# jhong93/vpd

Hardware: AMD Instinct MI355X
Metric: frame-crops/sec (VPD student train) (higher is better)
Workload: dtype bf16; 1 GPU; configs[1]: Diving48-shaped synthetic crops 128x128, ResNet-34 student (5-ch RGB+flow), emb_dim 128, sum-MSE + AdamW, batch=256 per GPU; global_batch=256, parallelism=dp1

## Files before the change

include/vpd_hip.h:

```cpp
#ifndef VPD_HIP_H
#define VPD_HIP_H
#include <stddef.h>
#ifdef __cplusplus
extern "C" {
#endif

typedef struct vpd_plan vpd_plan_t;

const char* vpd_last_error(void);
int vpd_abi_version(void);
const char* vpd_elem_dtype(void);

int vpd_plan_create(const char* arch, int c_in, int img_h, int img_w, int emb_dim, int motion,
                    int max_batch, int train, vpd_plan_t** out);
#define VPD_TRAIN_EARLY_BUCKET0 2
void vpd_plan_destroy(vpd_plan_t* plan);

int vpd_plan_num_tensors(const vpd_plan_t* plan);
int vpd_plan_tensor_info(const vpd_plan_t* plan, int i, int* kind, int* is_decoder, long long* offset,
                         long long* numel, int* ndim, int dims[4]);
long long vpd_plan_param_numel(const vpd_plan_t* plan);
int vpd_plan_num_bn(const vpd_plan_t* plan);
int vpd_plan_bn_info(const vpd_plan_t* plan, int i, int* channels, long long* rm_off, long long* rv_off);
long long vpd_plan_bn_numel(const vpd_plan_t* plan);

int vpd_plan_num_buckets(const vpd_plan_t* plan);
int vpd_plan_bucket_range(const vpd_plan_t* plan, int bucket, long long* offset, long long* numel);

size_t vpd_plan_workspace_bytes(const vpd_plan_t* plan);
int vpd_plan_init_workspace(vpd_plan_t* plan, void* workspace, void* stream);

int vpd_pack_weights(vpd_plan_t* plan, const float* params, const float* bn_running, void* workspace, void* stream);

int vpd_forward_eval(vpd_plan_t* plan, const float* params, const float* x, int n, float* emb_out,
                     const float* target, float* loss_step, double* loss_accum, void* workspace, void* stream);


int vpd_forward_train(vpd_plan_t* plan, const float* params, float* bn_running, const float* x,
                      const float* target, int n, float* emb_out, float* loss_step, double* loss_accum,
                      void* workspace, void* stream);

int vpd_backward(vpd_plan_t* plan, const float* params, float* grads, int n, void** bucket_events,
                 void* workspace, void* stream);

int vpd_backward_ext(vpd_plan_t* plan, const float* params, float* grads, const float* d_emb, int n, float* dx_nchw,
                     void** bucket_events, void* workspace, void* stream);

int vpd_adamw_step(float* params, const float* grads, float* adam_m, float* adam_v, long long numel,
                   double lr, double beta1, double beta2, double eps, double weight_decay, int step, void* stream);

int vpd_plan_adamw_step(vpd_plan_t* plan, float* params, const float* grads, float* adam_m, float* adam_v,
                        long long numel, double lr, double beta1, double beta2, double eps, double weight_decay,
                        int step, void* workspace, void* stream);

int vpd_plan_set_loss_scale(vpd_plan_t* plan, float scale);

typedef struct vpd_scale_state {
    float scale;
    unsigned int found;
    int growth_tracker;
    int applied_steps;
    int skipped_steps;
    int reserved[3];
} vpd_scale_state;

int vpd_plan_set_scale_state(vpd_plan_t* plan, const vpd_scale_state* state);

int vpd_plan_check_grads(vpd_plan_t* plan, const float* grads, long long numel, vpd_scale_state* state, void* workspace,
                         void* stream);
int vpd_op_check_finite(const float* x, long long n, vpd_scale_state* state, void* stream);

int vpd_adamw_step_scaled(float* params, const float* grads, float* adam_m, float* adam_v, long long numel, double lr,
                          double beta1, double beta2, double eps, double weight_decay, const vpd_scale_state* state,
                          void* stream);
int vpd_plan_adamw_step_scaled(vpd_plan_t* plan, float* params, const float* grads, float* adam_m, float* adam_v,
                               long long numel, double lr, double beta1, double beta2, double eps, double weight_decay,
                               const vpd_scale_state* state, void* workspace, void* stream);

int vpd_scale_state_update(vpd_scale_state* state, float growth, float backoff, int growth_interval, void* stream);

int vpd_plan_set_lazy_grads(vpd_plan_t* plan, int on);
int vpd_plan_bucket_scratch_range(const vpd_plan_t* plan, int bucket, long long* ws_byte_offset, long long* numel);
int vpd_plan_grads_pending(const vpd_plan_t* plan);
int vpd_plan_materialize_grads(vpd_plan_t* plan, float* grads, void* workspace, void* stream);

typedef struct vpd_aug_params {
    int order[4];
    float factor[4];
    int flip;
    int noise;
    int crop_i, crop_j, crop_h, crop_w;
    unsigned int seed_lo, seed_hi;
} vpd_aug_params;

int vpd_augment_crops(const unsigned char* rgb_u8, const unsigned char* flow_u8, const unsigned char* mask_u8,
                      const float* noise, const vpd_aug_params* params, int n, int height, int width, int out_dim,
                      const float* mean_std6, float noise_sd, float* out_nchw, float* scratch, void* stream);
int vpd_plan_stage_crops(vpd_plan_t* plan, const unsigned char* rgb_u8, const unsigned char* flow_u8,
                         const unsigned char* mask_u8, const float* noise, const vpd_aug_params* params, int n,
                         int height, int width, const float* mean_std6, float noise_sd, float* scratch,
                         void* workspace, void* stream);

int vpd_plan_stage_views(vpd_plan_t* plan, const unsigned char* rgb_u8, const unsigned char* flow_u8, int n_frames,
                         int k_views, int height, int width, const float* mean_std6, void* workspace, void* stream);

int vpd_augment_views(const unsigned char* rgb_u8, const unsigned char* flow_u8, const vpd_aug_params* params, int n_frames,
                      int jitter, int flip, int height, int width, const float* mean_std6, float* out_nchw, float* scratch,
                      void* stream);
int vpd_plan_stage_views_jitter(vpd_plan_t* plan, const unsigned char* rgb_u8, const unsigned char* flow_u8,
                                const vpd_aug_params* params, int n_frames, int jitter, int flip, int height, int width,
                                const float* mean_std6, float* scratch, void* workspace, void* stream);

int vpd_graph_capture_eval(vpd_plan_t* plan, const float* params, const float* x, int n, float* emb_out,
                           void* workspace, void* stream);
int vpd_graph_launch_eval(vpd_plan_t* plan, int n, void* stream);

int vpd_plan_sync_errors(vpd_plan_t* plan, void* workspace, void* stream, unsigned* count_out);

int vpd_plan_set_timing(vpd_plan_t* plan, int enable);
int vpd_plan_read_timing(vpd_plan_t* plan, double* out, int nclasses);

int vpd_op_conv2d(const void* x_bf16, const void* w_bf16, void* y_bf16, double* stats, int n, int xHp, int xWp,
                  int xC, int yHp, int yWp, int yC, int ypad, int Hs, int Ws, int osub, int oph, int opw, int istr,
                  int Kc, int Co, const int* tapset9, int accumulate, void* stream);
int vpd_op_conv_bm(int M, int Co);
int vpd_op_conv2d_ep(const void* x_bf16, const void* w_bf16, void* y_bf16, int n, int xHp, int xWp, int xC, int yHp, int yWp,
                     int yC, int ypad, int Hs, int Ws, int istr, int Kc, int Co, const int* tapset9, const float* ep_scale,
                     const float* ep_shift, const void* res_padded_bf16, int ep_relu, int accumulate,
                     const unsigned char* acc_mask, void* stream);
int vpd_op_conv2d_bnsums(const void* x_bf16, const void* w_bf16, void* y_bf16, const void* bst_z_bf16,
                         const unsigned char* bst_mask, double* rows, int n, int xHp, int xWp, int xC, int Hs, int Ws,
                         int Kc, int Co, const int* tapset9, int accumulate, void* stream);
int vpd_op_conv2d_bnsums2(const void* x_bf16, const void* w_bf16, void* y_bf16, const void* bst_z_bf16,
                          const unsigned char* bst_mask, double* rows, const void* bst_z2_bf16, double* rows2, int n, int xHp,
                          int xWp, int xC, int Hs, int Ws, int Kc, int Co, const int* tapset9, void* stream);
int vpd_op_conv2d_dispatch(int n, int xHp, int xWp, int xC, int yHp, int yWp, int yC, int ypad, int Hs, int Ws, int osub, int oph,
                           int opw, int istr, int Kc, int Co, const int* tapset9, int accumulate, int flags, int* out12);
int vpd_op_bn_forward(const void* z_bf16, const double* rows, const float* gamma, const float* beta, float* running_mean,
                      float* running_var, float* mean, float* rstd, float* scale, float* shift, const void* res_padded_bf16,
                      void* out_padded_bf16, unsigned char* mask_bits, int n, int H, int W, int C, int relu, float momentum,
                      float eps, void* stream);
int vpd_op_bn_backward_apply(const void* dy_bf16, const void* z_bf16, const unsigned char* mask_bits, const double* rows,
                             const float* gamma, const float* mean, const float* rstd, void* dz_padded_bf16, float* dgamma,
                             float* dbeta, int n, int H, int W, int C, void* stream);
int vpd_op_conv1x1_bn(int mode, const void* x_padded, const void* w, int n, int H, int W, int istr, int Kc, int Co, double* rows,
                      const float* gamma, const float* beta, float* running_mean, float* running_var, float momentum, float eps,
                      float* mean, float* rstd, float* scale, float* shift, const void* res_padded, void* out_padded,
                      unsigned char* mask_bits, const void* dout, void* dz_padded, float* dgamma, float* dbeta, void* stream);
int vpd_op_conv1x1_bn2(int mode, const void* x_padded, const void* w, const void* x2_padded, const void* w2, int n, int H, int W,
                       int Kc, int Kc2, int Co, double* rows, double* rows2, const float* gamma, const float* beta,
                       float* running_mean, float* running_var, float* mean, float* rstd, float* scale, float* shift,
                       const float* gamma2, const float* beta2, float* running_mean2, float* running_var2, float* mean2, float* rstd2,
                       float* scale2, float* shift2, float momentum, float eps, void* out_padded, unsigned char* mask_bits,
                       const void* dout, void* dz_padded, void* dz2_padded, float* dgamma, float* dbeta, float* dgamma2,
                       float* dbeta2, void* stream);
int vpd_op_conv1x1_bn_dispatch(int n, int H, int W, int Kc, int Co, int two, int* out5);
int vpd_op_stem_pool_forward(const void* z, const float* scale, const float* shift, void* out_padded, unsigned char* idx,
                             int n, int Hz, int Wz, int C, int opad, void* stream);
int vpd_op_stem_dgrad(const void* dz, const float* w_oihw, float* dx_nchw, int n, int c_in, int H, int W, void* stream);
int vpd_op_stem_pool_backward(const void* dpool, const unsigned char* idx, const void* z, const float* mean, const float* rstd,
                              const float* scale, const float* shift, const float* gamma, const float* beta,
                              const void* pooled_padded, double* rows, float* coef, void* dz, float* dgamma, float* dbeta,
                              int n, int Hz, int Wz, int C, void* stream);
int vpd_op_bn_backward(void* dy, const void* z, const void* act_padded, const unsigned char* mask_bits, const float* mscale,
                       const float* mshift, const float* dy_pooled, double* rows, float* coef, void* sync, unsigned* err,
                       const float* gamma, const float* mean, const float* rstd, void* dz, int dzpad, float* dgamma,
                       float* dbeta, int n, int H, int W, int C, int write_g, int fused, void* stream);
int vpd_op_bn_backward_pair(void* dy, const void* act_padded, const void* zA, const float* meanA, const float* rstdA,
                            const float* gammaA, double* rowsA, void* dzA, float* dgammaA, float* dbetaA, const void* zB,
                            const float* meanB, const float* rstdB, const float* gammaB, double* rowsB, void* dzB,
                            float* dgammaB, float* dbetaB, void* sync, unsigned* err, int n, int H, int W, int C, void* stream);
int vpd_op_bn_backward_residency(int M, int C, int pair, int* out4);
int vpd_op_avgpool(const void* act_padded, int n, int H, int W, int C, int pad, float* pooled, void* stream);
int vpd_op_avgpool_bwd(const float* dpooled, int n, int H, int W, int C, void* dact, void* stream);
int vpd_op_sgemm(const float* A, const float* B, float* Y, const float* bias, int M, int N, int K, int ta, int tb, int relu,
                 void* stream);
int vpd_op_colsum(const float* A, int M, int N, float* out, void* stream);
int vpd_op_relu_mask(float* d, const float* act, long long n, void* stream);
int vpd_op_mse(const float* e, const float* t, long long n, float* de, float* loss_step, double* loss_accum, void* stream);
int vpd_op_wgrad(const void* dz_bf16, const void* x_bf16, float* dw, int n, int dzHp, int dzWp, int dzC, int dzpad,
                 int xHp, int xWp, int xC, int Hs, int Ws, int istr, int Kc, int Co, const int* tapset9,
                 float* slab, void* stream);
size_t vpd_op_wgrad_slab_bytes(void);
int vpd_op_wgrad_pair(const void* dz_bf16, const void* dz2_bf16, const void* x_bf16, float* dw, float* dw2, int n, int dzHp, int dzWp,
                      int dzC, int dzpad, int xHp, int xWp, int xC, int Hs, int Ws, int istr, int Kc, int Co, const int* tapset9,
                      float* slab, float* slab2, void* stream);
int vpd_op_wgrad_pair_lds_bytes(int Hs, int Ws, int ns, long long* bytes);
int vpd_op_tr_read_probe(const void* tile_bf16, void* out_bf16, void* stream);
size_t vpd_op_wgrad128_table_bytes(void);
size_t vpd_op_wgrad128_slab_floats(int Co, int Ci);
int vpd_op_wgrad128_group(int nprob, const void* const* dz, const void* const* x, float* const* dw, float* const* slab,
                          const int* dims, void* dev_table, void* stream);
int vpd_op_wgrad128_schedule(int n, const int* dims4, int G, int* ksplit, int* blk_begin, int* tasks, int cap,
                             double* est_us);

#ifdef __cplusplus
}
#endif
#endif
```

vpd_amd/_lib.py:

```python
import ctypes as C
import os

_HERE = os.path.dirname(os.path.abspath(__file__))
LIB_PATH = os.environ.get("VPD_LIB_PATH") or os.path.join(_HERE, "libvpdhip.so")
LIB_PATH_F16 = os.environ.get("VPD_LIB_PATH_F16") or os.path.join(_HERE, "libvpdhip_f16.so")
ABI_VERSION = 5

c_int_p = C.POINTER(C.c_int)
c_ll_p = C.POINTER(C.c_longlong)
vp = C.c_void_p

SIGNATURES = {
    "vpd_last_error": (C.c_char_p, []),
    "vpd_abi_version": (C.c_int, []),
    "vpd_elem_dtype": (C.c_char_p, []),
    "vpd_plan_create": (C.c_int, [C.c_char_p, C.c_int, C.c_int, C.c_int, C.c_int, C.c_int, C.c_int, C.c_int,
                                  C.POINTER(vp)]),
    "vpd_plan_destroy": (None, [vp]),
    "vpd_plan_num_tensors": (C.c_int, [vp]),
    "vpd_plan_tensor_info": (C.c_int, [vp, C.c_int, c_int_p, c_int_p, c_ll_p, c_ll_p, c_int_p, c_int_p]),
    "vpd_plan_param_numel": (C.c_longlong, [vp]),
    "vpd_plan_num_bn": (C.c_int, [vp]),
    "vpd_plan_bn_info": (C.c_int, [vp, C.c_int, c_int_p, c_ll_p, c_ll_p]),
    "vpd_plan_bn_numel": (C.c_longlong, [vp]),
    "vpd_plan_num_buckets": (C.c_int, [vp]),
    "vpd_plan_bucket_range": (C.c_int, [vp, C.c_int, c_ll_p, c_ll_p]),
    "vpd_plan_workspace_bytes": (C.c_size_t, [vp]),
    "vpd_plan_init_workspace": (C.c_int, [vp, vp, vp]),
    "vpd_pack_weights": (C.c_int, [vp, vp, vp, vp, vp]),
    "vpd_forward_eval": (C.c_int, [vp, vp, vp, C.c_int, vp, vp, vp, vp, vp, vp]),
    "vpd_forward_train": (C.c_int, [vp, vp, vp, vp, vp, C.c_int, vp, vp, vp, vp, vp]),
    "vpd_backward": (C.c_int, [vp, vp, vp, C.c_int, C.POINTER(vp), vp, vp]),
    "vpd_backward_ext": (C.c_int, [vp, vp, vp, vp, C.c_int, vp, C.POINTER(vp), vp, vp]),
    "vpd_adamw_step": (C.c_int, [vp, vp, vp, vp, C.c_longlong, C.c_double, C.c_double, C.c_double, C.c_double,
                                 C.c_double, C.c_int, vp]),
    "vpd_plan_adamw_step": (C.c_int, [vp, vp, vp, vp, vp, C.c_longlong, C.c_double, C.c_double, C.c_double, C.c_double,
                                      C.c_double, C.c_int, vp, vp]),
    "vpd_augment_crops": (C.c_int, [vp, vp, vp, vp, vp, C.c_int, C.c_int, C.c_int, C.c_int, C.POINTER(C.c_float),
                                    C.c_float, vp, vp, vp]),
    "vpd_plan_stage_crops": (C.c_int, [vp, vp, vp, vp, vp, vp, C.c_int, C.c_int, C.c_int, C.POINTER(C.c_float),
                                       C.c_float, vp, vp, vp]),
    "vpd_plan_stage_views": (C.c_int, [vp, vp, vp, C.c_int, C.c_int, C.c_int, C.c_int, C.POINTER(C.c_float), vp, vp]),
    "vpd_augment_views": (C.c_int, [vp, vp, vp, C.c_int, C.c_int, C.c_int, C.c_int, C.c_int, C.POINTER(C.c_float), vp, vp, vp]),
    "vpd_plan_stage_views_jitter": (C.c_int, [vp, vp, vp, vp, C.c_int, C.c_int, C.c_int, C.c_int, C.c_int,
                                              C.POINTER(C.c_float), vp, vp, vp]),
    "vpd_graph_capture_eval": (C.c_int, [vp, vp, vp, C.c_int, vp, vp, vp]),
    "vpd_graph_launch_eval": (C.c_int, [vp, C.c_int, vp]),
    "vpd_plan_sync_errors": (C.c_int, [vp, vp, vp, C.POINTER(C.c_uint)]),
    "vpd_plan_set_lazy_grads": (C.c_int, [vp, C.c_int]),
    "vpd_plan_set_loss_scale": (C.c_int, [vp, C.c_float]),
    "vpd_plan_set_scale_state": (C.c_int, [vp, vp]),
    "vpd_plan_check_grads": (C.c_int, [vp, vp, C.c_longlong, vp, vp, vp]),
    "vpd_op_check_finite": (C.c_int, [vp, C.c_longlong, vp, vp]),
    "vpd_adamw_step_scaled": (C.c_int, [vp, vp, vp, vp, C.c_longlong, C.c_double, C.c_double, C.c_double, C.c_double,
                                        C.c_double, vp, vp]),
    "vpd_plan_adamw_step_scaled": (C.c_int, [vp, vp, vp, vp, vp, C.c_longlong, C.c_double, C.c_double, C.c_double, C.c_double,
                                             C.c_double, vp, vp, vp]),
    "vpd_scale_state_update": (C.c_int, [vp, C.c_float, C.c_float, C.c_int, vp]),
    "vpd_plan_bucket_scratch_range": (C.c_int, [vp, C.c_int, C.POINTER(C.c_longlong), C.POINTER(C.c_longlong)]),
    "vpd_plan_grads_pending": (C.c_int, [vp]),
    "vpd_plan_materialize_grads": (C.c_int, [vp, vp, vp, vp]),
    "vpd_plan_set_timing": (C.c_int, [vp, C.c_int]),
    "vpd_plan_read_timing": (C.c_int, [vp, C.POINTER(C.c_double), C.c_int]),
    "vpd_op_conv2d": (C.c_int, [vp, vp, vp, vp] + [C.c_int] * 16 + [c_int_p, C.c_int, vp]),
    "vpd_op_conv_bm": (C.c_int, [C.c_int, C.c_int]),
    "vpd_op_conv2d_ep": (C.c_int, [vp, vp, vp] + [C.c_int] * 13 + [c_int_p, vp, vp, vp, C.c_int, C.c_int, vp, vp]),
    "vpd_op_conv2d_bnsums": (C.c_int, [vp] * 6 + [C.c_int] * 8 + [c_int_p, C.c_int, vp]),
    "vpd_op_conv2d_bnsums2": (C.c_int, [vp] * 8 + [C.c_int] * 8 + [c_int_p, vp]),
    "vpd_op_conv2d_dispatch": (C.c_int, [C.c_int] * 16 + [c_int_p, C.c_int, C.c_int, c_int_p]),
    "vpd_op_bn_forward": (C.c_int, [vp] * 13 + [C.c_int] * 5 + [C.c_float, C.c_float, vp]),
    "vpd_op_bn_backward_apply": (C.c_int, [vp] * 10 + [C.c_int] * 4 + [vp]),
    "vpd_op_conv1x1_bn": (C.c_int, [C.c_int, vp, vp] + [C.c_int] * 6 + [vp] * 5 + [C.c_float, C.c_float] + [vp] * 12),
    "vpd_op_conv1x1_bn2": (C.c_int, [C.c_int] + [vp] * 4 + [C.c_int] * 6 + [vp] * 18 + [C.c_float, C.c_float] + [vp] * 10),
    "vpd_op_conv1x1_bn_dispatch": (C.c_int, [C.c_int] * 6 + [c_int_p]),
    "vpd_op_stem_pool_forward": (C.c_int, [vp] * 5 + [C.c_int] * 5 + [vp]),
    "vpd_op_stem_dgrad": (C.c_int, [vp, vp, vp, C.c_int, C.c_int, C.c_int, C.c_int, vp]),
    "vpd_op_stem_pool_backward": (C.c_int, [vp] * 15 + [C.c_int] * 4 + [vp]),
    "vpd_op_bn_backward": (C.c_int, [vp] * 15 + [C.c_int] + [vp, vp] + [C.c_int] * 6 + [vp]),
    "vpd_op_bn_backward_pair": (C.c_int, [vp] * 20 + [C.c_int] * 4 + [vp]),
    "vpd_op_bn_backward_residency": (C.c_int, [C.c_int, C.c_int, C.c_int, c_int_p]),
    "vpd_op_avgpool": (C.c_int, [vp] + [C.c_int] * 5 + [vp, vp]),
    "vpd_op_avgpool_bwd": (C.c_int, [vp] + [C.c_int] * 4 + [vp, vp]),
    "vpd_op_sgemm": (C.c_int, [vp] * 4 + [C.c_int] * 6 + [vp]),
    "vpd_op_colsum": (C.c_int, [vp, C.c_int, C.c_int, vp, vp]),
    "vpd_op_relu_mask": (C.c_int, [vp, vp, C.c_longlong, vp]),
    "vpd_op_mse": (C.c_int, [vp, vp, C.c_longlong, vp, vp, vp, vp]),
    "vpd_op_wgrad": (C.c_int, [vp, vp, vp] + [C.c_int] * 13 + [c_int_p, vp, vp]),
    "vpd_op_wgrad_slab_bytes": (C.c_size_t, []),
    "vpd_op_wgrad_pair": (C.c_int, [vp] * 5 + [C.c_int] * 13 + [c_int_p, vp, vp, vp]),
    "vpd_op_wgrad_pair_lds_bytes": (C.c_int, [C.c_int, C.c_int, C.c_int, c_ll_p]),
    "vpd_op_tr_read_probe": (C.c_int, [vp, vp, vp]),
    "vpd_op_wgrad128_table_bytes": (C.c_size_t, []),
    "vpd_op_wgrad128_slab_floats": (C.c_size_t, [C.c_int, C.c_int]),
    "vpd_op_wgrad128_group": (C.c_int, [C.c_int, vp, vp, vp, vp, c_int_p, vp, vp]),
    "vpd_op_wgrad128_schedule": (C.c_int, [C.c_int, c_int_p, C.c_int, c_int_p, c_int_p, c_int_p, C.c_int,
                                           C.POINTER(C.c_double)]),
}

_libs = {}


class VpdHipError(RuntimeError):
    pass


def lib(dtype="bf16"):
    if dtype in _libs:
        return _libs[dtype]
    if dtype not in ("bf16", "fp16"):
        raise VpdHipError("unknown element type %r (bf16 | fp16)" % (dtype,))
    path = LIB_PATH if dtype == "bf16" else LIB_PATH_F16
    name = os.path.basename(path)
    if not os.path.isfile(path):
        raise VpdHipError(
            "%s not found at %s: build it with `python -c 'import __graft_entry__ as g; g.build()'` "
            "or `make -C vpd_amd/csrc`.  vpd_amd has no PyTorch/CPU fallback." % (name, path))
    import torch
    h = C.CDLL(path)
    ab_build = "VPD_LIB_PATH" in os.environ and dtype == "bf16"
    for sym, (res, args) in SIGNATURES.items():
        try:
            fn = getattr(h, sym)
        except AttributeError as e:
            if ab_build and (sym.startswith("vpd_op_") or sym in ("vpd_elem_dtype", "vpd_plan_set_loss_scale", "vpd_backward_ext")):
                continue
            raise VpdHipError("%s lacks symbol %s declared in include/vpd_hip.h" % (name, sym)) from e
        fn.restype = res
        fn.argtypes = args
    if h.vpd_abi_version() != ABI_VERSION and not (ab_build and os.environ.get("VPD_LIB_ALLOW_ABI") == str(h.vpd_abi_version())):
        raise VpdHipError("%s ABI version %d != expected %d" % (name, h.vpd_abi_version(), ABI_VERSION))
    if hasattr(h, "vpd_elem_dtype") and h.vpd_elem_dtype().decode() != dtype:
        raise VpdHipError("%s was built with %s elements, %s asked for" % (path, h.vpd_elem_dtype().decode(), dtype))
    _libs[dtype] = h
    return h


def check(rc, what="", dtype="bf16"):
    if rc != 0:
        msg = lib(dtype).vpd_last_error()
        raise VpdHipError("%s failed: %s" % (what or "libvpdhip call", msg.decode() if msg else "unknown error"))
```

vpd_amd/csrc/head.hip:

```cpp
#include "../../include/vpd_hip.h"
#include "common.h"
#include "kernels.h"

__global__ __launch_bounds__(256) void avgpool_kernel(const bf16_t* act, int Hp, int Wp, int pad, int H, int W, int C,
                                                      int N, float* pooled) {
    const int cv = C >> 3;
    const long total = (long)N * cv;
    const float inv = 1.f / (float)(H * W);
    for (long it = (long)blockIdx.x * blockDim.x + threadIdx.x; it < total; it += (long)gridDim.x * blockDim.x) {
        const int b = (int)(it / cv);
        const int c = (int)(it - (long)b * cv) << 3;
        float acc[8] = {0, 0, 0, 0, 0, 0, 0, 0};
        if (H == 4 && W == 4) {
            uint4 px[16];
#pragma unroll
            for (int q = 0; q < 16; ++q)
                px[q] = *reinterpret_cast<const uint4*>(act + ((size_t)(b * Hp + (q >> 2) + pad) * Wp + (q & 3) + pad) * C + c);
#pragma unroll
            for (int q = 0; q < 16; ++q) {
                float v[8];
                unpack8(px[q], v);
#pragma unroll
                for (int j = 0; j < 8; ++j) acc[j] += v[j];
            }
        } else {
            for (int y = 0; y < H; ++y)
                for (int x = 0; x < W; ++x) {
                    float v[8];
                    unpack8(*reinterpret_cast<const uint4*>(act + ((size_t)(b * Hp + y + pad) * Wp + x + pad) * C + c), v);
#pragma unroll
                    for (int j = 0; j < 8; ++j) acc[j] += v[j];
                }
        }
        float* o = pooled + (size_t)b * C + c;
#pragma unroll
        for (int j = 0; j < 8; ++j) o[j] = acc[j] * inv;
    }
}
hipError_t vpd_launch_avgpool(const bf16_t* act, int Hp, int Wp, int pad, int H, int W, int C, int N, float* pooled,
                              hipStream_t s) {
    long items = (long)N * (C / 8);
    int g = (int)((items + 255) / 256);
    hipLaunchKernelGGL(avgpool_kernel, dim3(g < 1 ? 1 : g), dim3(256), 0, s, act, Hp, Wp, pad, H, W, C, N, pooled);
    return hipGetLastError();
}

__global__ __launch_bounds__(256) void avgpool_bwd_kernel(const float* dpooled, int HW, int C, int N, bf16_t* dact) {
    const int cv = C >> 3;
    const long total = (long)N * HW * cv;
    const float inv = 1.f / (float)HW;
    const bool pow2 = (HW & (HW - 1)) == 0;
    for (long it = (long)blockIdx.x * blockDim.x + threadIdx.x; it < total; it += (long)gridDim.x * blockDim.x) {
        const int c = (int)(it % cv) << 3;
        const long m = it / cv;
        const int b = (int)(m / HW);
        float v[8];
        const float* d = dpooled + (size_t)b * C + c;
#pragma unroll
        for (int j = 0; j < 8; ++j) v[j] = pow2 ? d[j] * inv : d[j] / (float)HW;
        *reinterpret_cast<uint4*>(dact + (size_t)m * C + c) = pack8(v);
    }
}
hipError_t vpd_launch_avgpool_bwd(const float* dpooled, int H, int W, int C, int N, bf16_t* dact, hipStream_t s) {
    long items = (long)N * H * W * (C / 8);
    long g = (items + 255) / 256;
    if (g > 4096) g = 4096;
    hipLaunchKernelGGL(avgpool_bwd_kernel, dim3(g < 1 ? 1 : (int)g), dim3(256), 0, s, dpooled, H * W, C, N, dact);
    return hipGetLastError();
}

__global__ __launch_bounds__(256) void sgemm_small_kernel(const float* A, const float* B, float* Y, const float* bias,
                                                          int M, int N, int K, int ta, int tb, int relu) {
    const int lane = threadIdx.x & 63;
    const int tiles_n = (N + 15) >> 4;
    const int tile = blockIdx.x * 4 + (threadIdx.x >> 6);
    const int tm = tile / tiles_n, tn = tile - tm * tiles_n;
    if (tm * 16 >= M) return;
    const int r = lane & 15, kq = lane >> 4;
    const int m = tm * 16 + r, n = tn * 16 + r;
    const bool mok = m < M, nok = n < N;
    f32x4 acc = {0.f, 0.f, 0.f, 0.f};
    const size_t a_m = ta ? (size_t)(mok ? m : 0) : (size_t)(mok ? m : 0) * K;
    const size_t a_k = ta ? (size_t)M : 1;
    const size_t b_n = tb ? (size_t)(nok ? n : 0) * K : (size_t)(nok ? n : 0);
    const size_t b_k = tb ? 1 : (size_t)N;
    for (int k0 = 0; k0 < K; k0 += 32) {
        float av[8], bv[8];
#pragma unroll
        for (int u = 0; u < 8; ++u) {
            const int k = k0 + 4 * u + kq;
            const bool kok = k < K;
            av[u] = (mok && kok) ? A[a_m + (size_t)k * a_k] : 0.f;
            bv[u] = (nok && kok) ? B[b_n + (size_t)k * b_k] : 0.f;
        }
#pragma unroll
        for (int u = 0; u < 8; ++u) acc = __builtin_amdgcn_mfma_f32_16x16x4f32(av[u], bv[u], acc, 0, 0, 0);
    }
    if (nok) {
        const float bb = bias ? bias[n] : 0.f;
#pragma unroll
        for (int j = 0; j < 4; ++j) {
            const int mm = tm * 16 + 4 * kq + j;
            if (mm < M) {
                float v = acc[j] + bb;
                if (relu) v = v > 0.f ? v : 0.f;
                Y[(size_t)mm * N + n] = v;
            }
        }
    }
}
__global__ __launch_bounds__(256) void sgemm_nt_splitk_kernel(const float* A, const float* B, float* Y, const float* bias,
                                                              int M, int N, int K, int relu) {
    __shared__ float red[4][16][17];
    const int lane = threadIdx.x & 63, wave = threadIdx.x >> 6;
    const int tiles_n = (N + 15) >> 4;
    const int tm = blockIdx.x / tiles_n, tn = blockIdx.x - tm * tiles_n;
    const int r = lane & 15, kq = lane >> 4;
    const int m = tm * 16 + r, n = tn * 16 + r;
    const bool mok = m < M, nok = n < N;
    const float4* Ap = reinterpret_cast<const float4*>(A + (size_t)(mok ? m : 0) * K);
    const float4* Bp = reinterpret_cast<const float4*>(B + (size_t)(nok ? n : 0) * K);
    const int kper = K / 4;
    f32x4 acc = {0.f, 0.f, 0.f, 0.f};
    for (int k0 = wave * kper; k0 < (wave + 1) * kper; k0 += 64) {
        float4 av[4], bv[4];
#pragma unroll
        for (int u = 0; u < 4; ++u) {
            const int k = k0 + 16 * u + 4 * kq;
            const bool kok = k < (wave + 1) * kper;
            av[u] = (mok && kok) ? Ap[k >> 2] : float4{0.f, 0.f, 0.f, 0.f};
            bv[u] = (nok && kok) ? Bp[k >> 2] : float4{0.f, 0.f, 0.f, 0.f};
        }
#pragma unroll
        for (int u = 0; u < 4; ++u) {
            acc = __builtin_amdgcn_mfma_f32_16x16x4f32(av[u].x, bv[u].x, acc, 0, 0, 0);
            acc = __builtin_amdgcn_mfma_f32_16x16x4f32(av[u].y, bv[u].y, acc, 0, 0, 0);
            acc = __builtin_amdgcn_mfma_f32_16x16x4f32(av[u].z, bv[u].z, acc, 0, 0, 0);
            acc = __builtin_amdgcn_mfma_f32_16x16x4f32(av[u].w, bv[u].w, acc, 0, 0, 0);
        }
    }
#pragma unroll
    for (int j = 0; j < 4; ++j) red[wave][4 * kq + j][r] = acc[j];
    __syncthreads();
    if (wave == 0 && nok) {
        const float bb = bias ? bias[n] : 0.f;
#pragma unroll
        for (int j = 0; j < 4; ++j) {
            const int mm = tm * 16 + 4 * kq + j;
            if (mm < M) {
                float v = ((red[0][4 * kq + j][r] + red[1][4 * kq + j][r]) + red[2][4 * kq + j][r]) + red[3][4 * kq + j][r] + bb;
                if (relu) v = v > 0.f ? v : 0.f;
                Y[(size_t)mm * N + n] = v;
            }
        }
    }
}

hipError_t vpd_launch_sgemm(const float* A, const float* B, float* Y, const float* bias, int M, int N, int K, int ta,
                            int tb, int relu, hipStream_t s) {
    const int tiles = ((M + 15) / 16) * ((N + 15) / 16);
    if (!ta && tb && K % 64 == 0 && K >= 64) {
        hipLaunchKernelGGL(sgemm_nt_splitk_kernel, dim3(tiles), dim3(256), 0, s, A, B, Y, bias, M, N, K, relu);
        return hipGetLastError();
    }
    hipLaunchKernelGGL(sgemm_small_kernel, dim3((tiles + 3) / 4), dim3(256), 0, s, A, B, Y, bias, M, N, K, ta, tb, relu);
    return hipGetLastError();
}

__global__ __launch_bounds__(256) void colsum_kernel(const float* A, int M, int N, float* out) {
    __shared__ float sh[8][32];
    const int tx = threadIdx.x & 31, ty = threadIdx.x >> 5;
    const int n = blockIdx.x * 32 + tx;
    float a = 0.f;
    if (n < N)
        for (int m = ty; m < M; m += 8) a += A[(size_t)m * N + n];
    sh[ty][tx] = a;
    __syncthreads();
    if (ty == 0 && n < N) {
        float t = 0.f;
#pragma unroll
        for (int i = 0; i < 8; ++i) t += sh[i][tx];
        out[n] = t;
    }
}
hipError_t vpd_launch_colsum(const float* A, int M, int N, float* out, hipStream_t s) {
    hipLaunchKernelGGL(colsum_kernel, dim3((N + 31) / 32), dim3(256), 0, s, A, M, N, out);
    return hipGetLastError();
}

__global__ void relu_mask_kernel(float* d, const float* act, long n) {
    for (long i = (long)blockIdx.x * blockDim.x + threadIdx.x; i < n; i += (long)gridDim.x * blockDim.x)
        d[i] = act[i] > 0.f ? d[i] : 0.f;
}
hipError_t vpd_launch_relu_mask(float* d, const float* act, long n, hipStream_t s) {
    long g = (n + 255) / 256;
    if (g > 1024) g = 1024;
    hipLaunchKernelGGL(relu_mask_kernel, dim3(g < 1 ? 1 : (int)g), dim3(256), 0, s, d, act, n);
    return hipGetLastError();
}

__global__ __launch_bounds__(1024) void mse_kernel(const float* e, const float* t, long n, float* de,
                                                   float* loss_step, double* loss_accum) {
    __shared__ float sh[16];
    float a = 0.f;
    const long n4 = n >> 2;
    for (long i0 = threadIdx.x; i0 < n4; i0 += 8 * 1024) {
        float4 ev[8], tv[8];
#pragma unroll
        for (int u = 0; u < 8; ++u) {
            const long i = i0 + u * 1024;
            const long ic = i < n4 ? i : i0;
            ev[u] = reinterpret_cast<const float4*>(e)[ic];
            tv[u] = reinterpret_cast<const float4*>(t)[ic];
        }
#pragma unroll
        for (int u = 0; u < 8; ++u) {
            const long i = i0 + u * 1024;
            if (i < n4) {
                const float4 d = {ev[u].x - tv[u].x, ev[u].y - tv[u].y, ev[u].z - tv[u].z, ev[u].w - tv[u].w};
                a += d.x * d.x + d.y * d.y + d.z * d.z + d.w * d.w;
                if (de) reinterpret_cast<float4*>(de)[i] = float4{2.f * d.x, 2.f * d.y, 2.f * d.z, 2.f * d.w};
            }
        }
    }
    for (long i = (n4 << 2) + threadIdx.x; i < n; i += 1024) {
        const float d = e[i] - t[i];
        a += d * d;
        if (de) de[i] = 2.f * d;
    }
    a = wave_sum(a);
    if ((threadIdx.x & 63) == 0) sh[threadIdx.x >> 6] = a;
    __syncthreads();
    if (threadIdx.x == 0) {
        float tot = 0.f;
#pragma unroll
        for (int i = 0; i < 16; ++i) tot += sh[i];
        if (loss_step) loss_step[0] = tot;
        if (loss_accum) loss_accum[0] += (double)tot;
    }
}
hipError_t vpd_launch_mse(const float* e, const float* t, long n, float* de, float* loss_step, double* loss_accum,
                          hipStream_t s) {
    hipLaunchKernelGGL(mse_kernel, dim3(1), dim3(1024), 0, s, e, t, n, de, loss_step, loss_accum);
    return hipGetLastError();
}


__global__ __launch_bounds__(256) void scale_kernel(float* x, long n, float s) {
    for (long i = (long)blockIdx.x * 256 + threadIdx.x; i < n; i += (long)gridDim.x * 256) x[i] *= s;
}
hipError_t vpd_launch_scale(float* x, long n, float s, hipStream_t stream) {
    if (n <= 0) return hipSuccess;
    long g = (n + 255) / 256;
    if (g > 1024) g = 1024;
    hipLaunchKernelGGL(scale_kernel, dim3((unsigned)g), dim3(256), 0, stream, x, n, s);
    return hipGetLastError();
}
__global__ __launch_bounds__(256) void scale_by_state_kernel(float* x, long n, const vpd_scale_state* st) {
    const float s = st->scale;
    for (long i = (long)blockIdx.x * 256 + threadIdx.x; i < n; i += (long)gridDim.x * 256) x[i] *= s;
}
hipError_t vpd_launch_scale_by_state(float* x, long n, const vpd_scale_state* st, hipStream_t stream) {
    if (n <= 0) return hipSuccess;
    long g = (n + 255) / 256;
    if (g > 1024) g = 1024;
    hipLaunchKernelGGL(scale_by_state_kernel, dim3((unsigned)g), dim3(256), 0, stream, x, n, st);
    return hipGetLastError();
}
```

vpd_amd/csrc/kernels.h:

```cpp
#pragma once
#include <vector>

#include "common.h"

struct BnApplyParams {
    const bf16_t* z;
    const float* scale; const float* shift;
    int res_kind;
    const bf16_t* res; int rHp, rWp, rpad;
    const float* rscale; const float* rshift;
    bf16_t* out; int oHp, oWp, opad;
    int M, H, W, C, relu;
    unsigned char* mask_out;
    int xcd_tile_px;
};

struct StemPoolParams {
    const bf16_t* z; int Hz, Wz;
    const float* scale; const float* shift;
    bf16_t* out; int opad;
    unsigned char* idx;
    int N, Ho, Wo, C;
};

struct BnBwdParams {
    const bf16_t* dy;
    bf16_t* dy_rw;
    const bf16_t* z;
    const bf16_t* act; int aHp, aWp, apad;
    const float* mean; const float* rstd;
    float* coef;
    double* partials;
    bf16_t* dz; int dzHp, dzWp, dzpad;
    int M, H, W, C, write_g, ppb;
    const float* mscale; const float* mshift;
    const unsigned char* mask_bits;
    const float* dy_pooled; float dy_pool_scale;
    int xcd_tile_px;
};

struct StemPoolBwdParams {
    const bf16_t* dpool;
    const unsigned char* idx;
    const bf16_t* z;
    const float* mean; const float* rstd; const float* scale; const float* shift;
    bf16_t* g;
    double* partials;
    int M, Hz, Wz, Ho, Wo, C, ppb;
    int pass; const float* coef; bf16_t* dz;
    const bf16_t* pooled; int ppad; const float* gamma_p; const float* beta_p;
};

struct PackDesc {
    long long src_off;
    long long fwd_off;
    long long dgr_off;
    long long wg_off;
    int Co, Ci, kh, kw, Kc, ntaps, stem;
    long long numel;
};
struct AdamHyper { float decay, omb1, b2, omb2, step_size, inv_sqrt_bc2, eps, gscale; };
struct vpd_scale_state;
struct AdamHyperDyn { AdamHyper h; const vpd_scale_state* st; double lr, b1, b2; };
#define FR_MAX 96
struct FiniteRanges {
    const float* ptr[FR_MAX];
    long n[FR_MAX];
    int count;
};

hipError_t vpd_launch_conv(const ConvParams& p, hipStream_t stream);
hipError_t vpd_launch_scale(float* x, long n, float s, hipStream_t stream);
bool vpd_conv1x1_stream_eligible(const ConvParams& p);
hipError_t vpd_launch_conv1x1_stream(const ConvParams& p, hipStream_t stream);
void vpd_conv1x1_stream_grid(const ConvParams& p, int* bm, int* bn, int* lanes);
int vpd_conv_kernel_class(const ConvParams& p);
bool vpd_conv_takes_bn_sums(const ConvParams& p);
struct ConvDispatch {
    int kclass;
    int pws;
    int geo;
    int c64x2;
    int ws1x1, stream1x1;
    int halo;
    int bm, bn;
    int mode;
    int tiles_per_block;
};
ConvDispatch vpd_conv_dispatch(const ConvParams& p);
int vpd_conv_xcd_tile_px(const ConvParams& p);
hipError_t vpd_launch_wgrad_reduce(const WgradParams& p, hipStream_t stream);
extern "C" int vpd_conv_bm(int M, int Co);
hipError_t vpd_launch_wgrad(const WgradParams& p, hipStream_t stream);
size_t vpd_wgrad_slab_bytes();
bool vpd_wgrad_group_eligible(const WgradParams& p);
size_t vpd_wgrad_group_slab_floats(int M, int Co, int Kc, int ntaps = 9);
hipError_t vpd_launch_wgrad_group(const WgradParams* ps, int n, hipStream_t stream);
bool vpd_wgrad_overwrites(const WgradParams& p);
bool vpd_wgrad_pair_ok(const WgradParams& p3, const WgradParams& p1);
hipError_t vpd_launch_wgrad_pair(const WgradParams& p3, const WgradParams& p1, hipStream_t stream);
hipError_t vpd_launch_wgrad_pair_reduce(const WgradParams& p3, const WgradParams& p1, hipStream_t stream);
int vpd_wgrad_pair_lds_query(int H, int W, int ns, long long* bytes);
bool vpd_wgrad128_eligible(const WgradParams& p);
size_t vpd_wgrad128_table_bytes();
void* vpd_wgrad128_cache_new();
void vpd_wgrad128_cache_free(void* cache);
hipError_t vpd_launch_wgrad128_group(const WgradParams* ps, int n, void* cache, void* dev_table, hipStream_t stream);
bool vpd_wgrad_halo_shape_ok(int Hout, int Wout, int stride = 1, int Hin = 0, int Win = 0);

hipError_t vpd_launch_bn_finalize(double* partials, int T, int C, float count, const float* gamma,
                                  const float* beta, float* rm, float* rv, float momentum, float eps,
                                  float* mean, float* rstd, float* scale, float* shift, hipStream_t s);
hipError_t vpd_launch_bn_fold(const float* gamma, const float* beta, const float* rm, const float* rv, float eps,
                              float* scale, float* shift, int C, hipStream_t s);
hipError_t vpd_launch_bn_apply(const BnApplyParams& p, hipStream_t s);
hipError_t vpd_launch_stem_pool(const StemPoolParams& p, hipStream_t s);
int vpd_bn_bwd_blocks(int M, int C, int* ppb_out);
hipError_t vpd_launch_bn_bwd(const BnBwdParams& p, float count, const float* gamma, float* dgamma, float* dbeta,
                             hipStream_t s, bool reduce_done = false);
hipError_t vpd_launch_stem_pool_bwd(const StemPoolBwdParams& p, float count, const float* gamma, float* dgamma,
                                    float* dbeta, float* coef, bf16_t* dz, hipStream_t s);

struct BnFusedFwd {
    double* rows; float count; const float* gamma; const float* beta; float* rm; float* rv;
    float* mean; float* rstd; float* scale; float* shift;
    double* rows2; float count2; const float* gamma2; const float* beta2; float* rm2; float* rv2;
    float* mean2; float* rstd2; float* scale2; float* shift2;
    float momentum, eps;
};
struct BnFusedBwd {
    double* rows; void* sync; unsigned* err;
    const float* gamma; float* dgamma; float* dbeta; float count;
};
struct BnBwdSecond {
    BnFusedBwd f;
    const bf16_t* z; const float* mean; const float* rstd;
    bf16_t* dz;
};
#define VPD_GRID_SYNC_BYTES (18 * 128)
hipError_t vpd_launch_bn_fwd_fused(const BnApplyParams& p, const BnFusedFwd& f, hipStream_t s);
bool vpd_conv1x1_bn_eligible(const ConvParams& p);
bool vpd_conv1x1_bn2_eligible(const ConvParams& p);
hipError_t vpd_launch_conv1x1_bn2(const ConvParams& p, const BnFusedFwd* fwd, const BnFusedBwd* bwd3, const BnFusedBwd* bwdD,
                                  const float* mean3, const float* rstd3, const float* meanD, const float* rstdD,
                                  unsigned char* mask_out, bf16_t* dz3, bf16_t* dzD, int dzpad, int mode, hipStream_t stream);
hipError_t vpd_launch_conv1x1_bn(const ConvParams& p, const BnFusedFwd* fwd, const BnFusedBwd* bwd, const float* mean,
                                 const float* rstd, unsigned char* mask_out, bf16_t* dz, int dzpad, int mode, hipStream_t stream);
void vpd_conv1x1_bn_grid(const ConvParams& p, bool two, int out4[4]);
bool vpd_bn_bwd_fused_ok(int M, int C, bool mask_act, bool write_g);
struct BnBwdFusedGeom { int G, ppb, iters, keep[3]; size_t lds; };
BnBwdFusedGeom vpd_bn_bwd_fused_geom(int M, int C, int nt);
hipError_t vpd_launch_bn_bwd_fused(const BnBwdParams& p, const BnFusedBwd& f, hipStream_t s);
hipError_t vpd_launch_bn_bwd_apply_fused(const BnBwdParams& p, const BnFusedBwd& f, hipStream_t s, const BnBwdSecond* B = nullptr);
bool vpd_bn_bwd_fused2_ok(int M, int C);
hipError_t vpd_launch_bn_bwd_fused2(const BnBwdParams& p, const BnFusedBwd& fA, const BnBwdSecond& B, hipStream_t s);

hipError_t vpd_launch_stem_dgrad(const bf16_t* dz, const float* w_oihw, float* dx_nchw, int N, int Cin, int H, int W,
                                 hipStream_t s);

hipError_t vpd_launch_avgpool(const bf16_t* act, int Hp, int Wp, int pad, int H, int W, int C, int N, float* pooled,
                              hipStream_t s);
hipError_t vpd_launch_avgpool_bwd(const float* dpooled, int H, int W, int C, int N, bf16_t* dact, hipStream_t s);
hipError_t vpd_launch_sgemm(const float* A, const float* B, float* Y, const float* bias, int M, int N, int K, int ta,
                            int tb, int relu, hipStream_t s);
hipError_t vpd_launch_colsum(const float* A, int M, int N, float* out, hipStream_t s);
hipError_t vpd_launch_relu_mask(float* d, const float* act, long n, hipStream_t s);
hipError_t vpd_launch_mse(const float* e, const float* t, long n, float* de, float* loss_step, double* loss_accum,
                          hipStream_t s);

hipError_t vpd_launch_pack_input(const float* x, int N, int C, int H, int W, bf16_t* out, int Hp, int Wp, int pad,
                                 int Cp, hipStream_t s);
hipError_t vpd_launch_pack_weights(const PackDesc* d_descs, int ndesc, const int* d_blockmap, int nblocks,
                                   const float* master, bf16_t* arena, hipStream_t s);
hipError_t vpd_launch_adamw_pack(const PackDesc* d_descs, const int* d_blockmap, int nblocks, float* p, const float* g,
                                 float* m, float* v, bf16_t* arena, double lr, double b1, double b2, double eps, double wd,
                                 int step, hipStream_t s, const float* wg = nullptr, float gscale = 1.f);
hipError_t vpd_launch_unpack_grads(const PackDesc* d_descs, int ndesc, const int* d_blockmap, int nblocks,
                                   const float* wg, float* grads, hipStream_t s);
hipError_t vpd_launch_adamw(float* p, const float* g, float* m, float* v, long n, double lr, double b1, double b2,
                            double eps, double wd, int step, hipStream_t s, float gscale = 1.f);
hipError_t vpd_launch_adamw_pack_scaled(const PackDesc* d_descs, const int* d_blockmap, int nblocks, float* p, const float* g,
                                        float* m, float* v, bf16_t* arena, double lr, double b1, double b2, double eps,
                                        double wd, const vpd_scale_state* st, hipStream_t s, const float* wg = nullptr);
hipError_t vpd_launch_adamw_scaled(float* p, const float* g, float* m, float* v, long n, double lr, double b1, double b2,
                                   double eps, double wd, const vpd_scale_state* st, hipStream_t s);
hipError_t vpd_launch_check_finite(const FiniteRanges& r, vpd_scale_state* st, hipStream_t s);
hipError_t vpd_launch_scale_update(vpd_scale_state* st, float growth, float backoff, int interval, hipStream_t s);
hipError_t vpd_launch_scale_by_state(float* x, long n, const vpd_scale_state* st, hipStream_t stream);

#define ZR_MAX 16
struct ZeroRanges {
    float* ptr[ZR_MAX];
    long n4[ZR_MAX];
    int count;
};
hipError_t vpd_launch_zero_ranges(const ZeroRanges& z, hipStream_t s);

struct vpd_aug_params;
hipError_t vpd_launch_augment(const unsigned char* rgb, const unsigned char* flow, const unsigned char* mask,
                              const float* noise, const vpd_aug_params* params, int N, int H, int W, int out_dim,
                              const float* mean_std6, float noise_sd, float* out_nchw, bf16_t* xin, int xHp, int xWp,
                              int xpad, float* cmean_scratch, hipStream_t s);
hipError_t vpd_launch_views(const unsigned char* rgb, const unsigned char* flow, int F, int K, int H, int W,
                            const float* mean_std6, bf16_t* xin, int xHp, int xWp, int xpad, hipStream_t s);
hipError_t vpd_launch_views_jitter(const unsigned char* rgb, const unsigned char* flow, const vpd_aug_params* params, int F,
                                   int J, int flip, int H, int W, const float* mean_std6, float* out_nchw, bf16_t* xin,
                                   int xHp, int xWp, int xpad, float* cmean_scratch, hipStream_t s);
```

vpd_amd/csrc/plan.h:

```cpp
#pragma once
#include <hip/hip_runtime.h>
#include <string.h>

#include <vector>

#include "../../include/vpd_hip.h"
#include "common.h"
#include "kernels.h"

int fail(const char* what, hipError_t e = hipSuccess);
#define HCHECK(expr)                                   \
    do {                                               \
        hipError_t _e = (expr);                        \
        if (_e != hipSuccess) return fail(#expr, _e);  \
    } while (0)
#define LCHECK(expr)                                   \
    do {                                               \
        hipError_t _e = (expr);                        \
        if (_e != hipSuccess) return fail(#expr, _e);  \
    } while (0)

constexpr float kBnEps = 1e-5f;
constexpr float kBnMomentum = 0.1f;

struct BnInfo {
    int C = 0;
    long long w_off = 0, b_off = 0;
    long long rm_off = 0, rv_off = 0;
    size_t fl_off = 0;
    size_t rows_off = 0;
    size_t sync_off = 0;
};
struct ConvInfo {
    int Ci = 0, Co = 0, k = 0, stride = 1, pad = 0;
    int Hin = 0, Win = 0, Hout = 0, Wout = 0;
    bool stem = false;
    int Kc = 0, ntaps = 0;
    long long w_off = 0;
    long long fwd_off = 0, dgr_off = -1;
    long long wg_off = 0;
    long long slab_off = -1;
    size_t dz_own_off = 0;
    long long gslab_off = 0;
    BnInfo bn;
    size_t z_off = 0;
};
struct BlockInfo {
    ConvInfo c1, c2, c3, cd;
    bool ds = false;
    int stage = 0;
    size_t a1_off = 0, a2_off = 0, out_off = 0;
    size_t mask_off = 0;
    size_t mask1_off = 0;
    size_t mask2_off = 0;
};
struct StageInfo {
    int H = 0, W = 0, C = 0;
    size_t dz2_off[2] = {0, 0}, dz1_off[2] = {0, 0}, dzd_off = 0, idn_off = 0;
    size_t dz3_off = 0;
};
struct TensorRow {
    int kind, is_dec;
    long long off, numel;
    int ndim, dims[4];
};
struct LinInfo {
    int in = 0, out = 0;
    long long w_off = 0, b_off = 0;
};

struct vpd_plan {
    int c_in, H, W, D, motion, max_batch, train;
    int bottleneck = 0, base_width = 64, feat = 512;
    std::vector<int> layers;
    ConvInfo stem;
    std::vector<BlockInfo> blocks;
    StageInfo stages[4];
    LinInfo fc, dec[3];
    std::vector<TensorRow> tensors;
    std::vector<BnInfo*> bns;
    long long nparam = 0, nparam_padded = 0, nbn = 0;
    long long arena_elems = 0, wg_elems = 0, slab_elems = 0;
    long long bucket_off[4], bucket_numel[4];
    long long bucket_wg_off[4], bucket_wg_numel[4];
    size_t ws_bytes = 0;
    size_t xin_off = 0, arena_off = 0, wg_off = 0, partial_off = 0, z0_off = 0, p0_off = 0, idx_off = 0;
    size_t g0_off = 0, dz0_off = 0, G_off[3] = {0, 0, 0}, T_off[2] = {0, 0}, slab_off = 0;
    size_t pooled_off = 0, emb_off = 0, h1_off = 0, h2_off = 0, pred_off = 0;
    size_t dpred_off = 0, dh2_off = 0, dh1_off = 0, demb_off = 0, dpooled_off = 0;
    size_t desc_off = 0, bmap_pack_off = 0, bmap_unpack_off[4] = {0, 0, 0, 0};
    int xHp = 0, xWp = 0;
    int H0 = 0, W0 = 0, H1 = 0, W1 = 0;
    std::vector<PackDesc> descs;
    std::vector<int> bmap_pack;
    std::vector<int> bmap_adam;
    size_t bmap_adam_off = 0;
    int nstem_pack_blocks = 0;
    std::vector<int> bmap_unpack[4];
    size_t partial_bytes = 0;
    struct Graph { int n; hipGraph_t g; hipGraphExec_t e; };
    std::vector<Graph> graphs;
    void* bound_ws = nullptr;
    bool fused_bn = true;
    size_t fused_off = 0, fused_bytes = 0;
    size_t syncerr_off = 0;
    bool wg_group = true;
    size_t gslab_off = 0;
    bool dgrad_sums = true;
    bool relu_bits = true;
    bool lazy_next = false, grads_in_scratch = false;
    bool fwd_had_x = false;
    int nstem_unpack_blocks = 0;
    bool wg_merge34 = true;
    bool early_bucket0 = false;
    float loss_scale = 1.f;
    const vpd_scale_state* scale_state = nullptr;
    size_t wg2_tbl_off[8] = {0, 0, 0, 0, 0, 0, 0, 0};
    void* wg2_cache[8] = {nullptr, nullptr, nullptr, nullptr, nullptr, nullptr, nullptr, nullptr};
    bool timing = false;
    struct TimedLaunch { int cls; double flops; hipEvent_t a, b; };
    std::vector<TimedLaunch> timed;
    std::vector<hipEvent_t> ev_pool;
};

int check_call(const vpd_plan* p, const void* ws, int n, int min_n = 1);

inline TapSet conv_taps_fwd(const ConvInfo& c) {
    TapSet t;
    if (c.stem) {
        t.nr = c.k; t.nc = 1; t.dy0 = 0; t.dys = 1; t.dx0 = 0; t.dxs = 0; t.w0 = 0; t.wrs = 1; t.wcs = 0;
    } else {
        t.nr = c.k; t.nc = c.k; t.dy0 = 1 - c.pad; t.dys = 1; t.dx0 = 1 - c.pad; t.dxs = 1;
        t.w0 = 0; t.wrs = c.k; t.wcs = 1;
    }
    return t;
}

inline WgradParams wgrad_params(const ConvInfo& cv, int n, const bf16_t* dz, const bf16_t* x) {
    WgradParams q;
    memset(&q, 0, sizeof q);
    q.dz = dz; q.dzHp = cv.Hout + 2; q.dzWp = cv.Wout + 2; q.dzC = cv.Co; q.dzpad = 1;
    q.x = x; q.xHp = cv.Hin + 2; q.xWp = cv.Win + 2; q.xC = cv.Ci;
    q.N = n; q.Hs = cv.Hout; q.Ws = cv.Wout; q.istr = cv.stride; q.Kc = cv.Kc; q.Co = cv.Co;
    q.M = n * cv.Hout * cv.Wout;
    q.taps = conv_taps_fwd(cv);
    return q;
}
inline WgradParams grouped_wgrad_params(const ConvInfo& cv, int n, const bf16_t* dz, const bf16_t* x) {
    WgradParams q = wgrad_params(cv, n, dz, x);
    if (cv.k == 1 && cv.stride == 1 && cv.Co % 128 != 0 && cv.Ci % 128 == 0) {
        q.dz = x; q.dzC = cv.Ci; q.x = dz; q.xC = cv.Co; q.Co = cv.Ci; q.Kc = cv.Co; q.transposed = 1;
    }
    return q;
}
```

vpd_amd/csrc/plan.hip:

```cpp
#include <hip/hip_runtime.h>
#include <math.h>
#include <stdio.h>
#include <stdlib.h>
#include <string.h>

#include <string>
#include <algorithm>
#include <vector>

#include "plan.h"

static thread_local std::string g_err;
int fail(const char* what, hipError_t e) {
    char buf[512];
    if (e != hipSuccess) snprintf(buf, sizeof buf, "%s: %s", what, hipGetErrorString(e));
    else snprintf(buf, sizeof buf, "%s", what);
    g_err = buf;
    return -1;
}

extern "C" const char* vpd_last_error(void) { return g_err.c_str(); }
extern "C" const char* vpd_elem_dtype(void) { return VPD_ELEM_NAME; }
extern "C" int vpd_abi_version(void) { return 5; }

namespace {

struct Bump {
    size_t cur = 0;
    size_t take(size_t bytes) {
        size_t o = cur;
        cur += (bytes + 255) & ~(size_t)255;
        return o;
    }
};

inline size_t padded_elems(int n, int H, int W, int C, int pad) {
    return (size_t)n * (H + 2 * pad) * (W + 2 * pad) * C;
}

void add_tensor(vpd_plan* p, int kind, int is_dec, long long numel, int ndim, int d0, int d1, int d2, int d3,
                long long* off_out) {
    TensorRow r;
    r.kind = kind; r.is_dec = is_dec; r.off = p->nparam; r.numel = numel; r.ndim = ndim;
    r.dims[0] = d0; r.dims[1] = d1; r.dims[2] = d2; r.dims[3] = d3;
    p->tensors.push_back(r);
    *off_out = p->nparam;
    p->nparam += numel;
}

void add_conv(vpd_plan* p, ConvInfo& c, int Ci, int Co, int k, int stride, int pad, int Hin, int Win, bool stem) {
    c.Ci = Ci; c.Co = Co; c.k = k; c.stride = stride; c.pad = pad; c.Hin = Hin; c.Win = Win; c.stem = stem;
    c.Hout = (Hin + 2 * pad - k) / stride + 1;
    c.Wout = (Win + 2 * pad - k) / stride + 1;
    if (stem) { c.Kc = 64; c.ntaps = k; } else { c.Kc = Ci; c.ntaps = k * k; }
    add_tensor(p, 0, 0, (long long)Co * Ci * k * k, 4, Co, Ci, k, k, &c.w_off);
    c.bn.C = Co;
    add_tensor(p, 1, 0, Co, 1, Co, 0, 0, 0, &c.bn.w_off);
    add_tensor(p, 2, 0, Co, 1, Co, 0, 0, 0, &c.bn.b_off);
    c.bn.rm_off = p->nbn; c.bn.rv_off = p->nbn + Co;
    p->nbn += 2 * Co;
    c.fwd_off = p->arena_elems;
    p->arena_elems += (long long)c.ntaps * Co * c.Kc;
    if (!stem) {
        c.dgr_off = p->arena_elems;
        p->arena_elems += (long long)k * k * Ci * Co;
    }
    c.wg_off = p->wg_elems;
    p->wg_elems += (long long)c.ntaps * Co * c.Kc;
    if (stem && p->train && p->slab_elems == 0)
        p->slab_elems += 2 * (long long)(vpd_wgrad_slab_bytes() / 4);
    if (!stem && ((k == 3 && pad == 1) || (k == 1 && pad == 0)) && (stride == 1 || stride == 2) && p->train &&
        vpd_wgrad_halo_shape_ok(c.Hout, c.Wout, stride, Hin, Win)) {
        c.slab_off = k == 1 ? (long long)(vpd_wgrad_slab_bytes() / 4) : 0;
    }
}

}

extern "C" int vpd_plan_create(const char* arch, int c_in, int img_h, int img_w, int emb_dim, int motion,
                               int max_batch, int train, vpd_plan_t** out) {
    if (!arch || !out) return fail("null argument");
    std::vector<int> layers;
    int bottleneck = 0, base_width = 64;
    if (!strcmp(arch, "resnet18")) layers = {2, 2, 2, 2};
    else if (!strcmp(arch, "resnet34")) layers = {3, 4, 6, 3};
    else if (!strcmp(arch, "resnet50")) { layers = {3, 4, 6, 3}; bottleneck = 1; }
    else if (!strcmp(arch, "resnet101")) { layers = {3, 4, 23, 3}; bottleneck = 1; }
    else if (!strcmp(arch, "wide_resnet50_2")) { layers = {3, 4, 6, 3}; bottleneck = 1; base_width = 128; }
    else if (!strcmp(arch, "wide_resnet101_2")) { layers = {3, 4, 23, 3}; bottleneck = 1; base_width = 128; }
    else return fail("unsupported arch (resnet18 | resnet34 | resnet50 | resnet101 | wide_resnet50_2 | wide_resnet101_2)");
    if (c_in < 1 || c_in > 8) return fail("c_in must be in 1..8");
    if (img_h < 32 || img_w < 32 || (img_h % 2) || (img_w % 2)) return fail("img dims must be even and >= 32");
    if (emb_dim < 1 || max_batch < 1) return fail("bad emb_dim / max_batch");

    vpd_plan* p = new vpd_plan();
    p->c_in = c_in; p->H = img_h; p->W = img_w; p->D = emb_dim; p->motion = motion ? 1 : 0;
    p->max_batch = max_batch; p->train = train ? 1 : 0; p->layers = layers;
    p->early_bucket0 = (train & VPD_TRAIN_EARLY_BUCKET0) != 0;
    p->bottleneck = bottleneck; p->base_width = base_width; p->feat = bottleneck ? 2048 : 512;

    add_conv(p, p->stem, c_in, 64, 7, 2, 3, img_h, img_w, true);
    p->bns.push_back(&p->stem.bn);
    p->H0 = p->stem.Hout; p->W0 = p->stem.Wout;
    p->H1 = (p->H0 + 2 - 3) / 2 + 1; p->W1 = (p->W0 + 2 - 3) / 2 + 1;
    int inplanes = 64, h = p->H1, w = p->W1;
    const int widths[4] = {64, 128, 256, 512};
    long long stage_first_tensor_off[5];
    int nblocks_total = 0;
    for (int s = 0; s < 4; ++s) nblocks_total += layers[s];
    p->blocks.resize(nblocks_total);
    int bi = 0;
    for (int s = 0; s < 4; ++s) {
        stage_first_tensor_off[s] = p->nparam;
        for (int b = 0; b < layers[s]; ++b, ++bi) {
            BlockInfo& B = p->blocks[bi];
            const int stride = (b == 0 && s > 0) ? 2 : 1;
            B.stage = s;
            if (!bottleneck) {
                add_conv(p, B.c1, inplanes, widths[s], 3, stride, 1, h, w, false);
                add_conv(p, B.c2, widths[s], widths[s], 3, 1, 1, B.c1.Hout, B.c1.Wout, false);
                B.ds = (stride != 1 || inplanes != widths[s]);
                if (B.ds) add_conv(p, B.cd, inplanes, widths[s], 1, stride, 0, h, w, false);
                h = B.c1.Hout; w = B.c1.Wout; inplanes = widths[s];
            } else {
                const int width = widths[s] * base_width / 64, outc = widths[s] * 4;
                add_conv(p, B.c1, inplanes, width, 1, 1, 0, h, w, false);
                add_conv(p, B.c2, width, width, 3, stride, 1, h, w, false);
                add_conv(p, B.c3, width, outc, 1, 1, 0, B.c2.Hout, B.c2.Wout, false);
                B.ds = (stride != 1 || inplanes != outc);
                if (B.ds) add_conv(p, B.cd, inplanes, outc, 1, stride, 0, h, w, false);
                h = B.c2.Hout; w = B.c2.Wout; inplanes = outc;
            }
        }
        p->stages[s].H = h; p->stages[s].W = w; p->stages[s].C = inplanes;
    }
    for (auto& B : p->blocks) {
        p->bns.push_back(&B.c1.bn);
        p->bns.push_back(&B.c2.bn);
        if (bottleneck) p->bns.push_back(&B.c3.bn);
        if (B.ds) p->bns.push_back(&B.cd.bn);
    }
    if (h < 1 || w < 1) { delete p; return fail("image too small for 5 stride-2 stages"); }
    stage_first_tensor_off[4] = p->nparam;
    p->fc.in = p->feat; p->fc.out = emb_dim;
    add_tensor(p, 3, 0, (long long)emb_dim * p->feat, 2, emb_dim, p->feat, 0, 0, &p->fc.w_off);
    add_tensor(p, 4, 0, emb_dim, 1, emb_dim, 0, 0, 0, &p->fc.b_off);
    if (p->motion) {
        const int dims[4] = {emb_dim, 128, 128, 2 * emb_dim};
        for (int i = 0; i < 3; ++i) {
            p->dec[i].in = dims[i]; p->dec[i].out = dims[i + 1];
            add_tensor(p, 3, 1, (long long)dims[i + 1] * dims[i], 2, dims[i + 1], dims[i], 0, 0, &p->dec[i].w_off);
            add_tensor(p, 4, 1, dims[i + 1], 1, dims[i + 1], 0, 0, 0, &p->dec[i].b_off);
        }
    }
    p->nparam_padded = (p->nparam + 3) & ~3LL;
    p->bucket_off[0] = stage_first_tensor_off[3]; p->bucket_numel[0] = p->nparam - stage_first_tensor_off[3];
    p->bucket_off[1] = stage_first_tensor_off[2]; p->bucket_numel[1] = stage_first_tensor_off[3] - stage_first_tensor_off[2];
    p->bucket_off[2] = stage_first_tensor_off[1]; p->bucket_numel[2] = stage_first_tensor_off[2] - stage_first_tensor_off[1];
    p->bucket_off[3] = 0; p->bucket_numel[3] = stage_first_tensor_off[1];

    auto push_desc = [&](const ConvInfo& c, int bucket) {
        PackDesc d;
        d.src_off = c.w_off; d.fwd_off = c.fwd_off; d.dgr_off = c.dgr_off; d.wg_off = c.wg_off;
        d.Co = c.Co; d.Ci = c.Ci; d.kh = c.k; d.kw = c.k; d.Kc = c.Kc; d.ntaps = c.ntaps; d.stem = c.stem ? 1 : 0;
        d.numel = 0;
        const int id = (int)p->descs.size();
        p->descs.push_back(d);
        const long long nf = (long long)c.ntaps * c.Co * c.Kc;
        const long long ns = (long long)c.Co * c.Ci * c.k * c.k;
        const long long npk = nf > ns ? nf : ns;
        const long long npack = c.stem ? (npk + 1023) / 1024 : (long long)(c.Co / 32) * (c.Ci / 32);
        for (long long ch = 0; ch < npack; ++ch) { p->bmap_pack.push_back(id); p->bmap_pack.push_back((int)ch); }
        const long long uchunk = 1024;
        for (long long ch = 0; ch * uchunk < ns; ++ch) {
            p->bmap_unpack[bucket].push_back(id);
            p->bmap_unpack[bucket].push_back((int)ch);
        }
    };
    push_desc(p->stem, 3);
    p->nstem_unpack_blocks = (int)p->bmap_unpack[3].size() / 2;
    for (int b = 0; b < 4; ++b) { p->bucket_wg_off[b] = -1; p->bucket_wg_numel[b] = 0; }
    for (auto& B : p->blocks) {
        const int bucket = 3 - B.stage;
        push_desc(B.c1, bucket);
        push_desc(B.c2, bucket);
        if (bottleneck) push_desc(B.c3, bucket);
        if (B.ds) push_desc(B.cd, bucket);
        auto take = [&](const ConvInfo& cv) {
            const long long n = (long long)cv.ntaps * cv.Co * cv.Kc;
            if (p->bucket_wg_off[bucket] < 0) p->bucket_wg_off[bucket] = cv.wg_off;
            p->bucket_wg_off[bucket] = std::min(p->bucket_wg_off[bucket], (long long)cv.wg_off);
            p->bucket_wg_numel[bucket] += n;
        };
        take(B.c1); take(B.c2);
        if (bottleneck) take(B.c3);
        if (B.ds) take(B.cd);
    }
    {
        long long at = (long long)p->stem.ntaps * p->stem.Co * p->stem.Kc;
        for (int b = 3; b >= 0; --b) {
            if (p->bucket_wg_off[b] != at) { delete p; return fail("internal: weight-gradient scratch is not bucket-contiguous"); }
            at += p->bucket_wg_numel[b];
        }
        if (at != p->wg_elems) { delete p; return fail("internal: weight-gradient scratch size mismatch"); }
    }
    {
        const int nconv = (int)p->descs.size();
        for (size_t i = 0; i + 1 < p->bmap_pack.size(); i += 2) {
            if (p->bmap_pack[i] == 0) { p->nstem_pack_blocks++; continue; }
            p->bmap_adam.push_back(p->bmap_pack[i]); p->bmap_adam.push_back(p->bmap_pack[i + 1]);
        }
        std::vector<std::pair<long long, long long>> convs;
        for (int i = 1; i < nconv; ++i)
            convs.push_back({p->descs[i].src_off, (long long)p->descs[i].Co * p->descs[i].Ci * p->descs[i].kh * p->descs[i].kw});
        std::sort(convs.begin(), convs.end());
        long long pos = 0;
        auto plain = [&](long long a, long long b) {
            if (b <= a) return;
            PackDesc d = {};
            d.src_off = a; d.numel = b - a; d.stem = 2; d.kh = d.kw = 1; d.dgr_off = -1;
            const int id = (int)p->descs.size();
            p->descs.push_back(d);
            for (long long ch = 0; ch * 2048 < b - a; ++ch) { p->bmap_adam.push_back(id); p->bmap_adam.push_back((int)ch); }
        };
        for (auto& cv : convs) { plain(pos, cv.first); pos = cv.first + cv.second; }
        plain(pos, p->nparam_padded);
    }

    Bump bp;
    const int NB = max_batch;
    p->xHp = img_h + 6; p->xWp = img_w + 8;
    p->xin_off = bp.take(((size_t)NB * p->xHp * p->xWp * 8 + 256) * 2);
    p->arena_off = bp.take((size_t)p->arena_elems * 2);
    p->wg_off = bp.take((size_t)p->wg_elems * 4);
    for (BnInfo* b : p->bns) b->fl_off = bp.take((size_t)9 * b->C * 4);
    p->fused_bn = vpd_switches().fused_bn;
    {
        const size_t start = bp.cur;
        for (BnInfo* b : p->bns) {
            b->rows_off = bp.take((size_t)VPD_FUSED_ROWS * 2 * b->C * sizeof(double));
            b->sync_off = bp.take(VPD_GRID_SYNC_BYTES);
        }
        p->fused_off = start; p->fused_bytes = bp.cur - start;
        p->syncerr_off = bp.take(256);
    }
    p->desc_off = bp.take(p->descs.size() * sizeof(PackDesc));
    p->bmap_pack_off = bp.take(p->bmap_pack.size() * sizeof(int));
    p->bmap_adam_off = bp.take(p->bmap_adam.size() * sizeof(int));
    for (int i = 0; i < 4; ++i) p->bmap_unpack_off[i] = bp.take(p->bmap_unpack[i].size() * sizeof(int) + 16);
    p->partial_bytes = (size_t)VPD_STAT_ROWS * 2 * p->feat * sizeof(double);
    p->partial_off = bp.take(p->partial_bytes);
    p->z0_off = bp.take((size_t)NB * p->H0 * p->W0 * 64 * 2);
    p->p0_off = bp.take(padded_elems(NB, p->H1, p->W1, 64, 1) * 2);
    for (auto& B : p->blocks) {
        B.a1_off = bp.take(padded_elems(NB, B.c1.Hout, B.c1.Wout, B.c1.Co, 1) * 2);
        if (bottleneck) {
            B.a2_off = bp.take(padded_elems(NB, B.c2.Hout, B.c2.Wout, B.c2.Co, 1) * 2);
            B.out_off = bp.take(padded_elems(NB, B.c3.Hout, B.c3.Wout, B.c3.Co, 1) * 2);
        } else {
            B.out_off = bp.take(padded_elems(NB, B.c1.Hout, B.c1.Wout, B.c1.Co, 1) * 2);
        }
    }
    for (int s = 0; s < 4; ++s) {
        StageInfo& S = p->stages[s];
        S.idn_off = bp.take(padded_elems(NB, S.H, S.W, S.C, 1) * 2);
    }
    p->pooled_off = bp.take((size_t)NB * p->feat * 4);
    p->emb_off = bp.take((size_t)NB * emb_dim * 4);
    p->h1_off = bp.take((size_t)NB * 128 * 4);
    p->h2_off = bp.take((size_t)NB * 128 * 4);
    p->pred_off = bp.take((size_t)NB * 2 * emb_dim * 4);
    if (p->train) {
        p->idx_off = bp.take((size_t)NB * p->H1 * p->W1 * 64);
        size_t maxact = (size_t)NB * p->H1 * p->W1 * 64;
        for (auto& B : p->blocks) {
            B.c1.z_off = bp.take((size_t)NB * B.c1.Hout * B.c1.Wout * B.c1.Co * 2);
            B.c2.z_off = bp.take((size_t)NB * B.c2.Hout * B.c2.Wout * B.c2.Co * 2);
            if (bottleneck) B.c3.z_off = bp.take((size_t)NB * B.c3.Hout * B.c3.Wout * B.c3.Co * 2);
            if (B.ds) B.cd.z_off = bp.take((size_t)NB * B.cd.Hout * B.cd.Wout * B.cd.Co * 2);
            size_t e = (size_t)NB * B.c1.Hout * B.c1.Wout * B.c1.Co;
            maxact = e > maxact ? e : maxact;
            if (bottleneck) {
                e = (size_t)NB * B.c1.Hin * B.c1.Win * B.c1.Ci; maxact = e > maxact ? e : maxact;
                e = (size_t)NB * B.c2.Hout * B.c2.Wout * B.c2.Co; maxact = e > maxact ? e : maxact;
                e = (size_t)NB * B.c3.Hout * B.c3.Wout * B.c3.Co; maxact = e > maxact ? e : maxact;
            }
        }
        for (int s = 0; s < 4; ++s) {
            StageInfo& S = p->stages[s];
            for (int k = 0; k < 2; ++k) {
                S.dz2_off[k] = bp.take(padded_elems(NB, S.H, S.W, S.C, 1) * 2);
                S.dz1_off[k] = bp.take(padded_elems(NB, S.H, S.W, S.C, 1) * 2);
            }
            S.dzd_off = bp.take(padded_elems(NB, S.H, S.W, S.C, 1) * 2);
        }
        if (bottleneck) {
            for (int s = 0; s < 4; ++s) {
                size_t m1 = 0, m2 = 0, m3 = 0;
                for (auto& B : p->blocks) {
                    if (B.stage != s) continue;
                    size_t e1 = padded_elems(NB, B.c1.Hout, B.c1.Wout, B.c1.Co, 1), e2 = padded_elems(NB, B.c2.Hout, B.c2.Wout, B.c2.Co, 1),
                           e3 = padded_elems(NB, B.c3.Hout, B.c3.Wout, B.c3.Co, 1);
                    m1 = e1 > m1 ? e1 : m1; m2 = e2 > m2 ? e2 : m2; m3 = e3 > m3 ? e3 : m3;
                }
                StageInfo& S = p->stages[s];
                S.dz1_off[0] = S.dz1_off[1] = bp.take(m1 * 2);
                S.dz2_off[0] = S.dz2_off[1] = bp.take(m2 * 2);
                S.dz3_off = bp.take(m3 * 2);
            }
            for (int i = 0; i < 2; ++i) p->T_off[i] = bp.take(maxact * 2);
        }
        p->wg_group = vpd_switches().wg_group;
        p->wg_merge34 = vpd_switches().wg_merge && !p->early_bucket0;
        if (p->wg_group) {
            size_t stage_slab[4] = {0, 0, 0, 0};
            for (auto& B : p->blocks) {
                std::vector<ConvInfo*> cvs = {&B.c1, &B.c2};
                if (bottleneck) cvs.push_back(&B.c3);
                if (B.ds) cvs.push_back(&B.cd);
                for (ConvInfo* cv : cvs) {
                    if (cv->slab_off < 0) continue;
                    if (cv->k == 1) {
                        if (!bottleneck || !vpd_wgrad128_eligible(grouped_wgrad_params(*cv, NB, nullptr, nullptr))) continue;
                    } else if (cv->k != 3) {
                        continue;
                    } else if (cv->stride != 1) {
                        continue;
                    }
                    cv->dz_own_off = bp.take(padded_elems(NB, cv->Hout, cv->Wout, cv->Co, 1) * 2);
                    const int grp = (p->wg_merge34 && B.stage == 3) ? 2 : B.stage;
                    cv->gslab_off = (long long)stage_slab[grp];
                    stage_slab[grp] += vpd_wgrad_group_slab_floats(NB * cv->Hout * cv->Wout, cv->Co, cv->Kc, cv->k == 1 ? 1 : 9);
                }
            }
            size_t mx = 16;
            for (int s2 = 0; s2 < 4; ++s2) mx = stage_slab[s2] > mx ? stage_slab[s2] : mx;
            p->gslab_off = bp.take(mx * 4);
            for (int s2 = 0; s2 < 8; ++s2) p->wg2_tbl_off[s2] = bp.take(vpd_wgrad128_table_bytes());
        }
        p->relu_bits = vpd_switches().relu_bits;
        if (p->relu_bits)
            for (auto& B : p->blocks) {
                const ConvInfo& last = bottleneck ? B.c3 : B.c2;
                B.mask_off = bp.take((size_t)NB * last.Hout * last.Wout * last.Co / 8 + 16);
            }
        p->dgrad_sums = p->relu_bits && p->fused_bn && vpd_switches().dgrad_sums;
        if (p->dgrad_sums)
            for (auto& B : p->blocks) {
                if (bottleneck && B.stage < 2) continue;
                B.mask1_off = bp.take((size_t)NB * B.c1.Hout * B.c1.Wout * B.c1.Co / 8 + 16);
                if (bottleneck) B.mask2_off = bp.take((size_t)NB * B.c2.Hout * B.c2.Wout * B.c2.Co / 8 + 16);
            }
        for (int i = 0; i < 3; ++i) p->G_off[i] = bp.take(maxact * 2);
        p->slab_off = bp.take((size_t)(p->slab_elems > 0 ? p->slab_elems : 1) * 4);
        p->g0_off = bp.take((size_t)NB * p->H0 * p->W0 * 64 * 2);
        p->dz0_off = bp.take((size_t)NB * p->H0 * p->W0 * 64 * 2);
        p->dpred_off = bp.take((size_t)NB * 2 * emb_dim * 4);
        p->dh2_off = bp.take((size_t)NB * 128 * 4);
        p->dh1_off = bp.take((size_t)NB * 128 * 4);
        p->demb_off = bp.take((size_t)NB * emb_dim * 4);
        p->dpooled_off = bp.take((size_t)NB * p->feat * 4);
    }
    p->ws_bytes = bp.cur;
    *out = p;
    return 0;
}

extern "C" void vpd_plan_destroy(vpd_plan_t* p) {
    if (!p) return;
    for (auto& g : p->graphs) {
        (void)hipGraphExecDestroy(g.e);
        (void)hipGraphDestroy(g.g);
    }
    for (auto& t : p->timed) { (void)hipEventDestroy(t.a); (void)hipEventDestroy(t.b); }
    for (auto e : p->ev_pool) (void)hipEventDestroy(e);
    for (int i = 0; i < 8; ++i)
        if (p->wg2_cache[i]) vpd_wgrad128_cache_free(p->wg2_cache[i]);
    delete p;
}

extern "C" int vpd_plan_num_tensors(const vpd_plan_t* p) { return (int)p->tensors.size(); }
extern "C" int vpd_plan_tensor_info(const vpd_plan_t* p, int i, int* kind, int* is_decoder, long long* offset,
                                    long long* numel, int* ndim, int dims[4]) {
    if (i < 0 || i >= (int)p->tensors.size()) return fail("tensor index out of range");
    const TensorRow& r = p->tensors[i];
    *kind = r.kind; *is_decoder = r.is_dec; *offset = r.off; *numel = r.numel; *ndim = r.ndim;
    for (int k = 0; k < 4; ++k) dims[k] = r.dims[k];
    return 0;
}
extern "C" long long vpd_plan_param_numel(const vpd_plan_t* p) { return p->nparam_padded; }
extern "C" int vpd_plan_num_bn(const vpd_plan_t* p) { return (int)p->bns.size(); }
extern "C" int vpd_plan_bn_info(const vpd_plan_t* p, int i, int* channels, long long* rm_off, long long* rv_off) {
    if (i < 0 || i >= (int)p->bns.size()) return fail("bn index out of range");
    *channels = p->bns[i]->C; *rm_off = p->bns[i]->rm_off; *rv_off = p->bns[i]->rv_off;
    return 0;
}
extern "C" long long vpd_plan_bn_numel(const vpd_plan_t* p) { return p->nbn; }
extern "C" int vpd_plan_num_buckets(const vpd_plan_t*) { return 4; }
extern "C" int vpd_plan_bucket_range(const vpd_plan_t* p, int b, long long* offset, long long* numel) {
    if (b < 0 || b >= 4) return fail("bucket index out of range");
    *offset = p->bucket_off[b]; *numel = p->bucket_numel[b];
    return 0;
}
extern "C" int vpd_plan_bucket_scratch_range(const vpd_plan_t* p, int b, long long* ws_byte_offset, long long* numel) {
    if (b < 0 || b >= 4) return fail("bucket index out of range");
    if (!p->train) return fail("plan was created with train=0");
    *ws_byte_offset = (long long)p->wg_off + p->bucket_wg_off[b] * 4;
    *numel = p->bucket_wg_numel[b];
    return 0;
}
extern "C" size_t vpd_plan_workspace_bytes(const vpd_plan_t* p) { return p->ws_bytes; }

extern "C" int vpd_plan_init_workspace(vpd_plan_t* p, void* ws, void* stream) {
    hipStream_t s = (hipStream_t)stream;
    char* w = (char*)ws;
    HCHECK(hipMemsetAsync(ws, 0, p->ws_bytes, s));
    HCHECK(hipMemcpyAsync(w + p->desc_off, p->descs.data(), p->descs.size() * sizeof(PackDesc), hipMemcpyHostToDevice, s));
    HCHECK(hipMemcpyAsync(w + p->bmap_pack_off, p->bmap_pack.data(), p->bmap_pack.size() * sizeof(int), hipMemcpyHostToDevice, s));
    HCHECK(hipMemcpyAsync(w + p->bmap_adam_off, p->bmap_adam.data(), p->bmap_adam.size() * sizeof(int), hipMemcpyHostToDevice, s));
    for (int i = 0; i < 4; ++i)
        if (!p->bmap_unpack[i].empty())
            HCHECK(hipMemcpyAsync(w + p->bmap_unpack_off[i], p->bmap_unpack[i].data(),
                                  p->bmap_unpack[i].size() * sizeof(int), hipMemcpyHostToDevice, s));
    HCHECK(hipStreamSynchronize(s));
    p->bound_ws = ws;
    return 0;
}

int check_call(const vpd_plan* p, const void* ws, int n, int min_n) {
    if (!p || !ws) return fail("null plan / workspace");
    if (p->bound_ws != ws) return fail("workspace not initialised with vpd_plan_init_workspace");
    if (n < min_n || n > p->max_batch) return fail(min_n ? "batch size outside 1..max_batch" : "batch size outside 0..max_batch");
    return 0;
}

extern "C" int vpd_augment_crops(const unsigned char* rgb_u8, const unsigned char* flow_u8, const unsigned char* mask_u8,
                                 const float* noise, const vpd_aug_params* params, int n, int height, int width,
                                 int out_dim, const float* mean_std6, float noise_sd, float* out_nchw, float* scratch,
                                 void* stream) {
    if (!rgb_u8 || !params || !mean_std6 || !out_nchw || !scratch) return fail("null argument");
    if (n < 1 || height < 1 || width < 1 || out_dim < 1) return fail("bad shape");
    LCHECK(vpd_launch_augment(rgb_u8, flow_u8, mask_u8, noise, params, n, height, width, out_dim, mean_std6, noise_sd,
                              out_nchw, nullptr, 0, 0, 0, scratch, (hipStream_t)stream));
    return 0;
}

extern "C" int vpd_plan_stage_crops(vpd_plan_t* p, const unsigned char* rgb_u8, const unsigned char* flow_u8,
                                    const unsigned char* mask_u8, const float* noise, const vpd_aug_params* params,
                                    int n, int height, int width, const float* mean_std6, float noise_sd,
                                    float* scratch, void* workspace, void* stream) {
    if (n > 65535) return fail("more than 65535 crops per staging call");
    if (check_call(p, workspace, n)) return -1;
    if (!rgb_u8 || !params || !mean_std6 || !scratch) return fail("null argument");
    if (p->H != p->W) return fail("the input pipeline resizes to a square img_dim");
    if ((p->c_in == 5) != (flow_u8 != nullptr)) return fail("flow_u8 must be given exactly when the plan has 5 input channels");
    char* ws = (char*)workspace;
    LCHECK(vpd_launch_augment(rgb_u8, flow_u8, mask_u8, noise, params, n, height, width, p->H, mean_std6, noise_sd,
                              nullptr, reinterpret_cast<bf16_t*>(ws + p->xin_off), p->xHp, p->xWp, 3, scratch,
                              (hipStream_t)stream));
    return 0;
}

extern "C" int vpd_plan_stage_views(vpd_plan_t* p, const unsigned char* rgb_u8, const unsigned char* flow_u8, int n_frames,
                                    int k_views, int height, int width, const float* mean_std6, void* workspace,
                                    void* stream) {
    if (n_frames < 0 || (k_views != 1 && k_views != 2)) return fail("k_views must be 1 (frame) or 2 (frame, h-flip)");
    if ((long)n_frames * k_views > 65535) return fail("n_frames * k_views exceeds 65535 views per staging call");
    if (check_call(p, workspace, n_frames * k_views)) return -1;
    if (!rgb_u8 || !mean_std6) return fail("null argument");
    if (height != p->H || width != p->W) return fail("inference views are not resized: the frames must have the plan's size");
    if (width % 4) return fail("width must be a multiple of 4");
    if ((p->c_in == 5) != (flow_u8 != nullptr)) return fail("flow_u8 must be given exactly when the plan has 5 input channels");
    if (p->c_in != 3 && p->c_in != 5) return fail("inference views: 3 or 5 input channels");
    if (n_frames == 0) return 0;
    char* ws = (char*)workspace;
    LCHECK(vpd_launch_views(rgb_u8, flow_u8, n_frames, k_views, height, width, mean_std6,
                            reinterpret_cast<bf16_t*>(ws + p->xin_off), p->xHp, p->xWp, 3, (hipStream_t)stream));
    return 0;
}

static int check_jitter_views(const unsigned char* rgb_u8, const vpd_aug_params* params, int n_frames, int jitter, int height,
                              int width, const float* mean_std6, const float* scratch) {
    if (n_frames < 0 || jitter < 0) return fail("n_frames and jitter must not be negative");
    if (!rgb_u8 || !mean_std6) return fail("null argument");
    if (jitter > 0 && (!params || !scratch)) return fail("jittered views need params and scratch");
    if (height < 1 || width < 1) return fail("bad shape");
    if (width % 4) return fail("width must be a multiple of 4");
    return 0;
}

extern "C" int vpd_augment_views(const unsigned char* rgb_u8, const unsigned char* flow_u8, const vpd_aug_params* params,
                                 int n_frames, int jitter, int flip, int height, int width, const float* mean_std6,
                                 float* out_nchw, float* scratch, void* stream) {
    if (check_jitter_views(rgb_u8, params, n_frames, jitter, height, width, mean_std6, scratch)) return -1;
    if (!out_nchw) return fail("null argument");
    if ((long)n_frames * (1 + jitter) * (flip ? 2 : 1) > 65535) return fail("n_frames * views exceeds 65535 views per call");
    if (n_frames == 0) return 0;
    LCHECK(vpd_launch_views_jitter(rgb_u8, flow_u8, params, n_frames, jitter, flip, height, width, mean_std6, out_nchw,
                                   nullptr, 0, 0, 0, scratch, (hipStream_t)stream));
    return 0;
}

extern "C" int vpd_plan_stage_views_jitter(vpd_plan_t* p, const unsigned char* rgb_u8, const unsigned char* flow_u8,
                                           const vpd_aug_params* params, int n_frames, int jitter, int flip, int height,
                                           int width, const float* mean_std6, float* scratch, void* workspace,
                                           void* stream) {
    if (check_jitter_views(rgb_u8, params, n_frames, jitter, height, width, mean_std6, scratch)) return -1;
    const long views = (long)n_frames * (1 + jitter) * (flip ? 2 : 1);
    if (views > 65535) return fail("n_frames * views exceeds 65535 views per staging call");
    if (check_call(p, workspace, (int)views)) return -1;
    if (height != p->H || width != p->W) return fail("inference views are not resized: the frames must have the plan's size");
    if ((p->c_in == 5) != (flow_u8 != nullptr)) return fail("flow_u8 must be given exactly when the plan has 5 input channels");
    if (p->c_in != 3 && p->c_in != 5) return fail("inference views: 3 or 5 input channels");
    if (n_frames == 0) return 0;
    char* ws = (char*)workspace;
    LCHECK(vpd_launch_views_jitter(rgb_u8, flow_u8, params, n_frames, jitter, flip, height, width, mean_std6, nullptr,
                                   reinterpret_cast<bf16_t*>(ws + p->xin_off), p->xHp, p->xWp, 3, scratch,
                                   (hipStream_t)stream));
    return 0;
}

extern "C" int vpd_adamw_step(float* params, const float* grads, float* adam_m, float* adam_v, long long numel,
                              double lr, double beta1, double beta2, double eps, double weight_decay, int step,
                              void* stream) {
    if (!params || !grads || !adam_m || !adam_v) return fail("null argument");
    if (numel % 4) return fail("numel must be a multiple of 4 (use vpd_plan_param_numel)");
    if (step < 1) return fail("step is 1-based");
    LCHECK(vpd_launch_adamw(params, grads, adam_m, adam_v, (long)numel, lr, beta1, beta2, eps, weight_decay, step,
                            (hipStream_t)stream));
    return 0;
}

extern "C" int vpd_plan_adamw_step(vpd_plan_t* p, float* params, const float* grads, float* adam_m, float* adam_v,
                                   long long numel, double lr, double beta1, double beta2, double eps,
                                   double weight_decay, int step, void* workspace, void* stream) {
    if (!p || !params || !grads || !adam_m || !adam_v || !workspace) return fail("null argument");
    if (p->bound_ws != workspace) return fail("workspace not initialised with vpd_plan_init_workspace");
    if (numel % 4 || numel < p->nparam_padded) return fail("numel must be a multiple of 4 and cover the plan's parameters");
    if (step < 1) return fail("step is 1-based");
    hipStream_t s = (hipStream_t)stream;
    char* ws = (char*)workspace;
    LCHECK(vpd_launch_adamw_pack(reinterpret_cast<const PackDesc*>(ws + p->desc_off),
                                 reinterpret_cast<const int*>(ws + p->bmap_adam_off), (int)p->bmap_adam.size() / 2, params,
                                 grads, adam_m, adam_v, reinterpret_cast<bf16_t*>(ws + p->arena_off), lr, beta1, beta2,
                                 eps, weight_decay, step, s,
// ... 280 lines not shown
    if (q.taps.nr < 1 || q.taps.nc < 1) return fail("empty tap set");
    const ConvDispatch d = vpd_conv_dispatch(q);
    const int v[12] = {d.kclass, d.pws, d.geo, d.c64x2, d.ws1x1, d.stream1x1, d.halo, d.bm, d.bn, d.mode, d.tiles_per_block,
                       (flags & 8) ? (int)vpd_conv_takes_bn_sums(q) : 0};
    memcpy(out12, v, sizeof v);
    return 0;
}

extern "C" int vpd_op_bn_forward(const void* z, const double* rows, const float* gamma, const float* beta, float* running_mean,
                                 float* running_var, float* mean, float* rstd, float* scale, float* shift, const void* res,
                                 void* out, unsigned char* mask_bits, int n, int H, int W, int C, int relu, float momentum,
                                 float eps, void* stream) {
    if (!z || !rows || !gamma || !beta || !mean || !rstd || !scale || !shift || !out) return fail("null argument");
    BnApplyParams a;
    memset(&a, 0, sizeof a);
    a.z = (const bf16_t*)z;
    a.res_kind = res ? 1 : 0; a.res = (const bf16_t*)res; a.rHp = H + 2; a.rWp = W + 2; a.rpad = 1;
    a.out = (bf16_t*)out; a.oHp = H + 2; a.oWp = W + 2; a.opad = 1;
    a.M = n * H * W; a.H = H; a.W = W; a.C = C; a.relu = relu; a.mask_out = mask_bits;
    BnFusedFwd f;
    memset(&f, 0, sizeof f);
    f.rows = const_cast<double*>(rows); f.count = (float)a.M; f.gamma = gamma; f.beta = beta; f.rm = running_mean; f.rv = running_var;
    f.mean = mean; f.rstd = rstd; f.scale = scale; f.shift = shift; f.momentum = momentum; f.eps = eps;
    LCHECK(vpd_launch_bn_fwd_fused(a, f, (hipStream_t)stream));
    return 0;
}

extern "C" int vpd_op_bn_backward_apply(const void* dy, const void* z, const unsigned char* mask_bits, const double* rows,
                                        const float* gamma, const float* mean, const float* rstd, void* dz, float* dgamma,
                                        float* dbeta, int n, int H, int W, int C, void* stream) {
    if (!dy || !z || !mask_bits || !rows || !gamma || !mean || !rstd || !dz || !dgamma || !dbeta) return fail("null argument");
    BnBwdParams b;
    memset(&b, 0, sizeof b);
    b.dy = (const bf16_t*)dy; b.z = (const bf16_t*)z; b.mean = mean; b.rstd = rstd;
    b.dz = (bf16_t*)dz; b.dzHp = H + 2; b.dzWp = W + 2; b.dzpad = 1;
    b.M = n * H * W; b.H = H; b.W = W; b.C = C; b.mask_bits = mask_bits;
    BnFusedBwd f;
    memset(&f, 0, sizeof f);
    f.rows = const_cast<double*>(rows); f.gamma = gamma; f.dgamma = dgamma; f.dbeta = dbeta; f.count = (float)b.M;
    LCHECK(vpd_launch_bn_bwd_apply_fused(b, f, (hipStream_t)stream));
    return 0;
}

static ConvParams op_conv1x1_bn_params(const void* x, const void* w, int n, int H, int W, int istr, int Kc, int Co) {
    ConvParams q;
    memset(&q, 0, sizeof q);
    q.x = (const bf16_t*)x; q.xHp = H * istr + 2; q.xWp = W * istr + 2; q.xC = Kc; q.w = (const bf16_t*)w;
    q.yHp = H; q.yWp = W; q.yC = Co; q.ypad = 0;
    q.N = n; q.Hs = H; q.Ws = W; q.osub = 1; q.istr = istr;
    q.Kc = Kc; q.Co = Co; q.M = n * H * W;
    q.taps.nr = 1; q.taps.nc = 1; q.taps.dy0 = 1; q.taps.dys = 1; q.taps.dx0 = 1; q.taps.dxs = 1; q.taps.w0 = 0; q.taps.wrs = 1; q.taps.wcs = 1;
    return q;
}
static bool op_conv1x1_bn_shape_ok(int n, int H, int W, int istr, int Kc, int Co) {
    return n >= 1 && H >= 1 && W >= 1 && istr >= 1 && Kc >= 64 && Kc % 64 == 0 && Co >= 64 && Co % 64 == 0 &&
           (long long)n * H * W < (1ll << 31);
}

extern "C" int vpd_op_conv1x1_bn(int mode, const void* x, const void* w, int n, int H, int W, int istr, int Kc, int Co, double* rows,
                                 const float* gamma, const float* beta, float* running_mean, float* running_var, float momentum,
                                 float eps, float* mean, float* rstd, float* scale, float* shift, const void* res, void* out,
                                 unsigned char* mask_bits, const void* dout, void* dz, float* dgamma, float* dbeta, void* stream) {
    if (mode < 0 || mode > 3) return fail("mode 0 .. 3");
    if (!x || !w || !rows) return fail("null argument");
    if (mode == 1 && (!gamma || !beta || !mean || !rstd || !scale || !shift || !res || !out || (running_mean == nullptr) != (running_var == nullptr)))
        return fail("null argument");
    if (mode >= 2 && (!dout || !mask_bits)) return fail("null argument");
    if (mode == 3 && (!gamma || !mean || !rstd || !dz || !dgamma || !dbeta)) return fail("null argument");
    if (!op_conv1x1_bn_shape_ok(n, H, W, istr, Kc, Co)) return fail("bad argument");
    ConvParams q = op_conv1x1_bn_params(x, w, n, H, W, istr, Kc, Co);
    if (!vpd_conv1x1_bn_eligible(q)) return fail("conv1x1_bn_stream_kernel does not take this shape");
    BnFusedFwd f;
    BnFusedBwd b;
    memset(&f, 0, sizeof f);
    memset(&b, 0, sizeof b);
    if (mode == 0) { q.stats = rows; q.stat_rows = VPD_FUSED_ROWS; }
    else if (mode == 1) {
        q.y = (bf16_t*)out; q.yHp = H + 2; q.yWp = W + 2; q.ypad = 1;
        q.res = (const bf16_t*)res; q.rHp = H + 2; q.rWp = W + 2; q.rC = Co; q.rpad = 1;
        f.rows = rows; f.count = (float)q.M; f.gamma = gamma; f.beta = beta; f.rm = running_mean; f.rv = running_var;
        f.mean = mean; f.rstd = rstd; f.scale = scale; f.shift = shift; f.momentum = momentum; f.eps = eps;
    } else {
        q.y = (bf16_t*)const_cast<void*>(dout); q.acc_mask = mask_bits;
        b.rows = rows; b.gamma = gamma; b.dgamma = dgamma; b.dbeta = dbeta; b.count = (float)q.M;
    }
    LCHECK(vpd_launch_conv1x1_bn(q, mode == 1 ? &f : nullptr, mode >= 2 ? &b : nullptr, mode == 3 ? mean : nullptr,
                                 mode == 3 ? rstd : nullptr, mode == 1 ? mask_bits : nullptr, mode == 3 ? (bf16_t*)dz : nullptr,
                                 mode == 3 ? 1 : 0, mode, (hipStream_t)stream));
    return 0;
}

extern "C" int vpd_op_conv1x1_bn2(int mode, const void* x, const void* w, const void* x2, const void* w2, int n, int H, int W, int Kc,
                                  int Kc2, int Co, double* rows, double* rows2, const float* gamma, const float* beta,
                                  float* running_mean, float* running_var, float* mean, float* rstd, float* scale, float* shift,
                                  const float* gamma2, const float* beta2, float* running_mean2, float* running_var2, float* mean2,
                                  float* rstd2, float* scale2, float* shift2, float momentum, float eps, void* out,
                                  unsigned char* mask_bits, const void* dout, void* dz, void* dz2, float* dgamma, float* dbeta,
                                  float* dgamma2, float* dbeta2, void* stream) {
    if (mode < 1 || mode > 3) return fail("mode 1 .. 3");
    if (!x || !w || !x2 || !w2 || !rows || !rows2) return fail("null argument");
    if (mode == 1 && (!gamma || !beta || !mean || !rstd || !scale || !shift || !gamma2 || !beta2 || !mean2 || !rstd2 || !scale2 || !shift2 ||
                      !out || (running_mean == nullptr) != (running_var == nullptr) || (running_mean == nullptr) != (running_mean2 == nullptr) ||
                      (running_mean2 == nullptr) != (running_var2 == nullptr)))
        return fail("null argument");
    if (mode >= 2 && (!dout || !mask_bits)) return fail("null argument");
    if (mode == 3 && (!gamma || !mean || !rstd || !gamma2 || !mean2 || !rstd2 || !dz || !dz2 || !dgamma || !dbeta || !dgamma2 || !dbeta2))
        return fail("null argument");
    if (!op_conv1x1_bn_shape_ok(n, H, W, 1, Kc, Co) || Kc2 < 1) return fail("bad argument");
    ConvParams q = op_conv1x1_bn_params(x, w, n, H, W, 1, Kc, Co);
    q.x2 = (const bf16_t*)x2; q.w2 = (const bf16_t*)w2; q.Kc2 = Kc2;
    if (!vpd_conv1x1_bn2_eligible(q)) return fail("conv1x1_bn2_stream_kernel does not take this shape");
    BnFusedFwd f;
    BnFusedBwd b3, bd;
    memset(&f, 0, sizeof f);
    memset(&b3, 0, sizeof b3);
    memset(&bd, 0, sizeof bd);
    if (mode == 1) {
        q.y = (bf16_t*)out; q.yHp = H + 2; q.yWp = W + 2; q.ypad = 1;
        f.rows = rows; f.count = (float)q.M; f.gamma = gamma; f.beta = beta; f.rm = running_mean; f.rv = running_var;
        f.mean = mean; f.rstd = rstd; f.scale = scale; f.shift = shift;
        f.rows2 = rows2; f.count2 = (float)q.M; f.gamma2 = gamma2; f.beta2 = beta2; f.rm2 = running_mean2; f.rv2 = running_var2;
        f.mean2 = mean2; f.rstd2 = rstd2; f.scale2 = scale2; f.shift2 = shift2;
        f.momentum = momentum; f.eps = eps;
    } else {
        q.y = (bf16_t*)const_cast<void*>(dout); q.acc_mask = mask_bits;
        b3.rows = rows; b3.gamma = gamma; b3.dgamma = dgamma; b3.dbeta = dbeta; b3.count = (float)q.M;
        bd.rows = rows2; bd.gamma = gamma2; bd.dgamma = dgamma2; bd.dbeta = dbeta2; bd.count = (float)q.M;
    }
    const bool m3 = mode == 3;
    LCHECK(vpd_launch_conv1x1_bn2(q, mode == 1 ? &f : nullptr, mode >= 2 ? &b3 : nullptr, mode >= 2 ? &bd : nullptr, m3 ? mean : nullptr,
                                  m3 ? rstd : nullptr, m3 ? mean2 : nullptr, m3 ? rstd2 : nullptr, mode == 1 ? mask_bits : nullptr,
                                  m3 ? (bf16_t*)dz : nullptr, m3 ? (bf16_t*)dz2 : nullptr, m3 ? 1 : 0, mode, (hipStream_t)stream));
    return 0;
}

extern "C" int vpd_op_conv1x1_bn_dispatch(int n, int H, int W, int Kc, int Co, int two, int* out5) {
    if (!out5) return fail("null argument");
    if (!op_conv1x1_bn_shape_ok(n, H, W, 1, Kc, Co)) return fail("bad argument");
    static const double present = 0.0;
    ConvParams q = op_conv1x1_bn_params(nullptr, nullptr, n, H, W, 1, Kc, Co);
    if (two) { q.x2 = (const bf16_t*)&present; q.w2 = (const bf16_t*)&present; q.Kc2 = Kc; }
    int v[5] = {0, 0, 0, 0, 0};
    v[0] = two ? (int)vpd_conv1x1_bn2_eligible(q) : (int)vpd_conv1x1_bn_eligible(q);
    if (v[0]) vpd_conv1x1_bn_grid(q, two != 0, v + 1);
    memcpy(out5, v, sizeof v);
    return 0;
}

extern "C" int vpd_op_stem_pool_forward(const void* z, const float* scale, const float* shift, void* out_padded,
                                        unsigned char* idx, int n, int Hz, int Wz, int C, int opad, void* stream) {
    if (!z || !scale || !shift || !out_padded) return fail("null argument");
    if (n < 1 || Hz < 1 || Wz < 1 || C < 8 || C % 8 || opad < 0) return fail("bad shape");
    StemPoolParams q;
    memset(&q, 0, sizeof q);
    q.z = (const bf16_t*)z; q.Hz = Hz; q.Wz = Wz; q.scale = scale; q.shift = shift;
    q.out = (bf16_t*)out_padded; q.opad = opad; q.idx = idx;
    q.N = n; q.Ho = (Hz - 1) / 2 + 1; q.Wo = (Wz - 1) / 2 + 1; q.C = C;
    LCHECK(vpd_launch_stem_pool(q, (hipStream_t)stream));
    return 0;
}

extern "C" int vpd_op_stem_pool_backward(const void* dpool, const unsigned char* idx, const void* z, const float* mean,
                                         const float* rstd, const float* scale, const float* shift, const float* gamma,
                                         const float* beta, const void* pooled_padded, double* rows, float* coef, void* dz,
                                         float* dgamma, float* dbeta, int n, int Hz, int Wz, int C, void* stream) {
    if (!dpool || !idx || !z || !mean || !rstd || !scale || !shift || !gamma || !beta || !rows || !coef || !dz || !dgamma || !dbeta)
        return fail("null argument");
    if (n < 1 || Hz < 1 || Wz < 1 || C < 8 || C % 8 || 256 % (C / 8)) return fail("bad shape");
    StemPoolBwdParams sb;
    memset(&sb, 0, sizeof sb);
    sb.dpool = (const bf16_t*)dpool; sb.idx = idx; sb.z = (const bf16_t*)z;
    sb.mean = mean; sb.rstd = rstd; sb.scale = scale; sb.shift = shift; sb.partials = rows;
    sb.pooled = (const bf16_t*)pooled_padded; sb.ppad = 1; sb.gamma_p = gamma; sb.beta_p = beta;
    sb.M = n * Hz * Wz; sb.Hz = Hz; sb.Wz = Wz; sb.Ho = (Hz - 1) / 2 + 1; sb.Wo = (Wz - 1) / 2 + 1; sb.C = C;
    LCHECK(vpd_launch_stem_pool_bwd(sb, (float)sb.M, gamma, dgamma, dbeta, coef, (bf16_t*)dz, (hipStream_t)stream));
    return 0;
}

extern "C" int vpd_op_stem_dgrad(const void* dz, const float* w_oihw, float* dx_nchw, int n, int c_in, int H, int W, void* stream) {
    if (!dz || !w_oihw || !dx_nchw) return fail("null argument");
    if (n < 1) return fail("n must be at least 1");
    if (c_in < 1 || c_in > 8) return fail("c_in outside 1..8");
    if (H < 32 || W < 32 || (H & 1) || (W & 1)) return fail("H and W must be even and at least 32");
    if (reinterpret_cast<size_t>(dx_nchw) & 7) return fail("dx_nchw must be 8-byte aligned");
    LCHECK(vpd_launch_stem_dgrad((const bf16_t*)dz, w_oihw, dx_nchw, n, c_in, H, W, (hipStream_t)stream));
    return 0;
}

static BnBwdParams op_bn_bwd_params(void* dy, const void* z, const void* act_padded, const float* mean, const float* rstd,
                                    void* dz, int dzpad, int n, int H, int W, int C) {
    BnBwdParams b;
    memset(&b, 0, sizeof b);
    b.dy = (const bf16_t*)dy; b.dy_rw = (bf16_t*)dy; b.z = (const bf16_t*)z;
    b.act = (const bf16_t*)act_padded; b.aHp = H + 2; b.aWp = W + 2; b.apad = 1;
    b.mean = mean; b.rstd = rstd;
    b.dz = (bf16_t*)dz; b.dzHp = H + 2 * dzpad; b.dzWp = W + 2 * dzpad; b.dzpad = dzpad;
    b.M = n * H * W; b.H = H; b.W = W; b.C = C;
    return b;
}

extern "C" int vpd_op_bn_backward(void* dy, const void* z, const void* act_padded, const unsigned char* mask_bits,
                                  const float* mscale, const float* mshift, const float* dy_pooled, double* rows, float* coef,
                                  void* sync, unsigned* err, const float* gamma, const float* mean, const float* rstd, void* dz,
                                  int dzpad, float* dgamma, float* dbeta, int n, int H, int W, int C, int write_g, int fused,
                                  void* stream) {
    if (!dy || !z || !rows || !gamma || !mean || !rstd || !dz || !dgamma || !dbeta) return fail("null argument");
    if (n < 1 || H < 1 || W < 1 || C < 8 || C % 8 || dzpad < 0) return fail("bad shape");
    if ((mscale == nullptr) != (mshift == nullptr)) return fail("mscale and mshift come together");
    if ((act_padded != nullptr) + (mask_bits != nullptr) + (mscale != nullptr) > 1) return fail("one ReLU mask at most");
    if (write_g && !act_padded) return fail("write_g goes with the activation mask");
    BnBwdParams b = op_bn_bwd_params(dy, z, act_padded, mean, rstd, dz, dzpad, n, H, W, C);
    b.coef = coef; b.partials = rows; b.write_g = write_g; b.mscale = mscale; b.mshift = mshift; b.mask_bits = mask_bits;
    if (!fused) {
        if (mask_bits || dy_pooled) return fail("the three-launch path takes neither a ReLU bit map nor a pooled gradient");
        if (!coef) return fail("the three-launch path needs coef");
        LCHECK(vpd_launch_bn_bwd(b, (float)b.M, gamma, dgamma, dbeta, (hipStream_t)stream));
        return 0;
    }
    if (!sync || !err) return fail("the fused launch needs sync and err");
    if (!vpd_bn_bwd_fused_ok(b.M, C, act_padded != nullptr, write_g != 0)) return fail("no fused BatchNorm backward for this shape");
    if (dy_pooled) {
        if (!mask_bits) return fail("the folded average-pool gradient needs the ReLU bit map");
        if ((H * W) & (H * W - 1)) return fail("the folded average-pool gradient takes a power-of-two H W (vpd_op_avgpool_bwd first otherwise)");
        b.dy_pooled = dy_pooled; b.dy_pool_scale = 1.f / (float)(H * W);
    }
    BnFusedBwd f;
    memset(&f, 0, sizeof f);
    f.rows = rows; f.sync = sync; f.err = err; f.gamma = gamma; f.dgamma = dgamma; f.dbeta = dbeta; f.count = (float)b.M;
    LCHECK(vpd_launch_bn_bwd_fused(b, f, (hipStream_t)stream));
    return 0;
}

extern "C" int vpd_op_bn_backward_pair(void* dy, const void* act_padded, const void* zA, const float* meanA, const float* rstdA,
                                       const float* gammaA, double* rowsA, void* dzA, float* dgammaA, float* dbetaA,
                                       const void* zB, const float* meanB, const float* rstdB, const float* gammaB,
                                       double* rowsB, void* dzB, float* dgammaB, float* dbetaB, void* sync, unsigned* err, int n,
                                       int H, int W, int C, void* stream) {
    if (!dy || !act_padded || !zA || !meanA || !rstdA || !gammaA || !rowsA || !dzA || !dgammaA || !dbetaA || !zB || !meanB ||
        !rstdB || !gammaB || !rowsB || !dzB || !dgammaB || !dbetaB || !sync || !err)
        return fail("null argument");
    if (n < 1 || H < 1 || W < 1) return fail("bad shape");
    if (!vpd_bn_bwd_fused2_ok(n * H * W, C)) return fail("no paired BatchNorm backward for this shape");
    BnBwdParams b = op_bn_bwd_params(dy, zA, act_padded, meanA, rstdA, dzA, 1, n, H, W, C);
    BnFusedBwd fA;
    BnBwdSecond B;
    memset(&fA, 0, sizeof fA);
    memset(&B, 0, sizeof B);
    fA.rows = rowsA; fA.gamma = gammaA; fA.dgamma = dgammaA; fA.dbeta = dbetaA; fA.count = (float)b.M;
    fA.sync = sync; fA.err = err;
    B.f.rows = rowsB; B.f.gamma = gammaB; B.f.dgamma = dgammaB; B.f.dbeta = dbetaB; B.f.count = (float)b.M;
    B.z = (const bf16_t*)zB; B.mean = meanB; B.rstd = rstdB; B.dz = (bf16_t*)dzB;
    LCHECK(vpd_launch_bn_bwd_fused2(b, fA, B, (hipStream_t)stream));
    return 0;
}

extern "C" int vpd_op_bn_backward_residency(int M, int C, int pair, int* out4) {
    if (!out4 || M < 1 || C < 64 || C > 2048 || C % 8 || 1024 % (C / 8)) return fail("bad argument");
    const BnBwdFusedGeom q = vpd_bn_bwd_fused_geom(M, C, pair ? 3 : 2);
    out4[0] = q.G; out4[1] = q.keep[0]; out4[2] = q.keep[1]; out4[3] = q.keep[2];
    return 0;
}

extern "C" int vpd_op_avgpool(const void* act_padded, int n, int H, int W, int C, int pad, float* pooled, void* stream) {
    if (!act_padded || !pooled) return fail("null argument");
    if (n < 1 || H < 1 || W < 1 || C < 8 || C % 8 || pad < 0) return fail("bad shape");
    LCHECK(vpd_launch_avgpool((const bf16_t*)act_padded, H + 2 * pad, W + 2 * pad, pad, H, W, C, n, pooled, (hipStream_t)stream));
    return 0;
}

extern "C" int vpd_op_avgpool_bwd(const float* dpooled, int n, int H, int W, int C, void* dact, void* stream) {
    if (!dpooled || !dact) return fail("null argument");
    if (n < 1 || H < 1 || W < 1 || C < 8 || C % 8) return fail("bad shape");
    LCHECK(vpd_launch_avgpool_bwd(dpooled, H, W, C, n, (bf16_t*)dact, (hipStream_t)stream));
    return 0;
}

extern "C" int vpd_op_sgemm(const float* A, const float* B, float* Y, const float* bias, int M, int N, int K, int ta, int tb,
                            int relu, void* stream) {
    if (!A || !B || !Y) return fail("null argument");
    if (M < 1 || N < 1 || K < 1) return fail("bad shape");
    LCHECK(vpd_launch_sgemm(A, B, Y, bias, M, N, K, ta, tb, relu, (hipStream_t)stream));
    return 0;
}

extern "C" int vpd_op_colsum(const float* A, int M, int N, float* out, void* stream) {
    if (!A || !out || M < 1 || N < 1) return fail("bad argument");
    LCHECK(vpd_launch_colsum(A, M, N, out, (hipStream_t)stream));
    return 0;
}

extern "C" int vpd_op_relu_mask(float* d, const float* act, long long n, void* stream) {
    if (!d || !act || n < 1) return fail("bad argument");
    LCHECK(vpd_launch_relu_mask(d, act, (long)n, (hipStream_t)stream));
    return 0;
}

extern "C" int vpd_op_mse(const float* e, const float* t, long long n, float* de, float* loss_step, double* loss_accum,
                          void* stream) {
    if (!e || !t || n < 1) return fail("bad argument");
    LCHECK(vpd_launch_mse(e, t, (long)n, de, loss_step, loss_accum, (hipStream_t)stream));
    return 0;
}

extern "C" int vpd_op_wgrad(const void* dz, const void* x, float* dw, int n, int dzHp, int dzWp, int dzC, int dzpad,
                            int xHp, int xWp, int xC, int Hs, int Ws, int istr, int Kc, int Co, const int* tapset9,
                            float* slab, void* stream) {
    WgradParams q;
    memset(&q, 0, sizeof q);
    q.dz = (const bf16_t*)dz; q.dzHp = dzHp; q.dzWp = dzWp; q.dzC = dzC; q.dzpad = dzpad;
    q.x = (const bf16_t*)x; q.xHp = xHp; q.xWp = xWp; q.xC = xC; q.dw = dw; q.slab = slab;
    q.N = n; q.Hs = Hs; q.Ws = Ws; q.istr = istr; q.Kc = Kc; q.Co = Co; q.M = n * Hs * Ws;
    q.taps = tapset_from(tapset9);
    if (q.taps.nr < 1 || q.taps.nc < 1) return fail("empty tap set");
    LCHECK(vpd_launch_wgrad(q, (hipStream_t)stream));
    return 0;
}

extern "C" int vpd_op_wgrad_pair(const void* dz, const void* dz2, const void* x, float* dw, float* dw2, int n, int dzHp, int dzWp,
                                 int dzC, int dzpad, int xHp, int xWp, int xC, int Hs, int Ws, int istr, int Kc, int Co,
                                 const int* tapset9, float* slab, float* slab2, void* stream) {
    if (!dz || !dz2 || !x || !dw || !dw2 || !tapset9 || !slab || !slab2) return fail("null argument");
    if (n < 1 || Hs < 1 || Ws < 1) return fail("bad argument");
    WgradParams q;
    memset(&q, 0, sizeof q);
    q.dz = (const bf16_t*)dz; q.dzHp = dzHp; q.dzWp = dzWp; q.dzC = dzC; q.dzpad = dzpad;
    q.x = (const bf16_t*)x; q.xHp = xHp; q.xWp = xWp; q.xC = xC; q.dw = dw; q.slab = slab;
    q.N = n; q.Hs = Hs; q.Ws = Ws; q.istr = istr; q.Kc = Kc; q.Co = Co; q.M = n * Hs * Ws;
    WgradParams q1 = q;
    q1.dz = (const bf16_t*)dz2; q1.dw = dw2; q1.slab = slab2; q1.prefer_halo_1x1 = 1;
    q1.taps.nr = 1; q1.taps.nc = 1; q1.taps.dy0 = 1; q1.taps.dys = 1; q1.taps.dx0 = 1; q1.taps.dxs = 1;
    q1.taps.w0 = 0; q1.taps.wrs = 1; q1.taps.wcs = 1;
    q.taps = tapset_from(tapset9);
    if (!vpd_wgrad_pair_ok(q, q1)) return fail("not a pair the halo weight-gradient launch takes (shapes, or VPD_WGRAD_DS_RIDE=0 / VPD_WGRAD_1X1=0 / VPD_WGRAD_S2=0)");
    LCHECK(vpd_launch_wgrad_pair(q, q1, (hipStream_t)stream));
    return 0;
}
extern "C" int vpd_op_wgrad_pair_lds_bytes(int Hs, int Ws, int ns, long long* bytes) {
    return vpd_wgrad_pair_lds_query(Hs, Ws, ns, bytes);
}

extern "C" size_t vpd_op_wgrad128_table_bytes(void) { return vpd_wgrad128_table_bytes(); }
extern "C" size_t vpd_op_wgrad128_slab_floats(int Co, int Ci) { return vpd_wgrad_group_slab_floats(0, Co, Ci, 1) > vpd_wgrad_group_slab_floats(0, Co, Ci, 9) ? vpd_wgrad_group_slab_floats(0, Co, Ci, 1) : vpd_wgrad_group_slab_floats(0, Co, Ci, 9); }
extern "C" int vpd_op_wgrad128_group(int nprob, const void* const* dz, const void* const* x, float* const* dw,
                                     float* const* slab, const int* dims, void* dev_table, void* stream) {
    if (nprob < 1 || nprob > 18 || !dz || !x || !dw || !slab || !dims || !dev_table) return fail("bad argument");
    WgradParams qs[18];
    for (int i = 0; i < nprob; ++i) {
        const int n = dims[7 * i], H = dims[7 * i + 1], W = dims[7 * i + 2], Co = dims[7 * i + 3], Ci = dims[7 * i + 4];
        const int S = dims[7 * i + 5], ksz = dims[7 * i + 6];
        if ((S != 1 && S != 2) || (ksz != 1 && ksz != 3)) return fail("stride must be 1 or 2, k 1 or 3");
        WgradParams q;
        memset(&q, 0, sizeof q);
        q.dz = (const bf16_t*)dz[i]; q.dzHp = H + 2; q.dzWp = W + 2; q.dzC = Co; q.dzpad = 1;
        q.x = (const bf16_t*)x[i]; q.xHp = S * H + 2; q.xWp = S * W + 2; q.xC = Ci;
        q.dw = dw[i]; q.slab = slab[i];
        q.N = n; q.Hs = H; q.Ws = W; q.istr = S; q.Kc = Ci; q.Co = Co; q.M = n * H * W;
        if (ksz == 3) {
            q.taps.nr = 3; q.taps.nc = 3; q.taps.dy0 = 0; q.taps.dys = 1; q.taps.dx0 = 0; q.taps.dxs = 1;
            q.taps.w0 = 0; q.taps.wrs = 3; q.taps.wcs = 1;
        } else {
            q.taps.nr = 1; q.taps.nc = 1; q.taps.dy0 = 1; q.taps.dys = 1; q.taps.dx0 = 1; q.taps.dxs = 1;
            q.taps.w0 = 0; q.taps.wrs = 1; q.taps.wcs = 1;
        }
        if (!vpd_wgrad128_eligible(q)) return fail("shape not eligible for the 128 x 64 weight-gradient kernel");
        qs[i] = q;
    }
    LCHECK(vpd_launch_wgrad128_group(qs, nprob, nullptr, dev_table, (hipStream_t)stream));
    return 0;
}
```

vpd_amd/csrc/step.hip:

```cpp
#include <hip/hip_runtime.h>
#include <string.h>

#include <algorithm>
#include <vector>

#include "plan.h"

namespace {

struct Ctx {
    vpd_plan* p;
    char* ws;
    hipStream_t s;
    const float* params;
    int n;
    bf16_t* b16(size_t off) const { return reinterpret_cast<bf16_t*>(ws + off); }
    float* f32(size_t off) const { return reinterpret_cast<float*>(ws + off); }
    unsigned char* u8(size_t off) const { return reinterpret_cast<unsigned char*>(ws + off); }
    bf16_t* dz(const ConvInfo& cv, size_t shared_off) const { return b16(cv.dz_own_off ? cv.dz_own_off : shared_off); }
    double* stat_rows() const { return reinterpret_cast<double*>(ws + p->partial_off); }
    double* bn_rows(const BnInfo& b) const { return reinterpret_cast<double*>(ws + b.rows_off); }
    bool fused(const ConvInfo& cv) const { return p->fused_bn && !cv.stem; }
    float* bn_mean(const BnInfo& b) const { return f32(b.fl_off); }
    float* bn_rstd(const BnInfo& b) const { return f32(b.fl_off) + b.C; }
// ... 153 lines not shown
            ++ncls;
        }
    if (ncls == 0) return hipSuccess;
    q.ncls = ncls;
    if (ds) {
        if (q.oph != 0 || q.opw != 0 || q.taps.nr != 1 || q.taps.nc != 1 || ds->Co != cv.Co) return hipErrorInvalidValue;
        q.x2 = dzd; q.w2 = c.b16(c.p->arena_off) + ds->dgr_off; q.Kc2 = ds->Co;
    }
    if (sums) {
        q.bst_z = sums->z; q.bst_mask = sums->mask;
        q.stats = sums->rows; q.stat_rows = VPD_FUSED_ROWS;
        if (accumulate || !vpd_conv_takes_bn_sums(q)) return hipErrorInvalidValue;
    }
    return vpd_launch_conv(q, c.s);
}

hipError_t run_conv_wgrad(const Ctx& c, const ConvInfo& cv, const bf16_t* dz, const bf16_t* x, ZeroRanges* collect_zero = nullptr) {
    WgradParams q = wgrad_params(cv, c.n, dz, x);
    if (cv.stem) { q.dzHp = cv.Hout; q.dzWp = cv.Wout; q.dzpad = 0; q.xHp = c.p->xHp; q.xWp = c.p->xWp; q.xC = 8; }
    q.dw = c.f32(c.p->wg_off) + cv.wg_off;
    float* slab = c.f32(c.p->slab_off);
    q.slab = cv.slab_off >= 0 ? slab + cv.slab_off : (cv.stem ? slab : nullptr);
    q.prefer_halo_1x1 = !c.p->bottleneck;
    if (cv.slab_off >= 0 && !vpd_wgrad_overwrites(q)) q.slab = nullptr;
    if (collect_zero) {
        if (!vpd_wgrad_overwrites(q) && collect_zero->count < ZR_MAX) {
            collect_zero->ptr[collect_zero->count] = q.dw;
            collect_zero->n4[collect_zero->count++] = (long)cv.ntaps * cv.Co * cv.Kc / 4;
        }
        return hipSuccess;
    }
    if (vpd_wgrad_overwrites(q) && !cv.stem) {
        hipError_t e;
        {
            TimeScope ts(c.p, c.s, cv.stride == 1 ? 5 : 6, conv_flops(cv, c.n));
            q.defer_reduce = 1;
            e = vpd_launch_wgrad(q, c.s);
        }
        if (e != hipSuccess) return e;
        return vpd_launch_wgrad_reduce(q, c.s);
    }
    TimeScope ts(c.p, c.s, cv.stem ? 7 : (vpd_wgrad_overwrites(q) ? 5 : 6), conv_flops(cv, c.n));
    return vpd_launch_wgrad(q, c.s);
}

static void wgrad_pair_params(const Ctx& c, const ConvInfo& c1, const ConvInfo& cd, const bf16_t* dz1, const bf16_t* dzd, const bf16_t* x,
                              WgradParams* q3, WgradParams* q1) {
    float* slab = c.f32(c.p->slab_off);
    const ConvInfo* cvs[2] = {&c1, &cd};
    WgradParams* qs[2] = {q3, q1};
    for (int i = 0; i < 2; ++i) {
        *qs[i] = wgrad_params(*cvs[i], c.n, i ? dzd : dz1, x);
        qs[i]->dw = c.f32(c.p->wg_off) + cvs[i]->wg_off;
        qs[i]->slab = cvs[i]->slab_off >= 0 ? slab + cvs[i]->slab_off : nullptr;
        qs[i]->prefer_halo_1x1 = !c.p->bottleneck;
    }
}
bool wgrad_pair_ok(const Ctx& c, const ConvInfo& c1, const ConvInfo& cd) {
    if (c1.stem || cd.stem || c1.dz_own_off || cd.dz_own_off) return false;
    WgradParams q3, q1;
    wgrad_pair_params(c, c1, cd, c.b16(0), c.b16(0), c.b16(0), &q3, &q1);
    return vpd_wgrad_pair_ok(q3, q1);
}
hipError_t run_conv_wgrad_pair(const Ctx& c, const ConvInfo& c1, const ConvInfo& cd, const bf16_t* dz1, const bf16_t* dzd, const bf16_t* x) {
    WgradParams q3, q1;
    wgrad_pair_params(c, c1, cd, dz1, dzd, x, &q3, &q1);
    hipError_t e;
    {
        TimeScope ts(c.p, c.s, 6, conv_flops(c1, c.n) + conv_flops(cd, c.n));
        q3.defer_reduce = 1;
        e = vpd_launch_wgrad_pair(q3, q1, c.s);
    }
    if (e != hipSuccess) return e;
    return vpd_launch_wgrad_pair_reduce(q3, q1, c.s);
}

BnApplyParams bn_apply_params(const Ctx& c, const ConvInfo& cv, int res_kind, const bf16_t* res, bf16_t* out, int relu) {
    BnApplyParams a;
    memset(&a, 0, sizeof a);
    a.z = c.b16(cv.z_off);
    a.res_kind = res_kind; a.res = res; a.rHp = cv.Hout + 2; a.rWp = cv.Wout + 2; a.rpad = 1;
    a.out = out; a.oHp = cv.Hout + 2; a.oWp = cv.Wout + 2; a.opad = 1;
    a.M = c.n * cv.Hout * cv.Wout; a.H = cv.Hout; a.W = cv.Wout; a.C = cv.Co; a.relu = relu;
    return a;
}
hipError_t run_bn_apply(const Ctx& c, const ConvInfo& cv, int res_kind, const bf16_t* res, const ConvInfo* rcv,
                        bf16_t* out, int relu) {
    BnApplyParams a = bn_apply_params(c, cv, res_kind, res, out, relu);
    a.scale = c.bn_scale(cv.bn); a.shift = c.bn_shift(cv.bn);
    if (rcv) { a.rscale = c.bn_scale(rcv->bn); a.rshift = c.bn_shift(rcv->bn); }
    return vpd_launch_bn_apply(a, c.s);
}

hipError_t run_conv_train(const Ctx& c, const ConvInfo& cv, const bf16_t* x, float* bn_running) {
    hipError_t e = run_conv_fwd(c, cv, x, c.b16(cv.z_off), 0, true, nullptr, nullptr, nullptr, 0);
    if (e != hipSuccess || c.fused(cv)) return e;
    return run_bn_finalize(c, cv, bn_running);
}

int bn_xcd_tile_px(const Ctx& c, const ConvInfo& cv) {
    if (cv.k != 3 || cv.stride != 1 || cv.stem || cv.Ci != cv.Co) return 0;
    const ConvParams q = conv_dgrad_params(c, cv, c.b16(0), c.b16(0), 0);
    return vpd_conv_xcd_tile_px(q);
}

BnFusedFwd bn_fused_fwd(const Ctx& c, const ConvInfo& cv, float* bn_running, const ConvInfo* cv2 = nullptr) {
    BnFusedFwd f;
    memset(&f, 0, sizeof f);
    const BnInfo& b = cv.bn;
    f.rows = c.bn_rows(b); f.count = (float)(c.n * cv.Hout * cv.Wout);
    f.gamma = c.params + b.w_off; f.beta = c.params + b.b_off;
    f.rm = bn_running ? bn_running + b.rm_off : nullptr; f.rv = bn_running ? bn_running + b.rv_off : nullptr;
    f.mean = c.bn_mean(b); f.rstd = c.bn_rstd(b); f.scale = c.bn_scale(b); f.shift = c.bn_shift(b);
    if (cv2) {
        const BnFusedFwd g = bn_fused_fwd(c, *cv2, bn_running);
        f.rows2 = g.rows; f.count2 = g.count; f.gamma2 = g.gamma; f.beta2 = g.beta; f.rm2 = g.rm; f.rv2 = g.rv;
        f.mean2 = g.mean; f.rstd2 = g.rstd; f.scale2 = g.scale; f.shift2 = g.shift;
    }
    f.momentum = kBnMomentum; f.eps = kBnEps;
    return f;
}
hipError_t run_bn_fwd(const Ctx& c, const ConvInfo& cv, float* bn_running, int res_kind, const bf16_t* res,
                      const ConvInfo* rcv, bf16_t* out, int relu, unsigned char* mask_out = nullptr) {
    if (!c.fused(cv)) return run_bn_apply(c, cv, res_kind, res, rcv, out, relu);
    BnApplyParams a = bn_apply_params(c, cv, res_kind, res, out, relu);
    a.mask_out = mask_out;
    a.xcd_tile_px = bn_xcd_tile_px(c, cv);
    return vpd_launch_bn_fwd_fused(a, bn_fused_fwd(c, cv, bn_running, rcv), c.s);
}

BnBwdParams bn_bwd_params(const Ctx& c, const ConvInfo& cv, const bf16_t* dy, bf16_t* dz, int dzpad) {
    BnBwdParams b;
    memset(&b, 0, sizeof b);
    b.dy = dy; b.z = c.b16(cv.z_off);
    b.mean = c.bn_mean(cv.bn); b.rstd = c.bn_rstd(cv.bn);
    b.dz = dz; b.dzHp = cv.Hout + 2 * dzpad; b.dzWp = cv.Wout + 2 * dzpad; b.dzpad = dzpad;
    b.M = c.n * cv.Hout * cv.Wout; b.H = cv.Hout; b.W = cv.Wout; b.C = cv.Co;
    return b;
}
BnFusedBwd bn_bwd_side(const Ctx& c, const ConvInfo& cv, float* grads) {
    BnFusedBwd f;
    memset(&f, 0, sizeof f);
    f.rows = c.bn_rows(cv.bn);
    f.gamma = c.params + cv.bn.w_off; f.dgamma = grads + cv.bn.w_off; f.dbeta = grads + cv.bn.b_off;
    f.count = (float)(c.n * cv.Hout * cv.Wout);
    return f;
}
BnBwdSecond bn_bwd_second(const Ctx& c, const ConvInfo& cv, float* grads, bf16_t* dz) {
    return BnBwdSecond{bn_bwd_side(c, cv, grads), c.b16(cv.z_off), c.bn_mean(cv.bn), c.bn_rstd(cv.bn), dz};
}

bool relu_bits_ok(const Ctx& c, const ConvInfo& cv) {
    return c.p->relu_bits && c.fused(cv) && vpd_bn_bwd_fused_ok(c.n * cv.Hout * cv.Wout, cv.Co, false, false);
}
hipError_t run_bn_bwd(const Ctx& c, const ConvInfo& cv, bf16_t* dy, const bf16_t* act, bf16_t* dz, int dzpad,
                      int write_g, float* grads, bool relu_from_z = false, bool reduce_done = false,
                      const unsigned char* mask_bits = nullptr, const float* dy_pooled = nullptr) {
    BnBwdParams b = bn_bwd_params(c, cv, dy, dz, dzpad);
    b.dy_rw = dy; b.act = act; b.aHp = cv.Hout + 2; b.aWp = cv.Wout + 2; b.apad = 1;
    b.coef = c.bn_coef(cv.bn); b.partials = c.stat_rows(); b.write_g = write_g;
    if (mask_bits) { b.mask_bits = mask_bits; b.act = nullptr; b.write_g = 0; write_g = 0; }
    if (relu_from_z && !reduce_done) { b.act = nullptr; b.mscale = c.bn_scale(cv.bn); b.mshift = c.bn_shift(cv.bn); }
    if (reduce_done) b.act = nullptr;
    const bool fused = c.fused(cv) && !reduce_done && vpd_bn_bwd_fused_ok(b.M, b.C, b.act != nullptr, write_g != 0);
    if (dy_pooled) {
        const int hw = cv.Hout * cv.Wout;
        if (fused && mask_bits && vpd_switches().poolbwd_fold && (hw & (hw - 1)) == 0) { b.dy_pooled = dy_pooled; b.dy_pool_scale = 1.f / (float)hw; }
        else {
            hipError_t e = vpd_launch_avgpool_bwd(dy_pooled, cv.Hout, cv.Wout, cv.Co, c.n, dy, c.s);
            if (e != hipSuccess) return e;
        }
    }
    if (fused) {
        BnFusedBwd f = bn_bwd_side(c, cv, grads);
        f.sync = c.ws + cv.bn.sync_off; f.err = reinterpret_cast<unsigned*>(c.ws + c.p->syncerr_off);
        return vpd_launch_bn_bwd_fused(b, f, c.s);
    }
    return vpd_launch_bn_bwd(b, (float)b.M, c.params + cv.bn.w_off, grads + cv.bn.w_off, grads + cv.bn.b_off, c.s,
                             reduce_done);
}

hipError_t run_bn_bwd_apply(const Ctx& c, const ConvInfo& cv, const bf16_t* dy, bf16_t* dz, int dzpad, float* grads,
                            const unsigned char* mask_bits, const ConvInfo* cvB = nullptr, bf16_t* dzB = nullptr) {
    BnBwdParams b = bn_bwd_params(c, cv, dy, dz, dzpad);
    b.mask_bits = mask_bits;
    b.xcd_tile_px = bn_xcd_tile_px(c, cv);
    const BnFusedBwd f = bn_bwd_side(c, cv, grads);
    if (cvB) {
        const BnBwdSecond B = bn_bwd_second(c, *cvB, grads, dzB);
        return vpd_launch_bn_bwd_apply_fused(b, f, c.s, &B);
    }
    return vpd_launch_bn_bwd_apply_fused(b, f, c.s);
}

bool bn_bwd_pair_ok(const Ctx& c, const ConvInfo& A, const ConvInfo& Bc) {
    return c.fused(A) && c.fused(Bc) && A.Co == Bc.Co && vpd_bn_bwd_fused2_ok(c.n * A.Hout * A.Wout, A.Co);
}
hipError_t run_bn_bwd_pair(const Ctx& c, const ConvInfo& A, const ConvInfo& Bc, bf16_t* dy, const bf16_t* act, bf16_t* dzA,
                           bf16_t* dzB, float* grads) {
    BnBwdParams b = bn_bwd_params(c, A, dy, dzA, 1);
    b.dy_rw = dy; b.act = act; b.aHp = A.Hout + 2; b.aWp = A.Wout + 2; b.apad = 1;
    BnFusedBwd fA = bn_bwd_side(c, A, grads);
    fA.sync = c.ws + A.bn.sync_off;
    fA.err = reinterpret_cast<unsigned*>(c.ws + c.p->syncerr_off);
    return vpd_launch_bn_bwd_fused2(b, fA, bn_bwd_second(c, Bc, grads, dzB), c.s);
}

ConvParams conv3_params(const Ctx& c, const ConvInfo& cv, const bf16_t* x) {
    ConvParams q;
    memset(&q, 0, sizeof q);
    q.x = x; q.xHp = cv.Hin + 2; q.xWp = cv.Win + 2; q.xC = cv.Ci;
    q.w = c.b16(c.p->arena_off) + cv.fwd_off;
    q.yHp = cv.Hout; q.yWp = cv.Wout; q.yC = cv.Co; q.ypad = 0;
    q.N = c.n; q.Hs = cv.Hout; q.Ws = cv.Wout; q.osub = 1; q.istr = cv.stride;
    q.Kc = cv.Kc; q.Co = cv.Co; q.M = c.n * cv.Hout * cv.Wout;
    q.taps = conv_taps_fwd(cv);
    return q;
}
bool bneck_recompute_ok(const Ctx& c, const BlockInfo& B) {
    if (!c.p->bottleneck || B.ds || !c.p->train || !c.fused(B.c3) || !relu_bits_ok(c, B.c3)) return false;
    if (B.c3.k != 1 || B.c3.stride != 1) return false;
    return vpd_conv1x1_bn_eligible(conv3_params(c, B.c3, c.b16(B.a2_off)));
}
ConvParams conv3d_params(const Ctx& c, const BlockInfo& B, const bf16_t* xin) {
    ConvParams q = conv3_params(c, B.c3, c.b16(B.a2_off));
    q.x2 = xin; q.w2 = c.b16(c.p->arena_off) + B.cd.fwd_off; q.Kc2 = B.cd.Kc;
    return q;
}
bool bneck_recompute2_ok(const Ctx& c, const BlockInfo& B) {
    if (!c.p->bottleneck || !B.ds || !c.p->train || !c.fused(B.c3) || !c.fused(B.cd) || !relu_bits_ok(c, B.c3)) return false;
    if (B.c3.k != 1 || B.cd.k != 1 || B.c3.stride != 1 || B.cd.stride != 1 || B.c3.Ci != B.cd.Ci || B.c3.Co != B.cd.Co) return false;
    if (B.c3.Hin != B.cd.Hin || B.c3.Win != B.cd.Win) return false;
    return vpd_conv1x1_bn2_eligible(conv3d_params(c, B, c.b16(B.a2_off)));
}
hipError_t run_conv3d_bn_fwd(const Ctx& c, const BlockInfo& B, const bf16_t* xin, bf16_t* out, unsigned char* mask_out,
                             float* bn_running) {
    hipError_t e;
    for (int k = 0; k < 2; ++k) {
        const ConvInfo& cv = k ? B.cd : B.c3;
        ConvParams q = conv3_params(c, cv, k ? xin : c.b16(B.a2_off));
        q.stats = c.bn_rows(cv.bn); q.stat_rows = VPD_FUSED_ROWS;
        TimeScope ts(c.p, c.s, 4, 0.0);
        e = vpd_launch_conv1x1_bn(q, nullptr, nullptr, nullptr, nullptr, nullptr, nullptr, 0, 0, c.s);
        if (e != hipSuccess) return e;
    }
    ConvParams q = conv3d_params(c, B, xin);
    q.y = out; q.yHp = B.c3.Hout + 2; q.yWp = B.c3.Wout + 2; q.ypad = 1;
    const BnFusedFwd f = bn_fused_fwd(c, B.c3, bn_running, &B.cd);
    TimeScope ts(c.p, c.s, 4, conv_flops(B.c3, c.n) + conv_flops(B.cd, c.n));
    return vpd_launch_conv1x1_bn2(q, &f, nullptr, nullptr, nullptr, nullptr, nullptr, nullptr, mask_out, nullptr, nullptr, 0, 1, c.s);
}
hipError_t run_conv3d_bn_bwd(const Ctx& c, const BlockInfo& B, const bf16_t* xin, bf16_t* dout, const unsigned char* mask_bits,
                             bf16_t* dz3, bf16_t* dzd, float* grads) {
    ConvParams q = conv3d_params(c, B, xin);
    q.y = dout; q.acc_mask = mask_bits;
    const BnFusedBwd f3 = bn_bwd_side(c, B.c3, grads), fd = bn_bwd_side(c, B.cd, grads);
    hipError_t e;
    {
        TimeScope ts(c.p, c.s, 4, 0.0);
        e = vpd_launch_conv1x1_bn2(q, nullptr, &f3, &fd, nullptr, nullptr, nullptr, nullptr, nullptr, nullptr, nullptr, 0, 2, c.s);
    }
    if (e != hipSuccess) return e;
    TimeScope ts(c.p, c.s, 4, 0.0);
    return vpd_launch_conv1x1_bn2(q, nullptr, &f3, &fd, c.bn_mean(B.c3.bn), c.bn_rstd(B.c3.bn), c.bn_mean(B.cd.bn), c.bn_rstd(B.cd.bn),
                                  nullptr, dz3, dzd, 1, 3, c.s);
}
hipError_t run_conv3_bn_fwd(const Ctx& c, const ConvInfo& cv, const bf16_t* x, const bf16_t* res, bf16_t* out,
                            unsigned char* mask_out, float* bn_running) {
    ConvParams q = conv3_params(c, cv, x);
    q.stats = c.bn_rows(cv.bn); q.stat_rows = VPD_FUSED_ROWS;
    hipError_t e;
    {
        TimeScope ts(c.p, c.s, 4, 0.0);
        e = vpd_launch_conv1x1_bn(q, nullptr, nullptr, nullptr, nullptr, nullptr, nullptr, 0, 0, c.s);
    }
    if (e != hipSuccess) return e;
    q.stats = nullptr; q.stat_rows = 0;
    q.y = out; q.yHp = cv.Hout + 2; q.yWp = cv.Wout + 2; q.ypad = 1;
    q.res = res; q.rHp = cv.Hout + 2; q.rWp = cv.Wout + 2; q.rC = cv.Co; q.rpad = 1;
    const BnFusedFwd f = bn_fused_fwd(c, cv, bn_running);
    TimeScope ts(c.p, c.s, 4, conv_flops(cv, c.n));
    return vpd_launch_conv1x1_bn(q, &f, nullptr, nullptr, nullptr, mask_out, nullptr, 0, 1, c.s);
}
hipError_t run_conv3_bn_bwd(const Ctx& c, const ConvInfo& cv, const bf16_t* x, bf16_t* dout, const unsigned char* mask_bits,
                            bf16_t* dz, float* grads) {
    ConvParams q = conv3_params(c, cv, x);
    q.y = dout; q.acc_mask = mask_bits;
    const BnFusedBwd f = bn_bwd_side(c, cv, grads);
    hipError_t e;
    {
        TimeScope ts(c.p, c.s, 4, 0.0);
        e = vpd_launch_conv1x1_bn(q, nullptr, &f, nullptr, nullptr, nullptr, nullptr, 0, 2, c.s);
    }
    if (e != hipSuccess) return e;
    TimeScope ts(c.p, c.s, 4, 0.0);
    return vpd_launch_conv1x1_bn(q, nullptr, &f, c.bn_mean(cv.bn), c.bn_rstd(cv.bn), nullptr, dz, 1, 3, c.s);
}


int run_head(const Ctx& c, const bf16_t* last_act, float* emb_out, const float* target, bool need_grad,
             float* loss_step, double* loss_accum) {
    vpd_plan* p = c.p;
    const StageInfo& S = p->stages[3];
    LCHECK(vpd_launch_avgpool(last_act, S.H + 2, S.W + 2, 1, S.H, S.W, p->feat, c.n, c.f32(p->pooled_off), c.s));
    float* emb = (emb_out && !p->motion) ? emb_out : c.f32(p->emb_off);
    LCHECK(vpd_launch_sgemm(c.f32(p->pooled_off), c.params + p->fc.w_off, emb, c.params + p->fc.b_off, c.n, p->D, p->feat,
                            0, 1, 0, c.s));
    if (emb_out && emb != emb_out) LCHECK(hipMemcpyAsync(emb_out, emb, (size_t)c.n * p->D * 4, hipMemcpyDeviceToDevice, c.s));
    if (!target) return 0;
    const float* pred = emb;
    int pd = p->D;
    if (p->motion) {
        LCHECK(vpd_launch_sgemm(emb, c.params + p->dec[0].w_off, c.f32(p->h1_off), c.params + p->dec[0].b_off, c.n, 128,
                                p->D, 0, 1, 1, c.s));
        LCHECK(vpd_launch_sgemm(c.f32(p->h1_off), c.params + p->dec[1].w_off, c.f32(p->h2_off),
                                c.params + p->dec[1].b_off, c.n, 128, 128, 0, 1, 1, c.s));
        LCHECK(vpd_launch_sgemm(c.f32(p->h2_off), c.params + p->dec[2].w_off, c.f32(p->pred_off),
                                c.params + p->dec[2].b_off, c.n, 2 * p->D, 128, 0, 1, 0, c.s));
        pred = c.f32(p->pred_off);
        pd = 2 * p->D;
    }
    LCHECK(vpd_launch_mse(pred, target, (long)c.n * pd, need_grad ? c.f32(p->dpred_off) : nullptr, loss_step,
                          loss_accum, c.s));
    return 0;
}

ZeroRanges accumulator_zero_ranges(const Ctx& c) {
    ZeroRanges z;
    memset(&z, 0, sizeof z);
    z.ptr[0] = c.f32(c.p->partial_off); z.n4[0] = (long)c.p->partial_bytes / 16; z.count = 1;
    if (c.p->fused_bn) { z.ptr[1] = c.f32(c.p->fused_off); z.n4[1] = (long)c.p->fused_bytes / 16; z.count = 2; }
    return z;
}

StemPoolParams stem_pool_params(const Ctx& c, const float* scale, const float* shift, unsigned char* idx) {
    StemPoolParams sp;
    memset(&sp, 0, sizeof sp);
    sp.z = c.b16(c.p->z0_off); sp.Hz = c.p->H0; sp.Wz = c.p->W0;
    sp.scale = scale; sp.shift = shift;
    sp.out = c.b16(c.p->p0_off); sp.opad = 1; sp.idx = idx; sp.N = c.n; sp.Ho = c.p->H1; sp.Wo = c.p->W1; sp.C = 64;
    return sp;
}

int run_eval_forward(vpd_plan* p, const float* params, const float* x, int n, float* emb_out, const float* target,
                     float* loss_step, double* loss_accum, char* ws, hipStream_t s) {
    Ctx c{p, ws, s, params, n};
    if (x) LCHECK(vpd_launch_pack_input(x, n, p->c_in, p->H, p->W, c.b16(p->xin_off), p->xHp, p->xWp, 3, 8, s));
    bool pooled = false;
    if (vpd_switches().stem_pool_fused && n >= 64)
        LCHECK(run_conv_fwd(c, p->stem, c.b16(p->xin_off), c.b16(p->z0_off), 0, false, c.bn_escale(p->stem.bn),
                            c.bn_eshift(p->stem.bn), nullptr, 1, nullptr, c.b16(p->p0_off), &pooled));
    else
        LCHECK(run_conv_fwd(c, p->stem, c.b16(p->xin_off), c.b16(p->z0_off), 0, false, nullptr, nullptr, nullptr, 0));
    if (!pooled) LCHECK(vpd_launch_stem_pool(stem_pool_params(c, c.bn_escale(p->stem.bn), c.bn_eshift(p->stem.bn), nullptr), s));
    const bf16_t* cur = c.b16(p->p0_off);
    for (auto& B : p->blocks) {
        bf16_t* a1 = c.b16(B.a1_off);
        bf16_t* idb = c.b16(p->stages[B.stage].idn_off);
        const bool pair = B.ds && conv_pair_ok(c, B.c1, B.cd, false);
        const AltConv alt{&B.cd, idb, c.bn_escale(B.cd.bn), c.bn_eshift(B.cd.bn), 0};
        LCHECK(run_conv_fwd(c, B.c1, cur, a1, 1, false, c.bn_escale(B.c1.bn), c.bn_eshift(B.c1.bn), nullptr, 1, pair ? &alt : nullptr));
        const bf16_t* last_in = a1;
        if (p->bottleneck) {
            last_in = c.b16(B.a2_off);
            LCHECK(run_conv_fwd(c, B.c2, a1, c.b16(B.a2_off), 1, false, c.bn_escale(B.c2.bn), c.bn_eshift(B.c2.bn), nullptr, 1));
        }
        if (B.ds && !pair) LCHECK(run_conv_fwd(c, B.cd, cur, idb, 1, false, c.bn_escale(B.cd.bn), c.bn_eshift(B.cd.bn), nullptr, 0));
        const ConvInfo& last = p->bottleneck ? B.c3 : B.c2;
        LCHECK(run_conv_fwd(c, last, last_in, c.b16(B.out_off), 1, false, c.bn_escale(last.bn), c.bn_eshift(last.bn),
                            B.ds ? idb : cur, 1));
        cur = c.b16(B.out_off);
    }
    return run_head(c, cur, emb_out, target, false, loss_step, loss_accum);
}

struct WgradQueue {
    const Ctx& c;
    float* grads;
    void** bucket_events;
    bool lazy;
    struct Pending { const ConvInfo* cv; const bf16_t* dz; const bf16_t* x; };
    std::vector<Pending> pending;
    std::vector<int> deferred_buckets;

    hipError_t queue(const ConvInfo& cv, const bf16_t* dz, const bf16_t* x) {
        if (cv.dz_own_off) {
            pending.push_back({&cv, dz, x});
            return hipSuccess;
        }
        return run_conv_wgrad(c, cv, dz, x);
    }
    WgradParams task(const Pending& pd) const {
        WgradParams q = grouped_wgrad_params(*pd.cv, c.n, pd.dz, pd.x);
        q.dw = c.f32(c.p->wg_off) + pd.cv->wg_off;
        q.slab = c.f32(c.p->gslab_off) + pd.cv->gslab_off;
        return q;
    }
    hipError_t flush(int slot) {
        if (pending.empty()) return hipSuccess;
        vpd_plan* p = c.p;
        hipError_t r = hipSuccess;
        std::vector<Pending> rest;
        {
            std::vector<WgradParams> elig;
            std::vector<double> fl;
            for (const Pending& pd : pending) {
                const WgradParams q = task(pd);
                if (vpd_wgrad128_eligible(q)) { elig.push_back(q); fl.push_back(conv_flops(*pd.cv, c.n)); }
                else rest.push_back(pd);
            }
            const int total = (int)elig.size();
            const int nl = (total + 17) / 18;
            int at = 0;
            for (int l = 0; l < nl && r == hipSuccess; ++l) {
                const int cnt = (total - at + (nl - l) - 1) / (nl - l);
                double flops = 0.0;
                for (int i = 0; i < cnt; ++i) flops += fl[at + i];
                const int sl = (2 * slot + (l & 1)) & 7;
                if (l >= 2) {
                    if (p->wg2_cache[sl]) { vpd_wgrad128_cache_free(p->wg2_cache[sl]); p->wg2_cache[sl] = nullptr; }
                }
                if (!p->wg2_cache[sl]) p->wg2_cache[sl] = vpd_wgrad128_cache_new();
                TimeScope ts(p, c.s, 5, flops);
                r = vpd_launch_wgrad128_group(elig.data() + at, cnt, p->wg2_cache[sl], c.ws + p->wg2_tbl_off[sl], c.s);
                at += cnt;
            }
        }
        size_t done = 0;
        while (done < rest.size() && r == hipSuccess) {
            WgradParams qs[12];
            const int cnt = (int)std::min<size_t>(12, rest.size() - done);
            double flops = 0.0;
            int take = 0;
            for (int i = 0; i < cnt; ++i) {
                if (i > 0 && rest[done + i].cv->Hout != rest[done].cv->Hout) break;
                qs[take++] = task(rest[done + i]);
                flops += conv_flops(*rest[done + i].cv, c.n);
            }
            {
                TimeScope ts(p, c.s, 5, flops);
                r = vpd_launch_wgrad_group(qs, take, c.s);
            }
            done += take;
        }
        pending.clear();
        return r;
    }
    int unpack_bucket(int b) {
        const vpd_plan* p = c.p;
        int nb = (int)p->bmap_unpack[b].size() / 2;
        if (lazy) nb = b == 3 ? p->nstem_unpack_blocks : 0;
        if (nb > 0)
            LCHECK(vpd_launch_unpack_grads(reinterpret_cast<const PackDesc*>(c.ws + p->desc_off), (int)p->descs.size(),
                                           reinterpret_cast<const int*>(c.ws + p->bmap_unpack_off[b]), nb,
                                           c.f32(p->wg_off), grads, c.s));
        if (bucket_events && bucket_events[b]) LCHECK(hipEventRecord((hipEvent_t)bucket_events[b], c.s));
        return 0;
    }
    int stage_end(int bi) {
        const vpd_plan* p = c.p;
        const BlockInfo& B = p->blocks[bi];
        const bool last_of_stage = bi == 0 || p->blocks[bi - 1].stage != B.stage;
        if (!last_of_stage) return 0;
        if (p->wg_group && p->wg_merge34 && B.stage == 3 && bi > 0) { deferred_buckets.push_back(3 - B.stage); return 0; }
        LCHECK(flush(B.stage));
        for (int b : deferred_buckets)
            if (unpack_bucket(b)) return -1;
        deferred_buckets.clear();
        if (bi > 0) return unpack_bucket(3 - B.stage);
        return 0;
    }
};

struct Backward {
    const Ctx& c;
    float* grads;
    WgradQueue wq;
    bf16_t* G[3];
    int gi = 0;
    bool pool_pending = false;
    std::vector<char> bn2_sums_for;

    Backward(const Ctx& c_, float* grads_, void** bucket_events, bool lazy)
        : c(c_), grads(grads_), wq{c_, grads_, bucket_events, lazy},
          G{c_.b16(c_.p->G_off[0]), c_.b16(c_.p->G_off[1]), c_.b16(c_.p->G_off[2])}, bn2_sums_for(c_.p->blocks.size(), 0) {}

    const bf16_t* block_input(int bi) const { return bi == 0 ? c.b16(c.p->p0_off) : c.b16(c.p->blocks[bi - 1].out_off); }

    int head(bool scaled = true) {
        vpd_plan* p = c.p;
        const int n = c.n;
        hipStream_t s = c.s;
        const float* params = c.params;
        if (scaled) {
            if (p->scale_state)
                LCHECK(vpd_launch_scale_by_state(c.f32(p->dpred_off), (long)n * (p->motion ? 2 * p->D : p->D), p->scale_state, s));
            else if (p->loss_scale != 1.f)
                LCHECK(vpd_launch_scale(c.f32(p->dpred_off), (long)n * (p->motion ? 2 * p->D : p->D), p->loss_scale, s));
        }
        const float* demb = c.f32(p->dpred_off);
        if (p->motion) {
            const LinInfo* L = p->dec;
            LCHECK(vpd_launch_sgemm(c.f32(p->dpred_off), c.f32(p->h2_off), grads + L[2].w_off, nullptr, L[2].out, L[2].in, n, 1, 0, 0, s));
            LCHECK(vpd_launch_colsum(c.f32(p->dpred_off), n, L[2].out, grads + L[2].b_off, s));
            LCHECK(vpd_launch_sgemm(c.f32(p->dpred_off), params + L[2].w_off, c.f32(p->dh2_off), nullptr, n, L[2].in, L[2].out, 0, 0, 0, s));
            LCHECK(vpd_launch_relu_mask(c.f32(p->dh2_off), c.f32(p->h2_off), (long)n * 128, s));
            LCHECK(vpd_launch_sgemm(c.f32(p->dh2_off), c.f32(p->h1_off), grads + L[1].w_off, nullptr, L[1].out, L[1].in, n, 1, 0, 0, s));
            LCHECK(vpd_launch_colsum(c.f32(p->dh2_off), n, L[1].out, grads + L[1].b_off, s));
            LCHECK(vpd_launch_sgemm(c.f32(p->dh2_off), params + L[1].w_off, c.f32(p->dh1_off), nullptr, n, L[1].in, L[1].out, 0, 0, 0, s));
            LCHECK(vpd_launch_relu_mask(c.f32(p->dh1_off), c.f32(p->h1_off), (long)n * 128, s));
            LCHECK(vpd_launch_sgemm(c.f32(p->dh1_off), c.f32(p->emb_off), grads + L[0].w_off, nullptr, L[0].out, L[0].in, n, 1, 0, 0, s));
            LCHECK(vpd_launch_colsum(c.f32(p->dh1_off), n, L[0].out, grads + L[0].b_off, s));
            LCHECK(vpd_launch_sgemm(c.f32(p->dh1_off), params + L[0].w_off, c.f32(p->demb_off), nullptr, n, L[0].in, L[0].out, 0, 0, 0, s));
            demb = c.f32(p->demb_off);
        }
        LCHECK(vpd_launch_sgemm(demb, c.f32(p->pooled_off), grads + p->fc.w_off, nullptr, p->D, p->feat, n, 1, 0, 0, s));
        LCHECK(vpd_launch_colsum(demb, n, p->D, grads + p->fc.b_off, s));
        LCHECK(vpd_launch_sgemm(demb, params + p->fc.w_off, c.f32(p->dpooled_off), nullptr, n, p->feat, p->D, 0, 0, 0, s));
        const StageInfo& S = p->stages[3];
        if (!p->bottleneck && !p->blocks.back().ds) pool_pending = true;
        else LCHECK(vpd_launch_avgpool_bwd(c.f32(p->dpooled_off), S.H, S.W, p->feat, n, G[gi], s));
        return 0;
    }

    int inner_bn_bwd(const ConvInfo& cv, const bf16_t* dz, bf16_t* dx, const ConvInfo& bc, size_t mask_off, bf16_t* dzb) {
        if (mask_off && dgrad_takes_sums(c, cv, 0)) {
            const BnSums sm{c.b16(bc.z_off), c.u8(mask_off), c.bn_rows(bc.bn), nullptr, nullptr};
            LCHECK(run_conv_dgrad(c, cv, dz, dx, 0, nullptr, nullptr, nullptr, &sm));
            LCHECK(run_bn_bwd_apply(c, bc, dx, dzb, 1, grads, c.u8(mask_off)));
        } else {
            LCHECK(run_conv_dgrad(c, cv, dz, dx, 0));
            LCHECK(run_bn_bwd(c, bc, dx, nullptr, dzb, 1, 0, grads, true));
        }
        return 0;
    }

    const BnSums* prev_bn2_sums(int bi, BnSums& sm) {
        if (bi == 0) return nullptr;
        const BlockInfo& B = c.p->blocks[bi];
        const BlockInfo& Bp = c.p->blocks[bi - 1];
        if (!relu_bits_ok(c, Bp.c2)) return nullptr;
        if (Bp.ds && !(vpd_switches().dgrad_sums_pair && c.fused(Bp.c2) && c.fused(Bp.cd) && Bp.c2.Co == Bp.cd.Co)) return nullptr;
        if (!dgrad_takes_sums(c, B.c1, B.ds ? 0 : 1, Bp.ds)) return nullptr;
        sm = BnSums{c.b16(Bp.c2.z_off), c.u8(Bp.mask_off), c.bn_rows(Bp.c2.bn), Bp.ds ? c.b16(Bp.cd.z_off) : nullptr,
                    Bp.ds ? c.bn_rows(Bp.cd.bn) : nullptr};
        bn2_sums_for[bi - 1] = true;
        return &sm;
    }

    int basic_block(int bi) {
        const BlockInfo& B = c.p->blocks[bi];
        const StageInfo& S = c.p->stages[B.stage];
        const bf16_t* xin = block_input(bi);
        bf16_t* dout = G[gi];
        bf16_t* da1 = G[(gi + 1) % 3];
        bf16_t* dnew = G[(gi + 2) % 3];
        bf16_t* dz2 = c.dz(B.c2, S.dz2_off[bi & 1]);
        bf16_t* dz1 = c.dz(B.c1, S.dz1_off[bi & 1]);
        bf16_t* dzd = B.ds ? c.dz(B.cd, S.dzd_off) : nullptr;
        const unsigned char* mbits = (!B.ds && relu_bits_ok(c, B.c2)) ? c.u8(B.mask_off) : nullptr;
        bool bn_pair = false;
        if (bn2_sums_for[bi]) {
            LCHECK(run_bn_bwd_apply(c, B.c2, dout, dz2, 1, grads, c.u8(B.mask_off), B.ds ? &B.cd : nullptr, dzd));
            bn_pair = B.ds;
        } else if (B.ds && bn_bwd_pair_ok(c, B.c2, B.cd)) {
            LCHECK(run_bn_bwd_pair(c, B.c2, B.cd, dout, c.b16(B.out_off), dz2, dzd, grads));
            bn_pair = true;
        } else {
            LCHECK(run_bn_bwd(c, B.c2, dout, c.b16(B.out_off), dz2, 1, 1, grads, false, false, mbits,
                              pool_pending ? c.f32(c.p->dpooled_off) : nullptr));
            pool_pending = false;
        }
        LCHECK(wq.queue(B.c2, dz2, c.b16(B.a1_off)));
        if (inner_bn_bwd(B.c2, dz2, da1, B.c1, B.mask1_off, dz1)) return -1;
        const bool wg_pair = B.ds && wgrad_pair_ok(c, B.c1, B.cd);
        if (!wg_pair) LCHECK(wq.queue(B.c1, dz1, xin));
        BnSums sm;
        if (B.ds) {
            if (!bn_pair) LCHECK(run_bn_bwd(c, B.cd, dout, nullptr, dzd, 1, 0, grads));
            if (wg_pair) LCHECK(run_conv_wgrad_pair(c, B.c1, B.cd, dz1, dzd, xin));
            else LCHECK(wq.queue(B.cd, dzd, xin));
            if (conv_pair_ok(c, B.c1, B.cd, true)) {
                LCHECK(run_conv_dgrad(c, B.c1, dz1, dnew, 0, &B.cd, dzd, nullptr, prev_bn2_sums(bi, sm)));
            } else {
                LCHECK(run_conv_dgrad(c, B.c1, dz1, dnew, 0));
                LCHECK(run_conv_dgrad(c, B.cd, dzd, dnew, 1));
            }
            gi = (gi + 2) % 3;
        } else {
            LCHECK(run_conv_dgrad(c, B.c1, dz1, dout, 1, nullptr, nullptr, mbits, mbits ? prev_bn2_sums(bi, sm) : nullptr));
        }
        return wq.stage_end(bi);
    }

    int bottleneck_block(int bi) {
        const BlockInfo& B = c.p->blocks[bi];
        const StageInfo& S = c.p->stages[B.stage];
        const bf16_t* xin = block_input(bi);
        bf16_t* dout = G[gi];
        bf16_t* dnew = G[(gi + 2) % 3];
        bf16_t* dz3 = c.dz(B.c3, S.dz3_off);
        bf16_t* dz2 = c.dz(B.c2, S.dz2_off[bi & 1]);
        bf16_t* dz1 = c.dz(B.c1, S.dz1_off[bi & 1]);
        bf16_t* dzd = B.ds ? c.dz(B.cd, S.dzd_off) : nullptr;
        const unsigned char* mb3 = (!B.ds && relu_bits_ok(c, B.c3)) ? c.u8(B.mask_off) : nullptr;
        bool bn3_pair = false;
        if (B.ds && bneck_recompute2_ok(c, B)) {
            LCHECK(run_conv3d_bn_bwd(c, B, xin, dout, c.u8(B.mask_off), dz3, dzd, grads));
            bn3_pair = true;
        } else if (B.ds && bn_bwd_pair_ok(c, B.c3, B.cd)) {
            LCHECK(run_bn_bwd_pair(c, B.c3, B.cd, dout, c.b16(B.out_off), dz3, dzd, grads));
            bn3_pair = true;
        }
        if (bneck_recompute_ok(c, B)) LCHECK(run_conv3_bn_bwd(c, B.c3, c.b16(B.a2_off), dout, mb3, dz3, grads));
        else if (!bn3_pair) LCHECK(run_bn_bwd(c, B.c3, dout, c.b16(B.out_off), dz3, 1, 1, grads, false, false, mb3));
        LCHECK(wq.queue(B.c3, dz3, c.b16(B.a2_off)));
        if (inner_bn_bwd(B.c3, dz3, c.b16(c.p->T_off[0]), B.c2, B.mask2_off, dz2)) return -1;
        LCHECK(wq.queue(B.c2, dz2, c.b16(B.a1_off)));
        if (inner_bn_bwd(B.c2, dz2, c.b16(c.p->T_off[1]), B.c1, B.mask1_off, dz1)) return -1;
        LCHECK(wq.queue(B.c1, dz1, xin));
        if (B.ds) {
            if (!bn3_pair) LCHECK(run_bn_bwd(c, B.cd, dout, nullptr, dzd, 1, 0, grads));
            LCHECK(wq.queue(B.cd, dzd, xin));
            LCHECK(run_conv_dgrad(c, B.c1, dz1, dnew, 0));
            LCHECK(run_conv_dgrad(c, B.cd, dzd, dnew, 1));
            gi = (gi + 2) % 3;
        } else {
            LCHECK(run_conv_dgrad(c, B.c1, dz1, dout, 1, nullptr, nullptr, mb3));
        }
        return wq.stage_end(bi);
    }

    int stem() {
        const vpd_plan* p = c.p;
        StemPoolBwdParams sb;
        memset(&sb, 0, sizeof sb);
        sb.dpool = G[gi]; sb.idx = c.u8(p->idx_off); sb.z = c.b16(p->z0_off);
        sb.mean = c.bn_mean(p->stem.bn); sb.rstd = c.bn_rstd(p->stem.bn);
        sb.scale = c.bn_scale(p->stem.bn); sb.shift = c.bn_shift(p->stem.bn);
        sb.g = c.b16(p->g0_off); sb.partials = c.stat_rows();
        sb.pooled = c.b16(p->p0_off); sb.ppad = 1;
        sb.gamma_p = c.params + p->stem.bn.w_off; sb.beta_p = c.params + p->stem.bn.b_off;
        sb.M = c.n * p->H0 * p->W0; sb.Hz = p->H0; sb.Wz = p->W0; sb.Ho = p->H1; sb.Wo = p->W1; sb.C = 64;
        LCHECK(vpd_launch_stem_pool_bwd(sb, (float)sb.M, c.params + p->stem.bn.w_off, grads + p->stem.bn.w_off,
                                        grads + p->stem.bn.b_off, c.bn_coef(p->stem.bn), c.b16(p->dz0_off), c.s));
        LCHECK(wq.queue(p->stem, c.b16(p->dz0_off), c.b16(p->xin_off)));
        return wq.unpack_bucket(3);
    }
};

}

extern "C" int vpd_pack_weights(vpd_plan_t* p, const float* params, const float* bn_running, void* workspace,
                                void* stream) {
    if (!p || !workspace || !params) return fail("null argument");
    if (p->bound_ws != workspace) return fail("workspace not initialised with vpd_plan_init_workspace");
    hipStream_t s = (hipStream_t)stream;
    char* ws = (char*)workspace;
    Ctx c{p, ws, s, params, 1};
    LCHECK(vpd_launch_pack_weights(reinterpret_cast<const PackDesc*>(ws + p->desc_off), (int)p->descs.size(),
                                   reinterpret_cast<const int*>(ws + p->bmap_pack_off), (int)p->bmap_pack.size() / 2,
                                   params, c.b16(p->arena_off), s));
    if (bn_running)
        for (BnInfo* b : p->bns)
            LCHECK(vpd_launch_bn_fold(params + b->w_off, params + b->b_off, bn_running + b->rm_off,
                                      bn_running + b->rv_off, kBnEps, c.bn_escale(*b), c.bn_eshift(*b), b->C, s));
    return 0;
}

extern "C" int vpd_forward_eval(vpd_plan_t* p, const float* params, const float* x, int n, float* emb_out,
                                const float* target, float* loss_step, double* loss_accum, void* workspace,
                                void* stream) {
    if (check_call(p, workspace, n)) return -1;
    return run_eval_forward(p, params, x, n, emb_out, target, loss_step, loss_accum, (char*)workspace,
                            (hipStream_t)stream);
}

extern "C" int vpd_forward_train(vpd_plan_t* p, const float* params, float* bn_running, const float* x,
                                 const float* target, int n, float* emb_out, float* loss_step, double* loss_accum,
                                 void* workspace, void* stream) {
    if (check_call(p, workspace, n, 0)) return -1;
    if (!p->train) return fail("plan was created with train=0");
    hipStream_t s = (hipStream_t)stream;
    char* ws = (char*)workspace;
    if (n == 0) {
        if (loss_step) HCHECK(hipMemsetAsync(loss_step, 0, sizeof(float), s));
        return 0;
    }
    Ctx c{p, ws, s, params, n};
    p->fwd_had_x = x != nullptr;
    LCHECK(vpd_launch_zero_ranges(accumulator_zero_ranges(c), s));
    if (x) LCHECK(vpd_launch_pack_input(x, n, p->c_in, p->H, p->W, c.b16(p->xin_off), p->xHp, p->xWp, 3, 8, s));
    LCHECK(run_conv_fwd(c, p->stem, c.b16(p->xin_off), c.b16(p->z0_off), 0, true, nullptr, nullptr, nullptr, 0));
    LCHECK(run_bn_finalize(c, p->stem, bn_running));
    LCHECK(vpd_launch_stem_pool(stem_pool_params(c, c.bn_scale(p->stem.bn), c.bn_shift(p->stem.bn), c.u8(p->idx_off)), s));
    const bf16_t* cur = c.b16(p->p0_off);
    for (auto& B : p->blocks) {
        bf16_t* a1 = c.b16(B.a1_off);
        bf16_t* outp = c.b16(B.out_off);
        const bool pair = B.ds && conv_pair_ok(c, B.c1, B.cd, true);
        if (pair) {
            const AltConv alt{&B.cd, c.b16(B.cd.z_off), nullptr, nullptr, 0};
            LCHECK(run_conv_fwd(c, B.c1, cur, c.b16(B.c1.z_off), 0, true, nullptr, nullptr, nullptr, 0, &alt));
        } else {
            LCHECK(run_conv_train(c, B.c1, cur, bn_running));
        }
        LCHECK(run_bn_fwd(c, B.c1, bn_running, 0, nullptr, nullptr, a1, 1, B.mask1_off ? c.u8(B.mask1_off) : nullptr));
        const bf16_t* last_in = a1;
        if (p->bottleneck) {
            last_in = c.b16(B.a2_off);
            LCHECK(run_conv_train(c, B.c2, a1, bn_running));
            LCHECK(run_bn_fwd(c, B.c2, bn_running, 0, nullptr, nullptr, c.b16(B.a2_off), 1, B.mask2_off ? c.u8(B.mask2_off) : nullptr));
        }
        const ConvInfo& last = p->bottleneck ? B.c3 : B.c2;
        unsigned char* mbits = p->relu_bits ? c.u8(B.mask_off) : nullptr;
        if (bneck_recompute_ok(c, B)) {
            LCHECK(run_conv3_bn_fwd(c, B.c3, last_in, cur, outp, mbits, bn_running));
        } else if (bneck_recompute2_ok(c, B)) {
            LCHECK(run_conv3d_bn_fwd(c, B, cur, outp, mbits, bn_running));
        } else {
            LCHECK(run_conv_train(c, last, last_in, bn_running));
            if (B.ds) {
                if (!pair) LCHECK(run_conv_train(c, B.cd, cur, bn_running));
                LCHECK(run_bn_fwd(c, last, bn_running, 2, c.b16(B.cd.z_off), &B.cd, outp, 1, mbits));
            } else {
                LCHECK(run_bn_fwd(c, last, bn_running, 1, cur, nullptr, outp, 1, mbits));
            }
        }
        cur = outp;
    }
    return run_head(c, cur, emb_out, target, true, loss_step, loss_accum);
}

namespace {
int run_backward(vpd_plan* p, const float* params, float* grads, int n, void** bucket_events, char* ws, hipStream_t s, bool lazy,
                 const float* d_emb, float* dx_nchw) {
    p->grads_in_scratch = lazy;
    if (n == 0) {
        HCHECK(hipMemsetAsync(grads, 0, (size_t)p->nparam_padded * sizeof(float), s));
        if (lazy) HCHECK(hipMemsetAsync(ws + p->wg_off, 0, (size_t)p->wg_elems * sizeof(float), s));
        for (int b = 0; b < 4; ++b)
            if (bucket_events && bucket_events[b]) HCHECK(hipEventRecord((hipEvent_t)bucket_events[b], s));
        return 0;
    }
    Ctx c{p, ws, s, params, n};
    if (d_emb) HCHECK(hipMemcpyAsync(c.f32(p->dpred_off), d_emb, (size_t)n * p->D * sizeof(float), hipMemcpyDeviceToDevice, s));
    ZeroRanges zr = accumulator_zero_ranges(c);
    auto dry = [&](const ConvInfo& cv) { (void)run_conv_wgrad(c, cv, nullptr, nullptr, &zr); };
    for (auto& B : p->blocks) { dry(B.c1); dry(B.c2); if (p->bottleneck) dry(B.c3); if (B.ds) dry(B.cd); }
    dry(p->stem);
    if (zr.count >= ZR_MAX) {
        const int k = p->fused_bn ? 2 : 1;
        zr.ptr[k] = c.f32(p->wg_off); zr.n4[k] = (long)(p->wg_elems + 3) / 4; zr.count = k + 1;
    }
    LCHECK(vpd_launch_zero_ranges(zr, s));

    Backward bw(c, grads, bucket_events, lazy);
    if (bw.head(!d_emb)) return -1;
    for (int bi = (int)p->blocks.size() - 1; bi >= 0; --bi)
        if (p->bottleneck ? bw.bottleneck_block(bi) : bw.basic_block(bi)) return -1;
    if (bw.stem()) return -1;
    if (dx_nchw)
        LCHECK(vpd_launch_stem_dgrad(c.b16(p->dz0_off), params + p->stem.w_off, dx_nchw, n, p->c_in, p->H, p->W, s));
    return 0;
}
}

extern "C" int vpd_backward(vpd_plan_t* p, const float* params, float* grads, int n, void** bucket_events,
                            void* workspace, void* stream) {
    if (check_call(p, workspace, n, 0)) return -1;
    if (!p->train) return fail("plan was created with train=0");
    const bool lazy = p->lazy_next;
    p->lazy_next = false;
    return run_backward(p, params, grads, n, bucket_events, (char*)workspace, (hipStream_t)stream, lazy, nullptr, nullptr);
}

extern "C" int vpd_backward_ext(vpd_plan_t* p, const float* params, float* grads, const float* d_emb, int n, float* dx_nchw,
                                void** bucket_events, void* workspace, void* stream) {
    if (!p || !params || !grads || !d_emb || !workspace) return fail("vpd_backward_ext: null plan / params / grads / d_emb / workspace");
    if (!p->train) return fail("plan was created with train=0");
    if (p->motion) return fail("vpd_backward_ext: the plan has the motion head (d_emb is the gradient of the encoder's output)");
    if (n < 0 || n > p->max_batch) return fail("batch size outside 0..max_batch");
    if (p->bound_ws != workspace) return fail("workspace not initialised with vpd_plan_init_workspace");
    if (dx_nchw && (reinterpret_cast<size_t>(dx_nchw) & 7)) return fail("vpd_backward_ext: dx_nchw must be 8-byte aligned");
    if (dx_nchw && !p->fwd_had_x)
        return fail("vpd_backward_ext: dx_nchw needs a forward that took x (a batch staged by vpd_plan_stage_crops has no fp32 input)");
    p->lazy_next = false;
    return run_backward(p, params, grads, n, bucket_events, (char*)workspace, (hipStream_t)stream, false, d_emb, dx_nchw);
}

extern "C" int vpd_graph_capture_eval(vpd_plan_t* p, const float* params, const float* x, int n, float* emb_out,
                                      void* workspace, void* stream) {
    if (check_call(p, workspace, n)) return -1;
    hipStream_t s = (hipStream_t)stream;
    for (size_t i = 0; i < p->graphs.size(); ++i)
        if (p->graphs[i].n == n) {
            (void)hipGraphExecDestroy(p->graphs[i].e);
            (void)hipGraphDestroy(p->graphs[i].g);
            p->graphs.erase(p->graphs.begin() + i);
            break;
        }
    HCHECK(hipStreamBeginCapture(s, hipStreamCaptureModeThreadLocal));
    const int rc = run_eval_forward(p, params, x, n, emb_out, nullptr, nullptr, nullptr, (char*)workspace, s);
    hipGraph_t g = nullptr;
    hipError_t e = hipStreamEndCapture(s, &g);
    if (rc) { if (g) (void)hipGraphDestroy(g); return -1; }
    if (e != hipSuccess) return fail("hipStreamEndCapture", e);
    hipGraphExec_t ge = nullptr;
    e = hipGraphInstantiate(&ge, g, nullptr, nullptr, 0);
    if (e != hipSuccess) { (void)hipGraphDestroy(g); return fail("hipGraphInstantiate", e); }
    p->graphs.push_back({n, g, ge});
    return 0;
}

extern "C" int vpd_graph_launch_eval(vpd_plan_t* p, int n, void* stream) {
    for (auto& g : p->graphs)
        if (g.n == n) {
            HCHECK(hipGraphLaunch(g.e, (hipStream_t)stream));
            return 0;
        }
    return fail("no captured eval graph for this batch size");
// ... 2 lines not shown
```

vpd_amd/csrc/switches.h:

```cpp
#pragma once
#include <stdlib.h>

#define VPD_SWITCHES(X)                                        \
    X(fused_bn,           "VPD_FUSED_BN",          1)          \
    X(bn_pair,            "VPD_BN_PAIR",           1)          \
    X(bn_xcd,             "VPD_BN_XCD",            1)          \
    X(bn_xcd_force,       "VPD_BN_XCD_FORCE",     -1)          \
    X(dgrad_sums,         "VPD_DGRAD_SUMS",        1)          \
    X(dgrad_sums_l1,      "VPD_DGRAD_SUMS_L1",     1)          \
    X(dgrad_sums_s2,      "VPD_DGRAD_SUMS_S2",     1)          \
    X(dgrad_sums_pair,    "VPD_DGRAD_SUMS_PAIR",   1)          \
    X(dgrad_sums_1x1,     "VPD_DGRAD_SUMS_1X1",    1)          \
    X(relu_bits,          "VPD_RELU_BITS",         1)          \
    X(poolbwd_fold,       "VPD_POOLBWD_FOLD",      1)          \
    X(ds_merge,           "VPD_DS_MERGE",          1)          \
    X(pws,                "VPD_PWS",               1)          \
    X(pws_blocks,         "VPD_PWS_BLOCKS",        0)          \
    X(ws_256x64,          "VPD_WS_256x64",         1)          \
    X(ws_mw8,             "VPD_WS_MW8",            1)          \
    X(no_ws,              "VPD_NO_WS",             0)          \
    X(pws_geo,            "VPD_PWS_GEO",           1)          \
    X(pws_rot,            "VPD_PWS_ROT",           1)          \
    X(reserve_cus,        "VPD_RESERVE_CUS",       0)          \
    X(c64x2,              "VPD_C64X2",             1)          \
    X(c64_contig,         "VPD_C64_CONTIG",        1)          \
    X(conv1x1_ws,         "VPD_CONV1X1_WS",        1)          \
    X(conv_s2_ws,         "VPD_CONV_S2_WS",        1)          \
    X(conv_s2_dgrad_ws,   "VPD_CONV_S2_DGRAD_WS",  1)          \
    X(wg2,                "VPD_WG2",               1)          \
    X(wg2_1x1,            "VPD_WG2_1X1",           1)          \
    X(wg2_tco256,         "VPD_WG2_TCO256",        1)          \
    X(conv1x1_stream,     "VPD_CONV1X1_STREAM",    1)          \
    X(bneck_recompute,    "VPD_BNECK_RECOMPUTE",   1)          \
    X(wg_group,           "VPD_WG_GROUP",          1)          \
    X(wg_merge,           "VPD_WG_MERGE",          1)          \
    X(wgrad_1x1,          "VPD_WGRAD_1X1",        -1)          \
    X(wgrad_s2,           "VPD_WGRAD_S2",          1)          \
    X(wgrad_ds_ride,      "VPD_WGRAD_DS_RIDE",     1)          \
    X(stem_lds_store,     "VPD_STEM_LDS_STORE",    1)          \
    X(stem_pair,          "VPD_STEM_PAIR",         1)          \
    X(stem_quad,          "VPD_STEM_QUAD",         1)          \
    X(stem_poolsums,      "VPD_STEM_POOLSUMS",     1)          \
    X(stem_pool_fused,    "VPD_STEM_POOL_FUSED",   1)          \
    X(ablate,             "VPD_ABLATE",            0)

struct VpdSwitches {
#define VPD_SWITCH_FIELD(field, env, dflt) int field;
    VPD_SWITCHES(VPD_SWITCH_FIELD)
#undef VPD_SWITCH_FIELD
};

inline const VpdSwitches& vpd_switches() {
    static const VpdSwitches s = [] {
        VpdSwitches v;
#define VPD_SWITCH_READ(field, env, dflt) { const char* e = getenv(env); v.field = e ? atoi(e) : (dflt); }
        VPD_SWITCHES(VPD_SWITCH_READ)
#undef VPD_SWITCH_READ
        return v;
    }();
    return s;
}
```

Before: 78240 crops/s.

## Fuse head avgpool, FC, MSE loss and backward into single kernels

```diff
diff --git a/include/vpd_hip.h b/include/vpd_hip.h
--- a/include/vpd_hip.h
+++ b/include/vpd_hip.h
@@ -178,6 +178,11 @@
 int vpd_op_colsum(const float* A, int M, int N, float* out, void* stream);
 int vpd_op_relu_mask(float* d, const float* act, long long n, void* stream);
 int vpd_op_mse(const float* e, const float* t, long long n, float* de, float* loss_step, double* loss_accum, void* stream);
+int vpd_op_head_forward(const void* act_padded, int n, int H, int W, int C, int pad, const float* w, const float* bias,
+                        const float* target, float* pooled, float* emb, float* de, float* loss_step, double* loss_accum,
+                        unsigned* ticket, int D, const float* const* mlp_wb, float* h1, float* h2, float* pred, void* stream);
+int vpd_op_head_backward(const float* dy, const float* x, const float* w, const float* mask_act, float* dw, float* db, float* dx,
+                         int n, int out, int in, void* stream);
 int vpd_op_wgrad(const void* dz_bf16, const void* x_bf16, float* dw, int n, int dzHp, int dzWp, int dzC, int dzpad,
                  int xHp, int xWp, int xC, int Hs, int Ws, int istr, int Kc, int Co, const int* tapset9,
                  float* slab, void* stream);
diff --git a/vpd_amd/_lib.py b/vpd_amd/_lib.py
--- a/vpd_amd/_lib.py
+++ b/vpd_amd/_lib.py
@@ -85,6 +85,8 @@
     "vpd_op_colsum": (C.c_int, [vp, C.c_int, C.c_int, vp, vp]),
     "vpd_op_relu_mask": (C.c_int, [vp, vp, C.c_longlong, vp]),
     "vpd_op_mse": (C.c_int, [vp, vp, C.c_longlong, vp, vp, vp, vp]),
+    "vpd_op_head_forward": (C.c_int, [vp] + [C.c_int] * 5 + [vp] * 9 + [C.c_int] + [vp] * 5),
+    "vpd_op_head_backward": (C.c_int, [vp] * 7 + [C.c_int] * 3 + [vp]),
     "vpd_op_wgrad": (C.c_int, [vp, vp, vp] + [C.c_int] * 13 + [c_int_p, vp, vp]),
     "vpd_op_wgrad_slab_bytes": (C.c_size_t, []),
     "vpd_op_wgrad_pair": (C.c_int, [vp] * 5 + [C.c_int] * 13 + [c_int_p, vp, vp, vp]),
diff --git a/vpd_amd/csrc/head.hip b/vpd_amd/csrc/head.hip
--- a/vpd_amd/csrc/head.hip
+++ b/vpd_amd/csrc/head.hip
@@ -2,6 +2,33 @@
 #include "common.h"
 #include "kernels.h"
 
+static __device__ __forceinline__ void avgpool_item(const bf16_t* act, int Hp, int Wp, int pad, int H, int W, int C, int b, int c,
+                                                    float inv, float* out) {
+    float acc[8] = {0, 0, 0, 0, 0, 0, 0, 0};
+    if (H == 4 && W == 4) {
+        uint4 px[16];
+#pragma unroll
+        for (int q = 0; q < 16; ++q)
+            px[q] = *reinterpret_cast<const uint4*>(act + ((size_t)(b * Hp + (q >> 2) + pad) * Wp + (q & 3) + pad) * C + c);
+#pragma unroll
+        for (int q = 0; q < 16; ++q) {
+            float v[8];
+            unpack8(px[q], v);
+#pragma unroll
+            for (int j = 0; j < 8; ++j) acc[j] += v[j];
+        }
+    } else {
+        for (int y = 0; y < H; ++y)
+            for (int x = 0; x < W; ++x) {
+                float v[8];
+                unpack8(*reinterpret_cast<const uint4*>(act + ((size_t)(b * Hp + y + pad) * Wp + x + pad) * C + c), v);
+#pragma unroll
+                for (int j = 0; j < 8; ++j) acc[j] += v[j];
+            }
+    }
+#pragma unroll
+    for (int j = 0; j < 8; ++j) out[j] = acc[j] * inv;
+}
 __global__ __launch_bounds__(256) void avgpool_kernel(const bf16_t* act, int Hp, int Wp, int pad, int H, int W, int C,
                                                       int N, float* pooled) {
     const int cv = C >> 3;
@@ -10,31 +37,11 @@
     for (long it = (long)blockIdx.x * blockDim.x + threadIdx.x; it < total; it += (long)gridDim.x * blockDim.x) {
         const int b = (int)(it / cv);
         const int c = (int)(it - (long)b * cv) << 3;
-        float acc[8] = {0, 0, 0, 0, 0, 0, 0, 0};
-        if (H == 4 && W == 4) {
-            uint4 px[16];
-#pragma unroll
-            for (int q = 0; q < 16; ++q)
-                px[q] = *reinterpret_cast<const uint4*>(act + ((size_t)(b * Hp + (q >> 2) + pad) * Wp + (q & 3) + pad) * C + c);
-#pragma unroll
-            for (int q = 0; q < 16; ++q) {
-                float v[8];
-                unpack8(px[q], v);
-#pragma unroll
-                for (int j = 0; j < 8; ++j) acc[j] += v[j];
-            }
-        } else {
-            for (int y = 0; y < H; ++y)
-                for (int x = 0; x < W; ++x) {
-                    float v[8];
-                    unpack8(*reinterpret_cast<const uint4*>(act + ((size_t)(b * Hp + y + pad) * Wp + x + pad) * C + c), v);
-#pragma unroll
-                    for (int j = 0; j < 8; ++j) acc[j] += v[j];
-                }
-        }
-        float* o = pooled + (size_t)b * C + c;
-#pragma unroll
-        for (int j = 0; j < 8; ++j) o[j] = acc[j] * inv;
+        float o[8];
+        avgpool_item(act, Hp, Wp, pad, H, W, C, b, c, inv, o);
+        float* dst = pooled + (size_t)b * C + c;
+#pragma unroll
+        for (int j = 0; j < 8; ++j) dst[j] = o[j];
     }
 }
 hipError_t vpd_launch_avgpool(const bf16_t* act, int Hp, int Wp, int pad, int H, int W, int C, int N, float* pooled,
@@ -69,11 +76,11 @@
     return hipGetLastError();
 }
 
-__global__ __launch_bounds__(256) void sgemm_small_kernel(const float* A, const float* B, float* Y, const float* bias,
-                                                          int M, int N, int K, int ta, int tb, int relu) {
+static __device__ __forceinline__ void sgemm_small_body(const float* A, const float* B, float* Y, const float* bias, int M, int N,
+                                                        int K, int ta, int tb, int relu, const float* mask_act, int block) {
     const int lane = threadIdx.x & 63;
     const int tiles_n = (N + 15) >> 4;
-    const int tile = blockIdx.x * 4 + (threadIdx.x >> 6);
+    const int tile = block * 4 + (threadIdx.x >> 6);
     const int tm = tile / tiles_n, tn = tile - tm * tiles_n;
     if (tm * 16 >= M) return;
     const int r = lane & 15, kq = lane >> 4;
@@ -104,10 +111,15 @@
             if (mm < M) {
                 float v = acc[j] + bb;
                 if (relu) v = v > 0.f ? v : 0.f;
+                if (mask_act) v = mask_act[(size_t)mm * N + n] > 0.f ? v : 0.f;
                 Y[(size_t)mm * N + n] = v;
             }
         }
     }
+}
+__global__ __launch_bounds__(256) void sgemm_small_kernel(const float* A, const float* B, float* Y, const float* bias,
+                                                          int M, int N, int K, int ta, int tb, int relu) {
+    sgemm_small_body(A, B, Y, bias, M, N, K, ta, tb, relu, nullptr, blockIdx.x);
 }
 __global__ __launch_bounds__(256) void sgemm_nt_splitk_kernel(const float* A, const float* B, float* Y, const float* bias,
                                                               int M, int N, int K, int relu) {
@@ -167,10 +179,10 @@
     return hipGetLastError();
 }
 
-__global__ __launch_bounds__(256) void colsum_kernel(const float* A, int M, int N, float* out) {
+static __device__ __forceinline__ void colsum_body(const float* A, int M, int N, float* out, int block) {
     __shared__ float sh[8][32];
     const int tx = threadIdx.x & 31, ty = threadIdx.x >> 5;
-    const int n = blockIdx.x * 32 + tx;
+    const int n = block * 32 + tx;
     float a = 0.f;
     if (n < N)
         for (int m = ty; m < M; m += 8) a += A[(size_t)m * N + n];
@@ -183,6 +195,9 @@
         out[n] = t;
     }
 }
+__global__ __launch_bounds__(256) void colsum_kernel(const float* A, int M, int N, float* out) {
+    colsum_body(A, M, N, out, blockIdx.x);
+}
 hipError_t vpd_launch_colsum(const float* A, int M, int N, float* out, hipStream_t s) {
     hipLaunchKernelGGL(colsum_kernel, dim3((N + 31) / 32), dim3(256), 0, s, A, M, N, out);
     return hipGetLastError();
@@ -199,12 +214,10 @@
     return hipGetLastError();
 }
 
-__global__ __launch_bounds__(1024) void mse_kernel(const float* e, const float* t, long n, float* de,
-                                                   float* loss_step, double* loss_accum) {
-    __shared__ float sh[16];
+static __device__ __forceinline__ float mse_thread_sum(const float* e, const float* t, long n, float* de, int tid) {
     float a = 0.f;
     const long n4 = n >> 2;
-    for (long i0 = threadIdx.x; i0 < n4; i0 += 8 * 1024) {
+    for (long i0 = tid; i0 < n4; i0 += 8 * 1024) {
         float4 ev[8], tv[8];
 #pragma unroll
         for (int u = 0; u < 8; ++u) {
@@ -223,11 +236,17 @@
             }
         }
     }
-    for (long i = (n4 << 2) + threadIdx.x; i < n; i += 1024) {
+    for (long i = (n4 << 2) + tid; i < n; i += 1024) {
         const float d = e[i] - t[i];
         a += d * d;
         if (de) de[i] = 2.f * d;
     }
+    return a;
+}
+__global__ __launch_bounds__(1024) void mse_kernel(const float* e, const float* t, long n, float* de,
+                                                   float* loss_step, double* loss_accum) {
+    __shared__ float sh[16];
+    float a = mse_thread_sum(e, t, n, de, threadIdx.x);
     a = wave_sum(a);
     if ((threadIdx.x & 63) == 0) sh[threadIdx.x >> 6] = a;
     __syncthreads();
@@ -245,6 +264,252 @@
     return hipGetLastError();
 }
 
+
+#define VPD_HEAD_LDS_PAD 4
+#define VPD_HEAD_HID 128
+
+static __device__ __forceinline__ void head_pool_tile(const bf16_t* act, int Hp, int Wp, int pad, int H, int W, int K, int M, int tm,
+                                                      float* pl, int ldk, float* pooled, bool store) {
+    const int cv = K >> 3;
+    const float inv = 1.f / (float)(H * W);
+    for (int it = threadIdx.x; it < 16 * cv; it += blockDim.x) {
+        const int row = it / cv, c = (it - row * cv) << 3;
+        const int b = tm * 16 + row;
+        float o[8] = {0, 0, 0, 0, 0, 0, 0, 0};
+        if (b < M) {
+            avgpool_item(act, Hp, Wp, pad, H, W, K, b, c, inv, o);
+            if (store) {
+                float* dst = pooled + (size_t)b * K + c;
+#pragma unroll
+                for (int j = 0; j < 8; ++j) dst[j] = o[j];
+            }
+        }
+        float* l = pl + row * ldk + c;
+#pragma unroll
+        for (int j = 0; j < 8; ++j) l[j] = o[j];
+    }
+}
+static __device__ __forceinline__ void head_load_b(float4 (&bv)[4], const float4* Bp, bool nok, int k0, int kq, int kend) {
+#pragma unroll
+    for (int u = 0; u < 4; ++u) {
+        const int k = k0 + 16 * u + 4 * kq;
+        bv[u] = (nok && k < kend) ? Bp[k >> 2] : float4{0.f, 0.f, 0.f, 0.f};
+    }
+}
+static __device__ __forceinline__ f32x4 head_tile_quarter(const float* al, int lda, const float4* Bp, bool nok, float4 (&bv)[4],
+                                                          int kbeg, int kend, int r, int kq) {
+    f32x4 acc = {0.f, 0.f, 0.f, 0.f};
+    for (int k0 = kbeg; k0 < kend; k0 += 64) {
+        float4 av[4];
+#pragma unroll
+        for (int u = 0; u < 4; ++u) {
+            const int k = k0 + 16 * u + 4 * kq;
+            av[u] = k < kend ? *reinterpret_cast<const float4*>(al + r * lda + k) : float4{0.f, 0.f, 0.f, 0.f};
+        }
+#pragma unroll
+        for (int u = 0; u < 4; ++u) {
+            acc = __builtin_amdgcn_mfma_f32_16x16x4f32(av[u].x, bv[u].x, acc, 0, 0, 0);
+            acc = __builtin_amdgcn_mfma_f32_16x16x4f32(av[u].y, bv[u].y, acc, 0, 0, 0);
+            acc = __builtin_amdgcn_mfma_f32_16x16x4f32(av[u].z, bv[u].z, acc, 0, 0, 0);
+            acc = __builtin_amdgcn_mfma_f32_16x16x4f32(av[u].w, bv[u].w, acc, 0, 0, 0);
+        }
+        if (k0 + 64 < kend) head_load_b(bv, Bp, nok, k0 + 64, kq, kend);
+    }
+    return acc;
+}
+static __device__ __forceinline__ void head_ticket_loss(const float* pred, const float* target, long n, float* loss_step,
+                                                        double* loss_accum, unsigned* ticket, unsigned nblocks) {
+    __shared__ float sh[16];
+    __shared__ unsigned last;
+    asm volatile("s_waitcnt vmcnt(0)" ::: "memory");
+    __syncthreads();
+    if (threadIdx.x == 0) {
+        __builtin_amdgcn_fence(__ATOMIC_RELEASE, "agent");
+        asm volatile("s_waitcnt vmcnt(0)" ::: "memory");
+        const unsigned t = __hip_atomic_fetch_add(ticket, 1u, __ATOMIC_RELAXED, __HIP_MEMORY_SCOPE_AGENT);
+        last = t == nblocks - 1u;
+        if (t == nblocks - 1u) {
+            __hip_atomic_store(ticket, 0u, __ATOMIC_RELAXED, __HIP_MEMORY_SCOPE_AGENT);
+            __builtin_amdgcn_fence(__ATOMIC_ACQUIRE, "agent");
+            asm volatile("s_waitcnt vmcnt(0)" ::: "memory");
+        }
+    }
+    __syncthreads();
+    if (!last) return;
+    const int lane = threadIdx.x & 63, wave = threadIdx.x >> 6, nwaves = blockDim.x >> 6;
+    for (int vw = wave; vw < 16; vw += nwaves) {
+        float a = mse_thread_sum(pred, target, n, nullptr, vw * 64 + lane);
+        a = wave_sum(a);
+        if (lane == 0) sh[vw] = a;
+    }
+    __syncthreads();
+    if (threadIdx.x == 0) {
+        float tot = 0.f;
+#pragma unroll
+        for (int i = 0; i < 16; ++i) tot += sh[i];
+        if (loss_step) loss_step[0] = tot;
+        if (loss_accum) loss_accum[0] += (double)tot;
+    }
+}
+
+__global__ __launch_bounds__(256) void head_fwd_kernel(const bf16_t* act, int Hp, int Wp, int pad, int H, int W, const float* B,
+                                                       const float* bias, const float* target, float* pooled, float* Y, float* de,
+                                                       float* loss_step, double* loss_accum, unsigned* ticket, int M, int N, int K) {
+    extern __shared__ __align__(16) float pl[];
+    __shared__ float red[4][16][17];
+    const int lane = threadIdx.x & 63, wave = threadIdx.x >> 6;
+    const int tiles_n = (N + 15) >> 4;
+    const int tm = blockIdx.x / tiles_n, tn = blockIdx.x - tm * tiles_n;
+    const int r = lane & 15, kq = lane >> 4;
+    const int n = tn * 16 + r;
+    const bool nok = n < N;
+    const int ldk = K + VPD_HEAD_LDS_PAD;
+    const float4* Bp = reinterpret_cast<const float4*>(B + (size_t)(nok ? n : 0) * K);
+    const int kper = K / 4;
+    const int kbeg = wave * kper, kend = kbeg + kper;
+    float4 bv[4];
+    head_load_b(bv, Bp, nok, kbeg, kq, kend);
+    head_pool_tile(act, Hp, Wp, pad, H, W, K, M, tm, pl, ldk, pooled, tn == 0);
+    __syncthreads();
+    const f32x4 acc = head_tile_quarter(pl, ldk, Bp, nok, bv, kbeg, kend, r, kq);
+#pragma unroll
+    for (int j = 0; j < 4; ++j) red[wave][4 * kq + j][r] = acc[j];
+    __syncthreads();
+    if (wave == 0 && nok) {
+        const float bb = bias ? bias[n] : 0.f;
+#pragma unroll
+        for (int j = 0; j < 4; ++j) {
+            const int mm = tm * 16 + 4 * kq + j;
+            if (mm < M) {
+                const float v = ((red[0][4 * kq + j][r] + red[1][4 * kq + j][r]) + red[2][4 * kq + j][r]) + red[3][4 * kq + j][r] + bb;
+                Y[(size_t)mm * N + n] = v;
+                const float d = v - target[(size_t)mm * N + n];
+                de[(size_t)mm * N + n] = 2.f * d;
+            }
+        }
+    }
+    head_ticket_loss(Y, target, (long)M * N, loss_step, loss_accum, ticket, gridDim.x);
+}
+
+struct HeadMlpParams {
+    const bf16_t* act; int Hp, Wp, pad, H, W;
+    const float* w[4]; const float* b[4];
+    int nout[4], kin[4];
+    float* out[4];
+    float* out0b;
+    const float* target; float* pooled; float* de; float* loss_step; double* loss_accum; unsigned* ticket;
+    int M;
+};
+__global__ __launch_bounds__(1024) void head_fwd_mlp_kernel(const HeadMlpParams p) {
+    extern __shared__ __align__(16) float lds[];
+    __shared__ float red[16][16][17];
+    const int lane = threadIdx.x & 63, wave = threadIdx.x >> 6;
+    const int r = lane & 15, kq = lane >> 4;
+    const int tm = blockIdx.x;
+    const int ld0 = p.kin[0] + VPD_HEAD_LDS_PAD, ldh = VPD_HEAD_HID + VPD_HEAD_LDS_PAD, lde = p.nout[0] + VPD_HEAD_LDS_PAD;
+    const int xfl = 16 * ld0 > 32 * ldh ? 16 * ld0 : 32 * ldh;
+    float* bufX = lds;
+    float* bufE = lds + xfl;
+    const float* ain[4] = {bufX, bufE, bufX, bufX + 16 * ldh};
+    float* aout[4] = {bufE, bufX, bufX + 16 * ldh, nullptr};
+    const int lin[4] = {ld0, lde, ldh, ldh}, lout[4] = {lde, ldh, ldh, 0};
+    head_pool_tile(p.act, p.Hp, p.Wp, p.pad, p.H, p.W, p.kin[0], p.M, tm, bufX, ld0, p.pooled, true);
+    __syncthreads();
+#pragma unroll
+    for (int l = 0; l < 4; ++l) {
+        const int N = p.nout[l], K = p.kin[l];
+        const int tiles_n = (N + 15) >> 4;
+        const int kw = wave & 3;
+        const int kper = K / 4, kbeg = kw * kper, kend = kbeg + kper;
+        for (int t0 = 0; t0 < tiles_n; t0 += 4) {
+            const int tn = t0 + (wave >> 2);
+            const int n = tn * 16 + r;
+            const bool nok = tn < tiles_n && n < N;
+            const float4* Bp = reinterpret_cast<const float4*>(p.w[l] + (size_t)(nok ? n : 0) * K);
+            float4 bv[4];
+            head_load_b(bv, Bp, nok, kbeg, kq, kend);
+            const f32x4 acc = head_tile_quarter(ain[l], lin[l], Bp, nok, bv, kbeg, kend, r, kq);
+#pragma unroll
+            for (int j = 0; j < 4; ++j) red[wave][4 * kq + j][r] = acc[j];
+            __syncthreads();
+            if (kw == 0 && nok) {
+                const float bb = p.b[l] ? p.b[l][n] : 0.f;
+#pragma unroll
+                for (int j = 0; j < 4; ++j) {
+                    const int row = 4 * kq + j, mm = tm * 16 + row;
+                    float v = ((red[wave][row][r] + red[wave + 1][row][r]) + red[wave + 2][row][r]) + red[wave + 3][row][r] + bb;
+                    if (l == 1 || l == 2) v = v > 0.f ? v : 0.f;
+                    if (l < 3) aout[l][row * lout[l] + n] = mm < p.M ? v : 0.f;
+                    if (mm < p.M) {
+                        p.out[l][(size_t)mm * N + n] = v;
+                        if (l == 0 && p.out0b) p.out0b[(size_t)mm * N + n] = v;
+                        if (l == 3) {
+                            const float d = v - p.target[(size_t)mm * N + n];
+                            p.de[(size_t)mm * N + n] = 2.f * d;
+                        }
+                    }
+                }
+            }
+            __syncthreads();
+        }
+    }
+    head_ticket_loss(p.out[3], p.target, (long)p.M * p.nout[3], p.loss_step, p.loss_accum, p.ticket, gridDim.x);
+}
+static size_t head_fwd_lds(int C, int D, int motion) {
+    const size_t x = (size_t)16 * (C + VPD_HEAD_LDS_PAD);
+    if (!motion) return x * sizeof(float);
+    const size_t h = (size_t)32 * (VPD_HEAD_HID + VPD_HEAD_LDS_PAD);
+    return ((x > h ? x : h) + (size_t)16 * (D + VPD_HEAD_LDS_PAD)) * sizeof(float);
+}
+bool vpd_head_fwd_ok(int C, int D, int motion) {
+    if (C < 64 || C % 64 || D < 1) return false;
+    if (motion && (D < 64 || D % 64)) return false;
+    return head_fwd_lds(C, D, motion) + (motion ? 18 : 5) * 1024 <= 64 * 1024;
+}
+hipError_t vpd_launch_head_fwd(const bf16_t* act, int Hp, int Wp, int pad, int H, int W, int C, int N, const float* w,
+                               const float* bias, const float* target, float* pooled, float* emb, float* de, float* loss_step,
+                               double* loss_accum, unsigned* ticket, int D, hipStream_t s) {
+    if (!vpd_head_fwd_ok(C, D, 0)) return hipErrorInvalidValue;
+    const int tiles = ((N + 15) / 16) * ((D + 15) / 16);
+    hipLaunchKernelGGL(head_fwd_kernel, dim3(tiles), dim3(256), head_fwd_lds(C, D, 0), s, act, Hp, Wp, pad, H, W, w, bias, target,
+                       pooled, emb, de, loss_step, loss_accum, ticket, N, D, C);
+    return hipGetLastError();
+}
+hipError_t vpd_launch_head_fwd_mlp(const bf16_t* act, int Hp, int Wp, int pad, int H, int W, int C, int N, const float* const* w4,
+                                   const float* const* b4, const float* target, float* pooled, float* emb, float* emb2, float* h1,
+                                   float* h2, float* pred, float* de, float* loss_step, double* loss_accum, unsigned* ticket, int D,
+                                   hipStream_t s) {
+    if (!vpd_head_fwd_ok(C, D, 1)) return hipErrorInvalidValue;
+    HeadMlpParams p;
+    p.act = act; p.Hp = Hp; p.Wp = Wp; p.pad = pad; p.H = H; p.W = W;
+    const int nout[4] = {D, VPD_HEAD_HID, VPD_HEAD_HID, 2 * D}, kin[4] = {C, D, VPD_HEAD_HID, VPD_HEAD_HID};
+    float* out[4] = {emb, h1, h2, pred};
+    for (int i = 0; i < 4; ++i) { p.w[i] = w4[i]; p.b[i] = b4[i]; p.nout[i] = nout[i]; p.kin[i] = kin[i]; p.out[i] = out[i]; }
+    p.out0b = emb2; p.target = target; p.pooled = pooled; p.de = de; p.loss_step = loss_step; p.loss_accum = loss_accum;
+    p.ticket = ticket; p.M = N;
+    hipLaunchKernelGGL(head_fwd_mlp_kernel, dim3((N + 15) / 16), dim3(1024), head_fwd_lds(C, D, 1), s, p);
+    return hipGetLastError();
+}
+
+__global__ __launch_bounds__(256) void head_bwd_kernel(const float* dy, const float* x, const float* w, const float* mask_act,
+                                                       float* dw, float* db, float* dx, int n, int out, int in, int nb_dw,
+                                                       int nb_db) {
+    int b = blockIdx.x;
+    if (b < nb_dw) { sgemm_small_body(dy, x, dw, nullptr, out, in, n, 1, 0, 0, nullptr, b); return; }
+    b -= nb_dw;
+    if (b < nb_db) { colsum_body(dy, n, out, db, b); return; }
+    b -= nb_db;
+    sgemm_small_body(dy, w, dx, nullptr, n, in, out, 0, 0, 0, mask_act, b);
+}
+hipError_t vpd_launch_head_bwd(const float* dy, const float* x, const float* w, const float* mask_act, float* dw, float* db,
+                               float* dx, int n, int out, int in, hipStream_t s) {
+    const int nb_dw = (((out + 15) / 16) * ((in + 15) / 16) + 3) / 4;
+    const int nb_db = (out + 31) / 32;
+    const int nb_dx = (((n + 15) / 16) * ((in + 15) / 16) + 3) / 4;
+    hipLaunchKernelGGL(head_bwd_kernel, dim3(nb_dw + nb_db + nb_dx), dim3(256), 0, s, dy, x, w, mask_act, dw, db, dx, n, out, in,
+                       nb_dw, nb_db);
+    return hipGetLastError();
+}
 
 __global__ __launch_bounds__(256) void scale_kernel(float* x, long n, float s) {
     for (long i = (long)blockIdx.x * 256 + threadIdx.x; i < n; i += (long)gridDim.x * 256) x[i] *= s;
diff --git a/vpd_amd/csrc/kernels.h b/vpd_amd/csrc/kernels.h
--- a/vpd_amd/csrc/kernels.h
+++ b/vpd_amd/csrc/kernels.h
@@ -167,6 +167,16 @@
 hipError_t vpd_launch_relu_mask(float* d, const float* act, long n, hipStream_t s);
 hipError_t vpd_launch_mse(const float* e, const float* t, long n, float* de, float* loss_step, double* loss_accum,
                           hipStream_t s);
+bool vpd_head_fwd_ok(int C, int D, int motion);
+hipError_t vpd_launch_head_fwd_mlp(const bf16_t* act, int Hp, int Wp, int pad, int H, int W, int C, int N, const float* const* w4,
+                                   const float* const* b4, const float* target, float* pooled, float* emb, float* emb2, float* h1,
+                                   float* h2, float* pred, float* de, float* loss_step, double* loss_accum, unsigned* ticket, int D,
+                                   hipStream_t s);
+hipError_t vpd_launch_head_fwd(const bf16_t* act, int Hp, int Wp, int pad, int H, int W, int C, int N, const float* w,
+                               const float* bias, const float* target, float* pooled, float* emb, float* de, float* loss_step,
+                               double* loss_accum, unsigned* ticket, int D, hipStream_t s);
+hipError_t vpd_launch_head_bwd(const float* dy, const float* x, const float* w, const float* mask_act, float* dw, float* db,
+                               float* dx, int n, int out, int in, hipStream_t s);
 
 hipError_t vpd_launch_pack_input(const float* x, int N, int C, int H, int W, bf16_t* out, int Hp, int Wp, int pad,
                                  int Cp, hipStream_t s);
diff --git a/vpd_amd/csrc/plan.h b/vpd_amd/csrc/plan.h
--- a/vpd_amd/csrc/plan.h
+++ b/vpd_amd/csrc/plan.h
@@ -104,6 +104,7 @@
     bool fused_bn = true;
     size_t fused_off = 0, fused_bytes = 0;
     size_t syncerr_off = 0;
+    size_t head_ticket_off = 0;
     bool wg_group = true;
     size_t gslab_off = 0;
     bool dgrad_sums = true;
diff --git a/vpd_amd/csrc/plan.hip b/vpd_amd/csrc/plan.hip
--- a/vpd_amd/csrc/plan.hip
+++ b/vpd_amd/csrc/plan.hip
@@ -241,6 +241,7 @@
             b->rows_off = bp.take((size_t)VPD_FUSED_ROWS * 2 * b->C * sizeof(double));
             b->sync_off = bp.take(VPD_GRID_SYNC_BYTES);
         }
+        p->head_ticket_off = bp.take(256);
         p->fused_off = start; p->fused_bytes = bp.cur - start;
         p->syncerr_off = bp.take(256);
     }
@@ -1127,6 +1128,44 @@
     return 0;
 }
 
+extern "C" int vpd_op_head_forward(const void* act_padded, int n, int H, int W, int C, int pad, const float* w, const float* bias,
+                                   const float* target, float* pooled, float* emb, float* de, float* loss_step, double* loss_accum,
+                                   unsigned* ticket, int D, const float* const* mlp_wb, float* h1, float* h2, float* pred,
+                                   void* stream) {
+    if (!act_padded || !w || !target || !pooled || !emb || !de || !ticket) return fail("vpd_op_head_forward: null argument");
+    if (n < 1 || H < 1 || W < 1 || D < 1 || pad < 0) return fail("vpd_op_head_forward: bad shape");
+    const int motion = mlp_wb != nullptr;
+    if (motion != (h1 != nullptr) || motion != (h2 != nullptr) || motion != (pred != nullptr))
+        return fail("vpd_op_head_forward: mlp_wb, h1, h2 and pred come together");
+    if (motion)
+        for (int i = 0; i < 6; ++i)
+            if (!mlp_wb[i]) return fail("vpd_op_head_forward: null argument");
+    if (!vpd_head_fwd_ok(C, D, motion))
+        return fail("vpd_op_head_forward: C must be a multiple of 64, at most 896 (the motion head: D a multiple of 64, C + D at most 704): a 16-crop row tile in LDS");
+    size_t al = reinterpret_cast<size_t>(emb) | reinterpret_cast<size_t>(target) | reinterpret_cast<size_t>(w);
+    if (motion) al |= reinterpret_cast<size_t>(pred) | reinterpret_cast<size_t>(mlp_wb[0]) | reinterpret_cast<size_t>(mlp_wb[2]) | reinterpret_cast<size_t>(mlp_wb[4]);
+    if (al & 15) return fail("vpd_op_head_forward: weights, target, emb and pred must be 16-byte aligned");
+    const bf16_t* act = (const bf16_t*)act_padded;
+    if (motion) {
+        const float* w4[4] = {w, mlp_wb[0], mlp_wb[2], mlp_wb[4]};
+        const float* b4[4] = {bias, mlp_wb[1], mlp_wb[3], mlp_wb[5]};
+        LCHECK(vpd_launch_head_fwd_mlp(act, H + 2 * pad, W + 2 * pad, pad, H, W, C, n, w4, b4, target, pooled, emb, nullptr, h1, h2, pred,
+                                       de, loss_step, loss_accum, ticket, D, (hipStream_t)stream));
+        return 0;
+    }
+    LCHECK(vpd_launch_head_fwd(act, H + 2 * pad, W + 2 * pad, pad, H, W, C, n, w, bias, target, pooled, emb, de, loss_step, loss_accum,
+                               ticket, D, (hipStream_t)stream));
+    return 0;
+}
+
+extern "C" int vpd_op_head_backward(const float* dy, const float* x, const float* w, const float* mask_act, float* dw, float* db,
+                                    float* dx, int n, int out, int in, void* stream) {
+    if (!dy || !x || !w || !dw || !db || !dx) return fail("vpd_op_head_backward: null argument");
+    if (n < 1 || out < 1 || in < 1) return fail("vpd_op_head_backward: bad shape");
+    LCHECK(vpd_launch_head_bwd(dy, x, w, mask_act, dw, db, dx, n, out, in, (hipStream_t)stream));
+    return 0;
+}
+
 extern "C" int vpd_op_wgrad(const void* dz, const void* x, float* dw, int n, int dzHp, int dzWp, int dzC, int dzpad,
                             int xHp, int xWp, int xC, int Hs, int Ws, int istr, int Kc, int Co, const int* tapset9,
                             float* slab, void* stream) {
diff --git a/vpd_amd/csrc/step.hip b/vpd_amd/csrc/step.hip
--- a/vpd_amd/csrc/step.hip
+++ b/vpd_amd/csrc/step.hip
@@ -479,6 +479,23 @@
              float* loss_step, double* loss_accum) {
     vpd_plan* p = c.p;
     const StageInfo& S = p->stages[3];
+    if (need_grad && target && vpd_switches().head_fused && vpd_head_fwd_ok(p->feat, p->D, p->motion) &&
+        (!p->motion || (p->dec[0].out == 128 && p->dec[1].out == 128 && p->dec[2].out == 2 * p->D))) {
+        unsigned* ticket = reinterpret_cast<unsigned*>(c.ws + p->head_ticket_off);
+        if (p->motion) {
+            const float* w4[4] = {c.params + p->fc.w_off, c.params + p->dec[0].w_off, c.params + p->dec[1].w_off, c.params + p->dec[2].w_off};
+            const float* b4[4] = {c.params + p->fc.b_off, c.params + p->dec[0].b_off, c.params + p->dec[1].b_off, c.params + p->dec[2].b_off};
+            LCHECK(vpd_launch_head_fwd_mlp(last_act, S.H + 2, S.W + 2, 1, S.H, S.W, p->feat, c.n, w4, b4, target, c.f32(p->pooled_off),
+                                           c.f32(p->emb_off), emb_out, c.f32(p->h1_off), c.f32(p->h2_off), c.f32(p->pred_off),
+                                           c.f32(p->dpred_off), loss_step, loss_accum, ticket, p->D, c.s));
+            return 0;
+        }
+        float* emb = emb_out ? emb_out : c.f32(p->emb_off);
+        LCHECK(vpd_launch_head_fwd(last_act, S.H + 2, S.W + 2, 1, S.H, S.W, p->feat, c.n, c.params + p->fc.w_off,
+                                   c.params + p->fc.b_off, target, c.f32(p->pooled_off), emb, c.f32(p->dpred_off), loss_step,
+                                   loss_accum, ticket, p->D, c.s));
+        return 0;
+    }
     LCHECK(vpd_launch_avgpool(last_act, S.H + 2, S.W + 2, 1, S.H, S.W, p->feat, c.n, c.f32(p->pooled_off), c.s));
     float* emb = (emb_out && !p->motion) ? emb_out : c.f32(p->emb_off);
     LCHECK(vpd_launch_sgemm(c.f32(p->pooled_off), c.params + p->fc.w_off, emb, c.params + p->fc.b_off, c.n, p->D, p->feat,
@@ -676,24 +693,33 @@
                 LCHECK(vpd_launch_scale(c.f32(p->dpred_off), (long)n * (p->motion ? 2 * p->D : p->D), p->loss_scale, s));
         }
         const float* demb = c.f32(p->dpred_off);
+        const bool one = vpd_switches().head_fused != 0;
         if (p->motion) {
             const LinInfo* L = p->dec;
-            LCHECK(vpd_launch_sgemm(c.f32(p->dpred_off), c.f32(p->h2_off), grads + L[2].w_off, nullptr, L[2].out, L[2].in, n, 1, 0, 0, s));
-            LCHECK(vpd_launch_colsum(c.f32(p->dpred_off), n, L[2].out, grads + L[2].b_off, s));
-            LCHECK(vpd_launch_sgemm(c.f32(p->dpred_off), params + L[2].w_off, c.f32(p->dh2_off), nullptr, n, L[2].in, L[2].out, 0, 0, 0, s));
-            LCHECK(vpd_launch_relu_mask(c.f32(p->dh2_off), c.f32(p->h2_off), (long)n * 128, s));
-            LCHECK(vpd_launch_sgemm(c.f32(p->dh2_off), c.f32(p->h1_off), grads + L[1].w_off, nullptr, L[1].out, L[1].in, n, 1, 0, 0, s));
-            LCHECK(vpd_launch_colsum(c.f32(p->dh2_off), n, L[1].out, grads + L[1].b_off, s));
-            LCHECK(vpd_launch_sgemm(c.f32(p->dh2_off), params + L[1].w_off, c.f32(p->dh1_off), nullptr, n, L[1].in, L[1].out, 0, 0, 0, s));
-            LCHECK(vpd_launch_relu_mask(c.f32(p->dh1_off), c.f32(p->h1_off), (long)n * 128, s));
-            LCHECK(vpd_launch_sgemm(c.f32(p->dh1_off), c.f32(p->emb_off), grads + L[0].w_off, nullptr, L[0].out, L[0].in, n, 1, 0, 0, s));
-            LCHECK(vpd_launch_colsum(c.f32(p->dh1_off), n, L[0].out, grads + L[0].b_off, s));
-            LCHECK(vpd_launch_sgemm(c.f32(p->dh1_off), params + L[0].w_off, c.f32(p->demb_off), nullptr, n, L[0].in, L[0].out, 0, 0, 0, s));
+            const float* dy[3] = {c.f32(p->dh1_off), c.f32(p->dh2_off), c.f32(p->dpred_off)};
+            const float* xin[3] = {c.f32(p->emb_off), c.f32(p->h1_off), c.f32(p->h2_off)};
+            float* dx[3] = {c.f32(p->demb_off), c.f32(p->dh1_off), c.f32(p->dh2_off)};
+            for (int i = 2; i >= 0; --i) {
+                if (one) {
+                    LCHECK(vpd_launch_head_bwd(dy[i], xin[i], params + L[i].w_off, i ? xin[i] : nullptr, grads + L[i].w_off,
+                                               grads + L[i].b_off, dx[i], n, L[i].out, L[i].in, s));
+                    continue;
+                }
+                LCHECK(vpd_launch_sgemm(dy[i], xin[i], grads + L[i].w_off, nullptr, L[i].out, L[i].in, n, 1, 0, 0, s));
+                LCHECK(vpd_launch_colsum(dy[i], n, L[i].out, grads + L[i].b_off, s));
+                LCHECK(vpd_launch_sgemm(dy[i], params + L[i].w_off, dx[i], nullptr, n, L[i].in, L[i].out, 0, 0, 0, s));
+                if (i) LCHECK(vpd_launch_relu_mask(dx[i], xin[i], (long)n * 128, s));
+            }
             demb = c.f32(p->demb_off);
         }
-        LCHECK(vpd_launch_sgemm(demb, c.f32(p->pooled_off), grads + p->fc.w_off, nullptr, p->D, p->feat, n, 1, 0, 0, s));
-        LCHECK(vpd_launch_colsum(demb, n, p->D, grads + p->fc.b_off, s));
-        LCHECK(vpd_launch_sgemm(demb, params + p->fc.w_off, c.f32(p->dpooled_off), nullptr, n, p->feat, p->D, 0, 0, 0, s));
+        if (one) {
+            LCHECK(vpd_launch_head_bwd(demb, c.f32(p->pooled_off), params + p->fc.w_off, nullptr, grads + p->fc.w_off,
+                                       grads + p->fc.b_off, c.f32(p->dpooled_off), n, p->D, p->feat, s));
+        } else {
+            LCHECK(vpd_launch_sgemm(demb, c.f32(p->pooled_off), grads + p->fc.w_off, nullptr, p->D, p->feat, n, 1, 0, 0, s));
+            LCHECK(vpd_launch_colsum(demb, n, p->D, grads + p->fc.b_off, s));
+            LCHECK(vpd_launch_sgemm(demb, params + p->fc.w_off, c.f32(p->dpooled_off), nullptr, n, p->feat, p->D, 0, 0, 0, s));
+        }
         const StageInfo& S = p->stages[3];
         if (!p->bottleneck && !p->blocks.back().ds) pool_pending = true;
         else LCHECK(vpd_launch_avgpool_bwd(c.f32(p->dpooled_off), S.H, S.W, p->feat, n, G[gi], s));
diff --git a/vpd_amd/csrc/switches.h b/vpd_amd/csrc/switches.h
--- a/vpd_amd/csrc/switches.h
+++ b/vpd_amd/csrc/switches.h
@@ -42,6 +42,7 @@
     X(stem_quad,          "VPD_STEM_QUAD",         1)          \
     X(stem_poolsums,      "VPD_STEM_POOLSUMS",     1)          \
     X(stem_pool_fused,    "VPD_STEM_POOL_FUSED",   1)          \
+    X(head_fused,         "VPD_HEAD_FUSED",        1)          \
     X(ablate,             "VPD_ABLATE",            0)
 
 struct VpdSwitches {
```

Result: no change. 78530 crops/s (median of 6 runs) (+0.4%).
